# rajan-dubey8/camouflage-multimodal

Measured on AMD Instinct MI355X. Metric: images/sec fwd+bwd (fusion model train step: fwd + loss + bwd + clip + AdamW), higher is better.
Workload: dtype bf16; 1 GPU; BASELINE configs[1] on the path that exists (SURVEY 8d): cross-attention fusion model, packed variable-Nr minibatch (Nr ~ real 303..530 histogram, mean 483), Nk=13 real KG rows, train mode dropout 0.3, random-init weights; batch_per_gpu=16, global_batch=16, rg_dim=128, hidden_dim=256, num_heads=8, parallelism=dp1, precision=bf16 MFMA operands, fp32 accumulate/optimizer

## Files before the change

### camouflage_multimodal_amd/csrc/fused_rows.h

```cpp
#pragma once
#include "common.h"

typedef unsigned short us16;

struct ShadowJob { us16* dst; int N, K, transposed, nsrc; const float* src[4]; int rows[4]; int ld[4]; int chunk_begin; int lo; };
#define SHADOW_MAXJ 24
#define SHADOW_MAXZ 24
struct ShadowBatch { ShadowJob j[SHADOW_MAXJ]; int n; void* zero_ptr[SHADOW_MAXZ]; size_t zero_bytes[SHADOW_MAXZ]; int nzero; };
int launch_weight_shadows(ShadowBatch& sb, hipStream_t stream);

struct FrontStream {
  const float* X; int M;
  const us16* W0; const float* b0;
  const us16* W1; const float* bq; const float* bkv;
  us16* X16;
  us16* R16; us16* Q16; us16* KV16;
  int tile_begin;
};
#define FUSED_FRONT_MAXZ 4
#define FUSED_FRONT_MAXX 20
#define FUSED_BWD1_MAXZ 16
struct FrontArgs {
  FrontStream s[2]; float qscale; int save; unsigned long long* stamps; int exp;
  void* zero_ptr[FUSED_FRONT_MAXZ]; unsigned zero_bytes[FUSED_FRONT_MAXZ]; int nzero;
  int split3;
  ShadowJob xjob[FUSED_FRONT_MAXX]; int nxjob; int xchunks; int xblock0;
};
int launch_fused_front(FrontArgs& a, int variant, hipStream_t stream);

struct BackStream {
  const us16* Wo; const float* bo; const us16* W1; const float* b1; const float* ln_g; const float* ln_b;
  const us16* R16;
  us16* O16; us16* Y16; us16* XH16; float* rstd; uint32_t* mask;
  float* Ymean; float* Hmean;
  uint32_t site_ffn;
};
struct BackArgs {
  BackStream s[2];
  const us16* Q16; const us16* KV16;
  const us16* Q2_16; const us16* KV2_16;
  const int* off; const int* tile_off; const float* inv_nr;
  const int4* tile_desc;
  float* lse2;
  int lead_tiles;
  float* part; int* tickets; int max_splits;
  int B, Nk, rg_tiles_max, rows_rg;
  DropCfg drop; int save; int exp;
  unsigned long long* stamps;
  int save_lse2;
};
int launch_fused_back(BackArgs& a, int variant, int lead_mode, hipStream_t stream);

struct Bwd1Stream {
  const us16* W1T; const us16* WoT;
  const uint32_t* mask; const us16* XH16; const float* rstd; const float* ln_g;
  const float* dHm; int ld_dHm;
  const float* dcomb; int ld_dcomb;
  us16* dH16; us16* dU16;
  float* dgamma; float* dbeta;
};
struct TailWgProd { const float* dy; const float* x; float* dW; float* db; int ld_dy, ld_x, rows, cols; int tile_begin; };
#define TAIL_WG_MAXP 8
struct TailWgArgs { TailWgProd p[TAIL_WG_MAXP]; int n, B, tiles; };
struct Bwd1Args {
  Bwd1Stream s[2];
  const us16* Q16; const us16* KV16;
  us16* dQKV16; float* dKV;
  const us16* O2_16; us16* dO2_16; float* delta2;
  const int* off; const int* tile_off; const float* inv_nr; const int4* tile_desc;
  const int* row_sample;
  int B, Nk, rg_tiles_max, rows_rg; float qscale; DropCfg drop; unsigned long long* stamps;
  int exp;
  int writer_blocks, writer_first_row;
  void* zero_ptr[FUSED_BWD1_MAXZ]; unsigned zero_bytes[FUSED_BWD1_MAXZ]; int nzero;
  TailWgArgs twg;
};
int launch_fused_bwd1(Bwd1Args& a, int variant, hipStream_t stream, int kg_only = 0);
int launch_wide2_bwd1(Bwd1Args& a, int variant, hipStream_t stream);
size_t fused_bwd1_lds();

struct Bwd2Args {
  const us16* Q2_16; const us16* dO2_16; const float* lse2; const float* delta2;
  const us16* KV2_16;
  us16* dQKV16;
  const us16* dU16; const us16* WcRgT; us16* dR16;
  float* dQ2acc;
  const float* dKV;
  const us16* dU2_16; const us16* WcKgT; us16* dQKVkg16; us16* dG16;
  float* dGpart;
  int* tickets;
  const int* off; const int* tile_off; const int4* tile_desc;
  int B, Nk, rg_tiles_max, rows_rg; float qscale; DropCfg drop; unsigned long long* stamps;
  int param_space;
  int split_finish;
};
int launch_fused_bwd2(Bwd2Args& a, int variant, hipStream_t stream);
int launch_wide2_bwd2(Bwd2Args& a, hipStream_t stream);
size_t fused_bwd2_lds();

#define FUSED_PART_FLOATS 544
#define FUSED_MAX_SPLITS 64
size_t fused_front_lds();
size_t fused_back_lds();

#define FUSED_WIDE_MAXSEG 48
int launch_wide_front(FrontArgs& a, int rt, hipStream_t stream, int kg_only = 0);
int launch_wide_rgfwd(const FrontStream& f, float qscale, BackArgs& b, int rt, int max_nr, hipStream_t stream);
int launch_wide_back(BackArgs& a, int rt, int max_nr, hipStream_t stream);
int wide_max_rows(int rt);

int launch_fold_rg(const float* Wq, const float* Wkv, const float* bq, const float* bkv, const float* Wrg, const float* brg, us16* Wf, float* bf, hipStream_t stream);
int launch_wide2_rgfwd(const FrontStream& f, const us16* Wf, const float* bf, float qscale, BackArgs& b, int max_nr, int save_r16, hipStream_t stream);
int wide2_max_rows();
```

### camouflage_multimodal_amd/csrc/fused_rows.hip

```cpp
#include "fused_rows.h"
#include "shadow_inl.h"
#include "gemm.h"
#include "mfma_inl.h"

namespace {

template <int NT, int KS, bool W_IS_A, int DEPTH, bool USE_ROT = true>
struct Stage {
  static constexpr int TOTAL = NT * KS;
  static constexpr int D = DEPTH < TOTAL ? DEPTH : TOTAL;
  static_assert(!USE_ROT || (KS & (KS - 1)) == 0, "rotated k order: power-of-two k steps");
  u32x4 buf[D];
  const u32x4* wp; int rot;
  __device__ __forceinline__ int keff(int ks) const { return USE_ROT ? ((ks + rot) & (KS - 1)) : ks; }
  __device__ __forceinline__ const u32x4* wptr(int i) const { return wp + 64 * (keff(i / NT) * NT + (i % NT)); }
  __device__ __forceinline__ void prefetch(const u32x4* __restrict__ wp_, int rot_) {
    wp = wp_; rot = rot_;
#pragma unroll
    for (int i = 0; i < D; ++i) buf[i] = *wptr(i);
  }
  __device__ __forceinline__ void run(const char* act, f32x16 (&acc)[NT]) {
    run_f([&](int ks) { return *reinterpret_cast<const bf16x8*>(act + 32 * ks); }, acc);
  }
  template <class F>
// ... 424 lines not shown
      if (h == 0) red[slot * 128 + w * 32 + l31] = p;
      __syncthreads();
      return (red[slot * 128 + l31] + red[slot * 128 + 32 + l31]) + (red[slot * 128 + 64 + l31] + red[slot * 128 + 96 + l31]);
    };
    const float mean = row_total(part, 0) * (1.0f / 256.0f);
    float sq = 0.f;
#pragma unroll
    for (int i = 0; i < 32; ++i) { u[i] -= mean; sq = fmaf(u[i], u[i], sq); }
    const float rstd = 1.0f / sqrtf(row_total(sq, 1) * (1.0f / 256.0f) + 1e-5f);
    rstd_keep = rstd;
    const bool rok = l31 < nrows;
#pragma unroll
    for (int t = 0; t < 2; ++t) {
      float ys[16];
#pragma unroll
      for (int g = 0; g < 4; ++g) {
        const int c0 = 64 * w + 32 * t + 8 * g + 4 * h;
        const float4 gm = *reinterpret_cast<const float4*>(S.ln_g + c0), bt = *reinterpret_cast<const float4*>(S.ln_b + c0);
        float* o = u + 16 * t + 4 * g;
        const float x0 = o[0] * rstd, x1 = o[1] * rstd, x2 = o[2] * rstd, x3 = o[3] * rstd;
        const float4 y = make_float4(x0 * gm.x + bt.x, x1 * gm.y + bt.y, x2 * gm.z + bt.z, x3 * gm.w + bt.w);
        *reinterpret_cast<u32x2*>(bufY + l31 * PR + 2 * c0) = u32x2{pack2(y.x, y.y), pack2(y.z, y.w)};
        if constexpr (OCC == 3) {
          ys[4 * g] = rok ? y.x : 0.f; ys[4 * g + 1] = rok ? y.y : 0.f; ys[4 * g + 2] = rok ? y.z : 0.f; ys[4 * g + 3] = rok ? y.w : 0.f;
          if (a.save) *reinterpret_cast<u32x2*>(smem + L::XH + l31 * PR + 2 * c0) = u32x2{pack2(x0, x1), pack2(x2, x3)};
        } else {
          *reinterpret_cast<float4*>(tile32 + l31 * PT + c0) = y;
          o[0] = x0; o[1] = x1; o[2] = x2; o[3] = x3;
        }
      }
      if constexpr (OCC == 2) continue;
#pragma unroll
      for (int st = 0; st < 4; ++st) {
        const int n = 8 >> st, m = 16 >> st;
        const bool up = (l31 & m) != 0;
#pragma unroll
        for (int i = 0; i < n; ++i) {
          const float send = up ? ys[i] : ys[i + n];
          const float keep = up ? ys[i + n] : ys[i];
          ys[i] = keep + __shfl_xor(send, m, 64);
        }
      }
      const float tot = ys[0] + __shfl_xor(ys[0], 1, 64);
      if ((l31 & 1) == 0) {
        const int i16 = (l31 >> 1) & 15;
        atomicAdd(S.Ymean + (size_t)b * 256 + 64 * w + 32 * t + 8 * (i16 >> 2) + 4 * h + (i16 & 3), tot * inv_n);
      }
    }
  }
  __syncthreads();
  stamp(a.stamps, 2);
  if constexpr (OCC == 2) {
    float sum = 0.f;
    for (int r = 0; r < nrows; ++r) sum += tile32[r * PT + tid];
    atomicAdd(S.Ymean + (size_t)b * 256 + tid, sum * inv_n);
  }

  {
    f32x16 acc[4] = {zero16(), zero16(), zero16(), zero16()};
    stf.run(bufY + l31 * PR + 16 * h, acc);
    const bool dodrop = a.drop.p > 0.f;
#pragma unroll
    for (int t = 0; t < 4; ++t) {
      const int f = 128 * w + 32 * t + l31;
      const float bias = S.b1[f];
      float colsum = 0.f;
      uint32_t wlo = 0u, whi = 0u;
#pragma unroll
      for (int i = 0; i < 16; ++i) {
        if (8 * (i >> 2) >= nrows) continue;
        const int row = acc_row(i, h);
        float v = fmaxf(acc[t][i] + bias, 0.f);
        if (dodrop) v *= drop_mult(a.drop, S.site_ffn, (uint32_t)(rowg0 + row) * 512u + (uint32_t)f);
        if (row >= nrows) v = 0.f;
        colsum += v;
        if (a.save) {
          const unsigned long long bal = __ballot(v > 0.f);
          SET_LANE(wlo, (uint32_t)bal, i); SET_LANE(whi, (uint32_t)(bal >> 32), i);
        }
      }
      colsum += __shfl_xor(colsum, 32, 64);
      if (h == 0) atomicAdd(S.Hmean + (size_t)b * 512 + f, colsum * inv_n);
      if (a.save && lane < 16) {
        const int ra = acc_row(lane, 0);
        if (ra < nrows) S.mask[(rowg0 + ra) * 16 + 4 * w + t] = wlo;
        if (ra + 4 < nrows) S.mask[(rowg0 + ra + 4) * 16 + 4 * w + t] = whi;
      }
    }
  }
  if (a.save) {
    char* bufXH = smem + L::XH;
    if (w == 0 && h == 0 && l31 < nrows) S.rstd[rowg0 + l31] = rstd_keep;
    __syncthreads();
    if constexpr (OCC == 2) {
#pragma unroll
      for (int t = 0; t < 2; ++t)
#pragma unroll
        for (int g = 0; g < 4; ++g) {
          const float* o = u + 16 * t + 4 * g;
          *reinterpret_cast<u32x2*>(bufXH + l31 * PR + 2 * (64 * w + 32 * t + 8 * g + 4 * h)) = u32x2{pack2(o[0], o[1]), pack2(o[2], o[3])};
        }
      __syncthreads();
    }
    copy_out<5>(bufXH, PR, 0, S.XH16, 256, rowg0, nrows);
    copy_out<5>(bufO, PR, 0, S.O16, 256, rowg0, nrows);
    copy_out<5>(bufY, PR, 0, S.Y16, 256, rowg0, nrows);
  }
  stamp(a.stamps, 3);
}


constexpr int W_GTAB = 0, W_BUFDU = 1024, W_KS = W_BUFDU + 32 * PR, W_VS = W_KS + 16 * PK, W_BUFDO = W_VS + 16 * PK,
              W_IMGS = W_BUFDO + 32 * PR, W_RED = W_IMGS + 16384, W_LDS = W_RED + 1024;
static_assert(32 * PR + 16384 == 32 * PT * 4, "the fp32 column-sum tile aliases [bufdO | images]");

__device__ __forceinline__ void tail_wg_tile(const TailWgArgs& g, int tile, float* dys, unsigned long long* stamps) {
  stamp(stamps, 0);
  int pi = 0;
  for (int i = 1; i < g.n; ++i) if (tile >= g.p[i].tile_begin) pi = i;
  const TailWgProd& P = g.p[pi];
  const int tid = threadIdx.x, B = g.B, ncb = P.cols >> 8, lt = tile - P.tile_begin, rb = lt / ncb;
  const int r0 = 16 * rb, c = 256 * (lt - rb * ncb) + tid;
  float xv[16], acc[16];
#pragma unroll
  for (int b = 0; b < 16; ++b) xv[b] = b < B ? P.x[(size_t)b * P.ld_x + c] : 0.f;
  const float dv = tid < B * 16 ? P.dy[(size_t)(tid >> 4) * P.ld_dy + r0 + (tid & 15)] : 0.f;
#pragma unroll
  for (int r = 0; r < 16; ++r) acc[r] = P.dW[(size_t)(r0 + r) * P.cols + c];
  const bool bias = c < 16;
  float bacc = bias ? P.db[r0 + tid] : 0.f;
  if (tid < B * 16) dys[tid] = dv;
  __syncthreads();
  stamp(stamps, 1);
#pragma unroll
  for (int b = 0; b < 16; ++b) {
    if (b < B) {
      const float4* d4 = reinterpret_cast<const float4*>(dys + 16 * b);
#pragma unroll
      for (int k = 0; k < 4; ++k) {
        const float4 d = d4[k];
        acc[4 * k] = fmaf(d.x, xv[b], acc[4 * k]); acc[4 * k + 1] = fmaf(d.y, xv[b], acc[4 * k + 1]);
        acc[4 * k + 2] = fmaf(d.z, xv[b], acc[4 * k + 2]); acc[4 * k + 3] = fmaf(d.w, xv[b], acc[4 * k + 3]);
      }
      if (bias) bacc += dys[16 * b + tid];
    }
  }
  stamp(stamps, 2);
#pragma unroll
  for (int r = 0; r < 16; ++r) P.dW[(size_t)(r0 + r) * P.cols + c] = acc[r];
  if (bias) P.db[r0 + tid] = bacc;
  stamp(stamps, 3);
}

template <int DEPTH, bool ROT>
__global__ __launch_bounds__(256, 2) void bwd1_kernel(const Bwd1Args a) {
  extern __shared__ __attribute__((aligned(16))) char smem[];
  const int tid = threadIdx.x, lane = tid & 63, l31 = lane & 31, h = lane >> 5;
  const int w = __builtin_amdgcn_readfirstlane(tid >> 6);
  const bool kg = (int)blockIdx.x >= a.rg_tiles_max && (int)blockIdx.x < a.rg_tiles_max + a.B;
  const int rot = ROT ? (int)(blockIdx.x >> 3) : 0;
  if ((int)blockIdx.x >= a.B + a.rg_tiles_max + a.writer_blocks + a.nzero) {
    tail_wg_tile(a.twg, (int)blockIdx.x - a.B - a.rg_tiles_max - a.writer_blocks - a.nzero, reinterpret_cast<float*>(smem), a.stamps);
    return;
  }
  if ((int)blockIdx.x >= a.B + a.rg_tiles_max + a.writer_blocks) {
    const int zi = (int)blockIdx.x - a.B - a.rg_tiles_max - a.writer_blocks;
    u32x4* z = static_cast<u32x4*>(a.zero_ptr[zi]);
    const unsigned n16 = a.zero_bytes[zi] >> 4;
    for (unsigned i = tid; i < n16; i += 256) z[i] = u32x4{0u, 0u, 0u, 0u};
    return;
  }
  if ((int)blockIdx.x >= a.B + a.rg_tiles_max) {
    constexpr int WR = 4;
    const int wb = (int)blockIdx.x - a.B - a.rg_tiles_max;
    const int total_rows = a.rows_rg + a.B * a.Nk;
    const float gscale = a.drop.scale;
    for (int r0 = a.writer_first_row + (wb * 4 + (tid >> 6)) * WR; r0 < total_rows; r0 += 4 * WR * a.writer_blocks) {
      int sb[WR]; uint32_t word[WR]; bool isk[WR]; int row[WR];
#pragma unroll
      for (int k = 0; k < WR; ++k) {
        const int r = min(r0 + k, total_rows - 1);
        isk[k] = r >= a.rows_rg;
        row[k] = isk[k] ? r - a.rows_rg : r;
        sb[k] = isk[k] ? row[k] / a.Nk : a.row_sample[row[k]];
        word[k] = a.s[isk[k] ? 1 : 0].mask[(size_t)row[k] * 16 + (lane >> 2)];
      }
      float4 g0[WR], g1[WR]; float inv[WR];
#pragma unroll
      for (int k = 0; k < WR; ++k) {
        const Bwd1Stream& W = a.s[isk[k] ? 1 : 0];
        const float* gp = W.dHm + (size_t)sb[k] * W.ld_dHm + 8 * lane;
        g0[k] = *reinterpret_cast<const float4*>(gp); g1[k] = *reinterpret_cast<const float4*>(gp + 4);
        inv[k] = isk[k] ? 1.0f / (float)a.Nk : a.inv_nr[sb[k]];
      }
#pragma unroll
      for (int k = 0; k < WR; ++k) {
        if (r0 + k >= total_rows) break;
        const uint32_t bits = word[k] >> (8 * (lane & 3));
        const float gs = inv[k] * gscale;
        auto sel = [&](int j, float g) { return ((bits >> j) & 1u) ? (uint32_t)f2bf(g * gs) : 0u; };
        const u32x4 fr = u32x4{sel(0, g0[k].x) | (sel(1, g0[k].y) << 16), sel(2, g0[k].z) | (sel(3, g0[k].w) << 16),
                               sel(4, g1[k].x) | (sel(5, g1[k].y) << 16), sel(6, g1[k].z) | (sel(7, g1[k].w) << 16)};
        *reinterpret_cast<u32x4*>(a.s[isk[k] ? 1 : 0].dH16 + (size_t)row[k] * 512 + 8 * lane) = fr;
      }
    }
    return;
  }
  int b; size_t rowg0; int nrows; float inv_n;
  if (kg) {
    b = (int)blockIdx.x - a.rg_tiles_max; rowg0 = (size_t)b * a.Nk; nrows = a.Nk; inv_n = 1.0f / (float)a.Nk;
  } else {
    const int4 td = a.tile_desc[blockIdx.x];
    if (td.x < 0) return;
    b = td.x; rowg0 = td.y; nrows = td.z; inv_n = __int_as_float(td.w);
  }
  const Bwd1Stream& S = a.s[kg ? 1 : 0];
  us16* gtab = reinterpret_cast<us16*>(smem + W_GTAB);
  char* bufdU = smem + W_BUFDU; char* bufQ = bufdU;
  char* Ks = smem + W_KS; char* Vs = smem + W_VS; char* bufdO = smem + W_BUFDO; char* imgs = smem + W_IMGS + w * 4096;
  float* red = reinterpret_cast<float*>(smem + W_RED);
  float* tile32 = reinterpret_cast<float*>(smem + W_BUFDO);
  stamp(a.stamps, 0);
  Stage<2, 32, true, DEPTH, false> st1;
  st1.prefetch(reinterpret_cast<const u32x4*>(S.W1T) + (size_t)w * (32 * 2 * 64) + lane, 0);
  const size_t vrow = rowg0 + min(l31, nrows - 1);
  const bool rok = l31 < nrows;
  {
    const float gs = inv_n * a.drop.scale;
    for (int f = tid; f < 512; f += 256) gtab[f] = f2bf(S.dHm[(size_t)b * S.ld_dHm + f] * gs);
  }
  u32x4 mw[4];
#pragma unroll
  for (int i = 0; i < 4; ++i) mw[i] = reinterpret_cast<const u32x4*>(S.mask + vrow * 16)[i];
  u32x4 qreg[4];
  if (!kg) {
#pragma unroll
    for (int i = 0; i < 4; ++i) {
      const int id = tid + 256 * i;
      qreg[i] = *reinterpret_cast<const u32x4*>(a.Q16 + (rowg0 + min(id >> 5, nrows - 1)) * 256 + 8 * (id & 31));
    }
    for (int c = tid; c < 16 * 64; c += 256) {
      const int j = c >> 6, ch = c & 63;
      u32x4 v = u32x4{0u, 0u, 0u, 0u};
      if (j < a.Nk) v = *reinterpret_cast<const u32x4*>(a.KV16 + ((size_t)b * a.Nk + j) * 512 + 8 * ch);
      if (ch < 32) *reinterpret_cast<u32x4*>(Ks + j * PK + 16 * ch) = v;
      else         *reinterpret_cast<u32x4*>(Vs + j * PK + 16 * (ch - 32)) = v;
    }
  }
  __syncthreads();
  Stage<2, 16, true, DEPTH> st2;
  f32x16 acc1[2] = {zero16(), zero16()};
  st1.run_f([&](int ks) {
    const uint32_t word = mw[ks >> 3][(ks >> 1) & 3];
    const uint32_t bits = (word >> (16 * (ks & 1))) >> (8 * h);
    const u32x4 g = *reinterpret_cast<const u32x4*>(smem + W_GTAB + 2 * (16 * ks + 8 * h));
    u32x4 fr;
#pragma unroll
    for (int d = 0; d < 4; ++d)
      fr[d] = (((bits >> (2 * d)) & 1u) ? (g[d] & 0xFFFFu) : 0u) | (((bits >> (2 * d + 1)) & 1u) ? (g[d] & 0xFFFF0000u) : 0u);
    return as_frag(fr);
  }, acc1);
  st2.prefetch(reinterpret_cast<const u32x4*>(S.WoT) + (size_t)w * (16 * 2 * 64) + lane, rot);
  stamp(a.stamps, 1);
  {
    float gg[32], xh[32];
    float s1 = 0.f, s2 = 0.f;
#pragma unroll
    for (int t = 0; t < 2; ++t)
#pragma unroll
      for (int g = 0; g < 4; ++g) {
        const int c0 = 64 * w + 32 * t + 8 * g + 4 * h;
        const float4 dc = *reinterpret_cast<const float4*>(S.dcomb + (size_t)b * S.ld_dcomb + c0);
        const float4 gm = *reinterpret_cast<const float4*>(S.ln_g + c0);
        const u32x2 xv = *reinterpret_cast<const u32x2*>(S.XH16 + vrow * 256 + c0);
        float* G = gg + 16 * t + 4 * g; float* X = xh + 16 * t + 4 * g;
        X[0] = bf_lo(xv.x); X[1] = bf_hi(xv.x); X[2] = bf_lo(xv.y); X[3] = bf_hi(xv.y);
        const float d0 = fmaf(dc.x, inv_n, acc1[t][4 * g]), d1 = fmaf(dc.y, inv_n, acc1[t][4 * g + 1]);
        const float d2 = fmaf(dc.z, inv_n, acc1[t][4 * g + 2]), d3 = fmaf(dc.w, inv_n, acc1[t][4 * g + 3]);
        *reinterpret_cast<float4*>(tile32 + l31 * PT + c0) = make_float4(d0 * X[0], d1 * X[1], d2 * X[2], d3 * X[3]);
        acc1[t][4 * g] = d0; acc1[t][4 * g + 1] = d1; acc1[t][4 * g + 2] = d2; acc1[t][4 * g + 3] = d3;
        G[0] = d0 * gm.x; G[1] = d1 * gm.y; G[2] = d2 * gm.z; G[3] = d3 * gm.w;
#pragma unroll
        for (int i = 0; i < 4; ++i) { s1 += G[i]; s2 = fmaf(G[i], X[i], s2); }
      }
    auto row_total = [&](float p, int slot) {
      p += __shfl_xor(p, 32, 64);
      if (h == 0) red[slot * 128 + w * 32 + l31] = p;
      __syncthreads();
      return (red[slot * 128 + l31] + red[slot * 128 + 32 + l31]) + (red[slot * 128 + 64 + l31] + red[slot * 128 + 96 + l31]);
    };
    const float m1 = row_total(s1, 0) * (1.0f / 256.0f);
    const float m2 = row_total(s2, 1) * (1.0f / 256.0f);
    {
      float sum = 0.f;
      for (int r = 0; r < nrows; ++r) sum += tile32[r * PT + tid];
      atomicAdd(S.dgamma + tid, sum);
    }
    const float rstd = S.rstd[vrow];
#pragma unroll
    for (int t = 0; t < 2; ++t)
#pragma unroll
      for (int g = 0; g < 4; ++g) {
        const int c0 = 64 * w + 32 * t + 8 * g + 4 * h;
        const float* G = gg + 16 * t + 4 * g; const float* X = xh + 16 * t + 4 * g;
        float du[4];
#pragma unroll
        for (int i = 0; i < 4; ++i) du[i] = rok ? (G[i] - m1 - X[i] * m2) * rstd : 0.f;
        *reinterpret_cast<u32x2*>(bufdU + l31 * PR + 2 * c0) = u32x2{pack2(du[0], du[1]), pack2(du[2], du[3])};
      }
    __syncthreads();
#pragma unroll
    for (int t = 0; t < 2; ++t)
#pragma unroll
// ... 434 lines not shown
      const int c = 32 * head + 8 * g + 4 * h;
      *reinterpret_cast<u32x2*>(bufT + l31 * PQ + 2 * (256 + c)) = u32x2{pack2(dk[4 * g], dk[4 * g + 1]), pack2(dk[4 * g + 2], dk[4 * g + 3])};
      *reinterpret_cast<u32x2*>(bufT + l31 * PQ + 2 * (512 + c)) = u32x2{pack2(dv[4 * g], dv[4 * g + 1]), pack2(dv[4 * g + 2], dv[4 * g + 3])};
    }
    char* im = imgs + head * 1024;
    *reinterpret_cast<u32x2*>(im + l31 * 32 + 8 * h) = u32x2{dsf.x, dsf.y};
    *reinterpret_cast<u32x2*>(im + l31 * 32 + 16 + 8 * h) = u32x2{dsf.z, dsf.w};
    f32x16 dq2 = zero16();
#pragma unroll
    for (int s = 0; s < 2; ++s) {
      const int r0 = 16 * s + 8 * h + q4;
      const bf16x8 sA = join(lds_tr16(im + r0 * 32 + 8 * p4), lds_tr16(im + (r0 + 4) * 32 + 8 * p4));
      const int co = 2 * (32 * head + 16 * g1 + 4 * p4);
      const bf16x8 kB = join(lds_tr16(bufT + r0 * PQ + co), lds_tr16(bufT + (r0 + 4) * PQ + co));
      dq2 = __builtin_amdgcn_mfma_f32_32x32x16_bf16(sA, kB, dq2, 0, 0, 0);
    }
#pragma unroll
    for (int i = 0; i < 8; ++i) {
      const int j = acc_row(i, h);
      if (j < Nk) atomicAdd(a.dQ2acc + ((size_t)b * Nk + j) * 256 + 32 * head + l31, dq2[i] * a.qscale);
    }
  }
  __syncthreads();
  stamp(a.stamps, 1);
  copy_out<6>(bufT, PQ, 512, a.dQKV16 + 256, 768, rowg0, nrows);
  stamp(a.stamps, 2);
  }
  if (a.split_finish) return;
  asm volatile("s_waitcnt vmcnt(0)" ::: "memory");
  __syncthreads();
  if (tid == 0) flag[0] = __hip_atomic_fetch_add(a.tickets + b, 1, __ATOMIC_RELAXED, __HIP_MEMORY_SCOPE_AGENT);
  __syncthreads();
  if (flag[0] != a.tile_off[b + 1] - a.tile_off[b]) return;
  if (tid == 0) {
    __builtin_amdgcn_fence(__ATOMIC_ACQUIRE, "agent");
    asm volatile("s_waitcnt vmcnt(0)" ::: "memory");
  }
  __syncthreads();
  const size_t krow0 = (size_t)b * Nk;
  for (int c = tid; c < 32 * 32; c += 256) {
    const int j = c >> 5, ch = c & 31;
    u32x4 v = u32x4{0u, 0u, 0u, 0u};
    if (j < Nk) {
      const float* src = a.dQ2acc + (krow0 + j) * 256 + 8 * ch;
      const float4 x0 = *reinterpret_cast<const float4*>(src), x1 = *reinterpret_cast<const float4*>(src + 4);
      v = u32x4{pack2(x0.x, x0.y), pack2(x0.z, x0.w), pack2(x1.x, x1.y), pack2(x1.z, x1.w)};
    }
    *reinterpret_cast<u32x4*>(bufT + j * PQ + 16 * ch) = v;
  }
  __syncthreads();
  copy_out<5>(bufT, PQ, 0, a.dQKVkg16, 768, krow0, Nk);
  stamp(a.stamps, 3);
}

__global__ __launch_bounds__(256) void bwd2_finish_kernel(const Bwd2Args a) {
  const size_t krow0 = (size_t)blockIdx.x * a.Nk;
  for (int c = threadIdx.x; c < a.Nk * 32; c += 256) {
    const int j = c >> 5, ch = c & 31;
    const float* src = a.dQ2acc + (krow0 + j) * 256 + 8 * ch;
    const float4 x0 = *reinterpret_cast<const float4*>(src), x1 = *reinterpret_cast<const float4*>(src + 4);
    *reinterpret_cast<u32x4*>(a.dQKVkg16 + (krow0 + j) * 768 + 8 * ch) = u32x4{pack2(x0.x, x0.y), pack2(x0.z, x0.w), pack2(x1.x, x1.y), pack2(x1.z, x1.w)};
  }
}

bool al16(const void* p) { return (reinterpret_cast<uintptr_t>(p) & 15) == 0; }

}

size_t fused_front_lds() { return F_LDS; }
size_t fused_back_lds() { return B_LDS; }

int launch_weight_shadows(ShadowBatch& sb, hipStream_t stream) {
  if (sb.n < 0 || sb.n > SHADOW_MAXJ) return (int)hipErrorInvalidValue;
  int total = 0;
  for (int i = 0; i < sb.n; ++i) {
    ShadowJob& J = sb.j[i];
    if ((J.N & 127) || (J.K & 15) || J.nsrc < 1 || J.nsrc > 4 || !J.dst || !al16(J.dst)) return (int)hipErrorInvalidValue;
    int sum = 0;
    for (int s = 0; s < J.nsrc; ++s) {
      if (!J.src[s] || (J.rows[s] & 7) || (!J.transposed && (!al16(J.src[s]) || (J.ld[s] & 3)))) return (int)hipErrorInvalidValue;
      sum += J.rows[s];
    }
    if (sum != (J.transposed ? J.K : J.N)) return (int)hipErrorInvalidValue;
    J.chunk_begin = total;
    total += J.N * J.K / 8;
  }
  if (sb.nzero < 0 || sb.nzero > SHADOW_MAXZ) return (int)hipErrorInvalidValue;
  for (int i = 0; i < sb.nzero; ++i)
    if (!sb.zero_ptr[i] || !al16(sb.zero_ptr[i]) || (sb.zero_bytes[i] & 15)) return (int)hipErrorInvalidValue;
  int blocks = (total + 255) / 256;
  if (sb.nzero && blocks < 64) blocks = 64;
  if (blocks == 0) return 0;
  const int prof = gemm_prof_open(stream, 0.0, PROF_SHADOW);
  hipLaunchKernelGGL(shadow_kernel, dim3(blocks), dim3(256), 0, stream, sb, total);
  gemm_prof_close(prof, stream);
  return (int)hipGetLastError();
}

int launch_fused_front(FrontArgs& a, int variant, hipStream_t stream) {
  int total = 0;
  for (int i = 0; i < 2; ++i) {
    FrontStream& S = a.s[i];
    if (S.M < 1 || !S.X || !S.W0 || !S.W1 || !S.b0 || !S.bq || !S.bkv || !S.R16 || !S.Q16 || !S.KV16 || (a.save && !S.X16))
      return (int)hipErrorInvalidValue;
    if (!al16(S.X) || !al16(S.b0) || !al16(S.bq) || !al16(S.bkv) || !al16(S.R16) || !al16(S.Q16) || !al16(S.KV16) || !al16(S.W0) || !al16(S.W1))
      return (int)hipErrorInvalidValue;
    S.tile_begin = total;
    total += (S.M + 31) / 32;
  }
  if (a.nzero < 0 || a.nzero > FUSED_FRONT_MAXZ) return (int)hipErrorInvalidValue;
  for (int i = 0; i < a.nzero; ++i)
    if (!a.zero_ptr[i] || !al16(a.zero_ptr[i]) || (a.zero_bytes[i] & 15)) return (int)hipErrorInvalidValue;
  const int prof = gemm_prof_open(stream, 2.0 * ((double)a.s[0].M + a.s[1].M) * (128.0 * 256.0 + 256.0 * 768.0), PROF_FRONT);
  if (variant == 0)      launch_lds<front_kernel<12, false>>(dim3(total), dim3(256), F_LDS, stream, a);
  else if (variant != 2) launch_lds<front_kernel<12, true>>(dim3(total), dim3(256), F_LDS, stream, a);
  else                   launch_lds<front_kernel<16, true>>(dim3(total), dim3(256), F_LDS, stream, a);
  gemm_prof_close(prof, stream);
  return (int)hipGetLastError();
}

int launch_fused_back(BackArgs& a, int variant, int lead_mode, hipStream_t stream) {
  if (a.B < 1 || a.Nk < 1 || a.Nk > 16 || a.rg_tiles_max < 1 || !a.Q16 || !a.KV16 || !a.Q2_16 || !a.KV2_16 || !a.off || !a.tile_off || !a.tile_desc || !a.inv_nr ||
      !a.part || !a.tickets || a.max_splits < 1 || a.max_splits > FUSED_MAX_SPLITS)
    return (int)hipErrorInvalidValue;
  for (int i = 0; i < 2; ++i) {
    const BackStream& S = a.s[i];
    if (!S.Wo || !S.bo || !S.W1 || !S.b1 || !S.ln_g || !S.ln_b || !S.R16 || !S.Ymean || !S.Hmean) return (int)hipErrorInvalidValue;
    if (a.save && (!S.O16 || !S.Y16 || !S.XH16 || !S.rstd || !S.mask)) return (int)hipErrorInvalidValue;
    if (!al16(S.bo) || !al16(S.ln_g) || !al16(S.ln_b) || !al16(S.Wo) || !al16(S.W1) || !al16(S.R16)) return (int)hipErrorInvalidValue;
  }
  const dim3 grid(a.B * a.max_splits + a.rg_tiles_max);
  a.lead_tiles = (lead_mode != 0 && a.rows_rg / 32 >= 256 && (int)grid.x > 512) ? 256 : 0;
  const double rows = (double)a.rows_rg + (double)a.B * a.Nk;
  const int prof = gemm_prof_open(stream, 2.0 * rows * (256.0 * 256.0 + 256.0 * 512.0) + 8.0 * (double)a.rows_rg * a.Nk * 256.0, PROF_BACK);
  if (variant == 0)        launch_lds<back_kernel<12, false, 2>>(grid, dim3(256), BackL<2>::LDS, stream, a);
  else if (variant != 2) {
    if (grid.x <= 512u)    launch_lds<back_kernel<12, true, 2>>(grid, dim3(256), BackL<2>::LDS, stream, a);
    else                   launch_lds<back_kernel<12, true, 3>>(grid, dim3(256), BackL<3>::LDS, stream, a);
  } else                   launch_lds<back_kernel<16, true, 2>>(grid, dim3(256), BackL<2>::LDS, stream, a);
  gemm_prof_close(prof, stream);
  return (int)hipGetLastError();
}

size_t fused_bwd1_lds() { return W_LDS; }

int launch_fused_bwd1(Bwd1Args& a, int variant, hipStream_t stream, int kg_only) {
  if (a.B < 1 || a.Nk < 1 || a.Nk > 16 || a.rg_tiles_max < 1 || !a.Q16 || !a.KV16 || !a.dQKV16 || !a.dKV || !a.O2_16 || !a.dO2_16 || !a.delta2 ||
      !a.off || !a.tile_off || !a.tile_desc || !a.inv_nr || !a.row_sample)
    return (int)hipErrorInvalidValue;
  for (int i = 0; i < 2; ++i) {
    const Bwd1Stream& S = a.s[i];
    if (!S.W1T || !S.WoT || !S.mask || !S.XH16 || !S.rstd || !S.ln_g || !S.dHm || !S.dcomb || !S.dH16 || !S.dU16 || !S.dgamma || !S.dbeta)
      return (int)hipErrorInvalidValue;
    if (!al16(S.W1T) || !al16(S.WoT) || !al16(S.mask) || !al16(S.ln_g) || !al16(S.dcomb) || (S.ld_dcomb & 3) || !al16(S.dH16) || !al16(S.dU16))
      return (int)hipErrorInvalidValue;
  }
  a.writer_first_row = kg_only ? a.rows_rg : 0;
  a.writer_blocks = (a.rows_rg + a.B * a.Nk - a.writer_first_row + 15) / 16;
  if (a.writer_blocks > 8192) a.writer_blocks = 8192;
  if (a.nzero < 0 || a.nzero > FUSED_BWD1_MAXZ) return (int)hipErrorInvalidValue;
  for (int i = 0; i < a.nzero; ++i)
    if (!a.zero_ptr[i] || !al16(a.zero_ptr[i]) || (a.zero_bytes[i] & 15)) return (int)hipErrorInvalidValue;
  TailWgArgs& t = a.twg;
  if (t.n < 0 || t.n > TAIL_WG_MAXP || (t.n && (t.B < 1 || t.B > 16))) return (int)hipErrorInvalidValue;
  t.tiles = 0;
  for (int i = 0; i < t.n; ++i) {
    TailWgProd& p = t.p[i];
    if (!p.dy || !p.x || !p.dW || !p.db || p.rows < 16 || (p.rows & 15) || p.cols < 256 || (p.cols & 255) || p.ld_dy < p.rows || p.ld_x < p.cols)
      return (int)hipErrorInvalidValue;
    p.tile_begin = t.tiles;
    t.tiles += (p.rows / 16) * (p.cols / 256);
  }
  Bwd1Args k = a;
  if (kg_only) { k.rg_tiles_max = 0; k.stamps = nullptr; }
  const dim3 grid(k.B + k.rg_tiles_max + k.writer_blocks + k.nzero + k.twg.tiles);
  const double rows = (kg_only ? 0.0 : (double)a.rows_rg) + (double)a.B * a.Nk;
  const int prof = gemm_prof_open(stream, 2.0 * rows * (512.0 * 256.0 + 256.0 * 256.0) + (kg_only ? 0.0 : 10.0 * (double)a.rows_rg * a.Nk * 256.0), PROF_BWD1);
  if (variant == 0) launch_lds<bwd1_kernel<12, false>>(grid, dim3(256), W_LDS, stream, k);
  else              launch_lds<bwd1_kernel<12, true>>(grid, dim3(256), W_LDS, stream, k);
  gemm_prof_close(prof, stream);
  return (int)hipGetLastError();
}

size_t fused_bwd2_lds() { return X_LDS; }

int launch_fused_bwd2(Bwd2Args& a, int variant, hipStream_t stream) {
  (void)variant;
  if (a.B < 1 || a.Nk < 1 || a.Nk > 16 || a.rg_tiles_max < 1 || !a.Q2_16 || !a.dO2_16 || !a.lse2 || !a.delta2 || !a.KV2_16 || !a.dQKV16 ||
      !a.dU16 || !a.WcRgT || !a.dR16 || !a.dQ2acc || !a.dKV || !a.dU2_16 || !a.WcKgT || !a.dQKVkg16 || !a.dG16 || !a.dGpart || !a.tickets || !a.off || !a.tile_off || !a.tile_desc)
    return (int)hipErrorInvalidValue;
  if (!al16(a.dQKV16) || !al16(a.dQKVkg16) || !al16(a.WcRgT) || !al16(a.WcKgT) || !al16(a.dQ2acc) || !al16(a.dKV)) return (int)hipErrorInvalidValue;
  const double rows = (double)a.rows_rg + (double)a.B * a.Nk;
  const int prof = gemm_prof_open(stream, (a.param_space ? 0.0 : 2.0 * rows * 768.0 * 256.0) + 10.0 * (double)a.rows_rg * a.Nk * 256.0, PROF_BWD2);
  if (!a.param_space) a.split_finish = 0;
  if (!a.param_space) launch_lds<bwd2_kernel<12, false>>(dim3(a.B + a.rg_tiles_max), dim3(256), X_LDS, stream, a);
  else                launch_lds<bwd2p_kernel<12, false>>(dim3(a.B + a.rg_tiles_max), dim3(256), X_LDS, stream, a);
  if (a.split_finish) hipLaunchKernelGGL(bwd2_finish_kernel, dim3(a.B), dim3(256), 0, stream, a);
  gemm_prof_close(prof, stream);
  return (int)hipGetLastError();
}
```

### camouflage_multimodal_amd/csrc/fusion_abi.hip

```cpp
#include <hip/hip_runtime.h>

#include <algorithm>
#include <cmath>
#include <cstdio>
#include <cstring>
#include <string>

#include "../../include/camo_fusion.h"

#include "attn.h"
#include "gemm.h"
#include "fused_rows.h"
#include "tail_wide.h"
#include "attn_maps.h"
#include "gemm16.h"
#include "misc.h"
#include "abi_util.h"

namespace {
thread_local std::string g_err;
}

int camo_abi::fail(int code, const std::string& msg) { g_err = msg; return code; }
int camo_abi::fail_hip(int e, const char* where) {
  g_err = std::string(where) + ": " + hipGetErrorString((hipError_t)e);
  return CAMO_E_HIP;
}
using namespace camo_abi;

namespace {

constexpr camo_options_t k_default_options = { -1,  -1,  -1,  -1,  -1,  1,  0,
                                               -1,  -1,  -1,  -1,  1,  1,
                                               1,  0,  0,  0,  0,  0,  -1};
unsigned long long* g_dbg_stamps = nullptr;
int g_dbg_stamp_blocks = 0;


struct Call {
  void* shadows = nullptr;
  bool shadows_valid = false;
  bool fold_missing = false;
  int shadows_state = 0;
  void* zero_bwd1_ptr[FUSED_BWD1_MAXZ]; unsigned zero_bwd1_bytes[FUSED_BWD1_MAXZ]; int nzero_bwd1 = 0;
  hipEvent_t tail_event = nullptr;
  int tail_skip = 0;
  bool tail_skip_taken = false;
};
const camo_options_t& options_of(const camo_dims_t* d) { return *(d && d->options ? d->options : &k_default_options); }

typedef unsigned short us;

struct Desc { int* row_sample; float* inv_nr; int* tile_off; int4* tile_desc; size_t bytes; };
Desc desc_carve(int B, int T, void* base) {
  Desc d{};
  Carver c(base);
  d.row_sample = c.take<int>((size_t)T); d.inv_nr = c.take<float>((size_t)B); d.tile_off = c.take<int>((size_t)B + 1);
  d.tile_desc = c.take<int4>((size_t)T / 32 + B);
  c.off = (c.off + 255) & ~size_t(255);
  d.bytes = c.off;
  return d;
}

static inline size_t tail_counter_words(int B) { return (size_t)4 * ((B + 15) / 16 > 0 ? (B + 15) / 16 : 1); }

struct Ws {
  float* zero_base; size_t zero_bytes;
  float *R, *G, *Q, *KV2, *KV, *Q2, *P, *P2, *O, *O2, *U, *U2, *st1, *st2, *Y, *Y2, *H1, *H2;
  float *means, *Ymean, *H1mean, *Y2mean, *H2mean; size_t means_n;
  float *comb, *F1, *fused, *hid, *a2;
  float *dlog, *dhid, *dfused, *dF1, *dcomb, *dHm1, *dHm2, *da2;
  float *dH1, *dH2, *dY, *dY2, *dU, *dU2, *dO, *dO2, *dQ, *dKV, *dQ2, *dKV2, *dS2, *dR, *dG;
  struct H16 {
    unsigned short *X, *KG, *R, *G, *O, *O2, *Y, *Y2, *dH1, *dH2, *dU, *dU2, *dQKV, *dQKVkg, *dR, *dG;
    unsigned short *H1, *H2;
    unsigned short *Wrg, *Wkg, *Win1, *Win2, *Wo1, *Wo2, *W1, *W2, *W1T, *W2T, *Wo1T, *Wo2T, *WcRgT, *WcKgT;
  } h;
  size_t Tp, TKp;
  struct F17 {
    us16 *Wrg, *Wkg, *Wqkv_rg, *Wqkv_kg, *Wo1, *Wo2, *W1, *W2;
    us16* Wf_rg; float* bf_rg;
    us16 *X16, *KG16, *R16, *G16, *Q16, *Q2_16, *KV16, *KV2_16, *O16, *O2_16, *Y16, *Y2_16, *XH16, *XH2_16;
    float *rstd1, *rstd2, *lse2, *part; uint32_t *mask1, *mask2;
    us16 *W1T, *W2T, *Wo1T, *Wo2T, *WcRgT, *WcKgT;
    us16 *dH16, *dH2_16, *dU16, *dU2_16, *dQKV16, *dQKVkg16, *dR16, *dG16, *dO2_16;
    float *delta2, *dGpart;
    us16* tailw[20];
  } f;
  int* tickets;
  float* dQ2acc;
  float* parM;
  float* tailsum;
  size_t bytes;
};

bool fused17_dims(const camo_dims_t& d) {
  return d.fusion_type == CAMO_FUSION_CROSS_ATTENTION && d.hidden_dim == 256 && d.num_heads == 8 && d.rg_dim == 128 && d.kg_dim == 128;
}

Ws carve(const camo_dims_t& d, int B, int T, int Nk, void* base) {
  Ws w{};
  Carver c(base);
  const size_t H = d.hidden_dim, TK = (size_t)B * Nk, nh = d.num_heads, Wd = 2 * d.num_classes + 2;
  if (d.fusion_type == CAMO_FUSION_CROSS_ATTENTION) {
    const size_t Fh = H / 2;
    w.R = c.take<float>(T * H); w.G = c.take<float>(TK * H);
    w.Q = c.take<float>(T * H); w.KV2 = c.take<float>(T * 2 * H);
    w.KV = c.take<float>(TK * 2 * H); w.Q2 = c.take<float>(TK * H);
    w.P = c.take<float>(T * nh * Nk); w.P2 = c.take<float>(T * nh * Nk);
    w.O = c.take<float>(T * H); w.O2 = c.take<float>(TK * H);
    w.U = c.take<float>(T * H); w.U2 = c.take<float>(TK * H);
    w.st1 = c.take<float>(T * 2); w.st2 = c.take<float>(TK * 2);
    w.Y = c.take<float>(T * H); w.Y2 = c.take<float>(TK * H);
    w.H1 = c.take<float>(T * 2 * H); w.H2 = c.take<float>(TK * 2 * H);
    w.means_n = (size_t)B * 6 * H;
    {
      const size_t nzt = ((size_t)2 * B + 3) & ~size_t(3);
      const size_t npar = (size_t)2 * (3 * H * d.rg_dim + 3 * H) + 8;
      const size_t nz = w.means_n + (size_t)B * H + nzt + TK * 2 * H + TK * H + (size_t)B * 4 * H + ((tail_counter_words(B) + 3) & ~size_t(3)) + npar;
      float* z = c.take<float>(nz);
      w.zero_base = z; w.zero_bytes = nz * sizeof(float);
      w.means = z; w.dfused = z ? z + w.means_n : nullptr;
      w.tickets = z ? reinterpret_cast<int*>(w.dfused + (size_t)B * H) : nullptr;
      w.dKV = z ? w.dfused + (size_t)B * H + nzt : nullptr;
      w.dQ2acc = z ? w.dKV + TK * 2 * H : nullptr;
      w.tailsum = z ? w.dQ2acc + TK * H : nullptr;
      w.parM = z ? w.tailsum + (size_t)B * 4 * H + ((tail_counter_words(B) + 3) & ~size_t(3)) : nullptr;
    }
    if (w.means) { w.Ymean = w.means; w.H1mean = w.Ymean + B * H; w.Y2mean = w.H1mean + B * 2 * H; w.H2mean = w.Y2mean + B * H; }
    w.comb = c.take<float>(B * 2 * H); w.F1 = c.take<float>(B * H); w.fused = c.take<float>(B * H);
    w.hid = c.take<float>(B * 4 * Fh);
    w.dlog = c.take<float>(B * Wd); w.dhid = c.take<float>(B * 4 * Fh);
    w.dF1 = c.take<float>(B * H); w.dcomb = c.take<float>(B * 2 * H);
    w.dHm1 = c.take<float>(B * 2 * H); w.dHm2 = c.take<float>(B * 2 * H);
    w.dH1 = c.take<float>(T * 2 * H); w.dH2 = c.take<float>(TK * 2 * H);
    w.dY = c.take<float>(T * H); w.dY2 = c.take<float>(TK * H);
    w.dU = c.take<float>(T * H); w.dU2 = c.take<float>(TK * H);
    w.dO = c.take<float>(T * H); w.dO2 = c.take<float>(TK * H);
    w.dQ = c.take<float>(T * H);
    w.dQ2 = c.take<float>(TK * H); w.dKV2 = c.take<float>(T * 2 * H);
    w.dS2 = c.take<float>(T * nh * Nk);
    w.dR = c.take<float>(T * H); w.dG = c.take<float>(TK * H);
    {
      const size_t Tp = ((size_t)T + 127) / 128 * 128, TKp = (TK + 127) / 128 * 128, D = d.rg_dim, Dk = d.kg_dim;
      w.Tp = Tp; w.TKp = TKp;
      Ws::H16& h = w.h;
      h.X = c.take<us>(Tp * D); h.KG = c.take<us>(TKp * Dk); h.R = c.take<us>(Tp * H); h.G = c.take<us>(TKp * H);
      h.O = c.take<us>(Tp * H); h.O2 = c.take<us>(TKp * H); h.Y = c.take<us>(Tp * H); h.Y2 = c.take<us>(TKp * H);
      h.dH1 = c.take<us>(Tp * 2 * H); h.dH2 = c.take<us>(TKp * 2 * H); h.dU = c.take<us>(Tp * H); h.dU2 = c.take<us>(TKp * H);
      h.dQKV = c.take<us>(Tp * 3 * H); h.dQKVkg = c.take<us>(TKp * 3 * H); h.dR = c.take<us>(Tp * H); h.dG = c.take<us>(TKp * H);
      h.Wrg = c.take<us>(H * D); h.Wkg = c.take<us>(H * Dk); h.Win1 = c.take<us>(3 * H * H); h.Win2 = c.take<us>(3 * H * H);
      h.Wo1 = c.take<us>(H * H); h.Wo2 = c.take<us>(H * H); h.W1 = c.take<us>(2 * H * H); h.W2 = c.take<us>(2 * H * H);
      h.W1T = c.take<us>(2 * H * H); h.W2T = c.take<us>(2 * H * H); h.Wo1T = c.take<us>(H * H); h.Wo2T = c.take<us>(H * H);
      h.WcRgT = c.take<us>(3 * H * H); h.WcKgT = c.take<us>(3 * H * H);
      h.H1 = c.take<us>(Tp * 2 * H); h.H2 = c.take<us>(TKp * 2 * H);
      if (fused17_dims(d)) {
        Ws::F17& f = w.f;
        f.Wrg = c.take<us>(H * D); f.Wkg = c.take<us>(H * Dk); f.Wqkv_rg = c.take<us>(3 * H * H); f.Wqkv_kg = c.take<us>(3 * H * H);
        f.Wo1 = c.take<us>(H * H); f.Wo2 = c.take<us>(H * H); f.W1 = c.take<us>(2 * H * H); f.W2 = c.take<us>(2 * H * H);
        f.X16 = c.take<us>(Tp * D); f.KG16 = c.take<us>(TKp * Dk); f.R16 = c.take<us>(Tp * H); f.G16 = c.take<us>(TKp * H);
        f.Q16 = c.take<us>(Tp * H); f.Q2_16 = c.take<us>(TKp * H); f.KV16 = c.take<us>(TKp * 2 * H); f.KV2_16 = c.take<us>(Tp * 2 * H);
        f.O16 = c.take<us>(Tp * H); f.O2_16 = c.take<us>(TKp * H); f.Y16 = c.take<us>(Tp * H); f.Y2_16 = c.take<us>(TKp * H);
        f.XH16 = c.take<us>(Tp * H); f.XH2_16 = c.take<us>(TKp * H);
        f.rstd1 = c.take<float>(Tp); f.rstd2 = c.take<float>(TKp); f.lse2 = c.take<float>((size_t)B * 8 * 16 * 2);
        f.mask1 = c.take<uint32_t>(Tp * 16); f.mask2 = c.take<uint32_t>(TKp * 16);
        f.part = c.take<float>(((size_t)T / 32 + B + 2) * 8 * FUSED_PART_FLOATS);
        f.W1T = c.take<us>(2 * H * H); f.W2T = c.take<us>(2 * H * H); f.Wo1T = c.take<us>(H * H); f.Wo2T = c.take<us>(H * H);
        f.WcRgT = c.take<us>(3 * H * H); f.WcKgT = c.take<us>(3 * H * H);
        f.dH16 = c.take<us>(Tp * 2 * H); f.dH2_16 = c.take<us>(TKp * 2 * H); f.dU16 = c.take<us>(Tp * H); f.dU2_16 = c.take<us>(TKp * H);
        f.dQKV16 = c.take<us>(Tp * 3 * H); f.dQKVkg16 = c.take<us>(TKp * 3 * H); f.dR16 = c.take<us>(Tp * H); f.dG16 = c.take<us>(TKp * H);
        f.dO2_16 = c.take<us>(TKp * H); f.delta2 = c.take<float>((size_t)B * 8 * 16); f.dGpart = c.take<float>(TKp * H);
        for (int i = 0; i < 10; ++i) f.tailw[i] = c.take<us>(i < 6 ? 2 * H * H : (i < 8 ? H * H : 2 * H * H));
        for (int i = 10; i < 20; ++i) f.tailw[i] = c.take<us>((i == 12 || i == 13) ? H * H : 2 * H * H);
        f.Wf_rg = c.take<us>(3 * H * D); f.bf_rg = c.take<float>(3 * H);
      }
    }
  } else {
    const size_t F = H / 2, Fh = F / 2, Dc = (size_t)d.rg_dim + d.kg_dim;
    w.means_n = (size_t)B * Dc;
    {
      const size_t nz = w.means_n + (size_t)B * F;
      float* z = c.take<float>(nz);
      w.zero_base = z; w.zero_bytes = nz * sizeof(float);
      w.comb = z;
      w.dfused = z ? z + w.means_n : nullptr;
    }
    w.means = w.comb;
    w.F1 = c.take<float>(B * H);
    w.a2 = c.take<float>(B * F);
    w.fused = c.take<float>(B * F);
    w.hid = c.take<float>(B * 4 * Fh);
    w.dlog = c.take<float>(B * Wd); w.dhid = c.take<float>(B * 4 * Fh);
    w.da2 = c.take<float>(B * F); w.dF1 = c.take<float>(B * H);
  }
  c.off = (c.off + 255) & ~size_t(255);
  w.bytes = c.off;
  return w;
}

int check_dims(const camo_dims_t* d, int B, int T, int Nk) {
  if (!d) return fail(CAMO_E_ARG, "dims is null");
  if (B < 1 || T < B || Nk < 1) return fail(CAMO_E_ARG, "need B >= 1, T >= B (every sample has >= 1 RG row), Nk >= 1");
  if (d->rg_dim < 1 || d->kg_dim < 1 || d->hidden_dim < 4 || d->num_classes < 1 || d->num_classes > 64)
    return fail(CAMO_E_ARG, "bad model dimensions");
  if (!(d->dropout >= 0.f && d->dropout < 1.f)) return fail(CAMO_E_ARG, "dropout must be in [0,1)");
  if (d->fusion_type == CAMO_FUSION_CROSS_ATTENTION) {
    if (d->num_heads < 1 || d->hidden_dim % d->num_heads) return fail(CAMO_E_ARG, "hidden_dim must be divisible by num_heads");
    if (d->hidden_dim % 2) return fail(CAMO_E_UNSUPPORTED, "hidden_dim must be even");
    if (!attn_supported(d->hidden_dim, d->num_heads, Nk))
      return fail(CAMO_E_UNSUPPORTED, "attention kernels support num_heads <= 256, head_dim <= 256, Nk <= 64 within 160 KB of LDS");
    if (!ln_supported(d->hidden_dim)) return fail(CAMO_E_UNSUPPORTED, "LayerNorm kernels support hidden_dim <= 1024");
  } else if (d->fusion_type == CAMO_FUSION_LATE) {
    if (d->hidden_dim % 4) return fail(CAMO_E_UNSUPPORTED, "late fusion needs hidden_dim divisible by 4");
  } else {
    return fail(CAMO_E_ARG, "unknown fusion_type");
  }
  if ((double)T * d->hidden_dim * 2 > 2.0e9 || (double)T * d->num_heads * Nk > 4.0e9)
    return fail(CAMO_E_UNSUPPORTED, "batch too large for 32-bit element indices");
  return 0;
}

void set_res(GemmProb& p, const float* res, int ldr) { p.res = res; p.ldr = ldr; }
void set_drop(GemmProb& p, uint32_t site) { p.flags |= GF_DROPOUT; p.drop_site = site; }
void set_bcast(GemmProb& p, const float* v, int ldv, const int* row_sample, const float* inv_nr, int uniform_n) {
  p.flags |= GF_RES_BCAST; p.res = v; p.ldr = ldv; p.row_sample = row_sample; p.inv_nr = inv_nr; p.uniform_n = uniform_n;
}

struct GB16 {
  Gemm16Batch b; Gemm16Knobs kn; hipStream_t st;
  GB16(const DropCfg& d, const camo_options_t& o, hipStream_t st_) : st(st_) {
    std::memset(&b, 0, sizeof(b)); b.drop = d;
    kn.tn_big = o.tn_big; kn.balance = o.tn_balance; kn.tn_kcap = o.tn_kcap; kn.exp = o.tn_exp;
  }
  Gemm16Prob& add() { Gemm16Prob& p = b.p[b.n++]; std::memset(&p, 0, sizeof(p)); p.aux_scale = 1.f; return p; }
  Gemm16Prob& nt(const us* x, int ldx, const us* W, int ldw, const float* bias, float* y, int ldy, us* y16, int ldy16,
                 int M, int N, int K, int flags = 0) {
    Gemm16Prob& p = add();
    p.A = x; p.lda = ldx; p.B = W; p.ldb = ldw; p.bias = bias; p.C = y; p.ldc = ldy; p.C16 = y16; p.ldc16 = ldy16;
    p.M = M; p.N = N; p.K = K; p.flags = flags;
    return p;
  }
  Gemm16Prob& tn(const us* dy, int lddy, const us* x, int ldx, float* dW, int lddw, float* db, int Nout, int Nin, int rows) {
    Gemm16Prob& p = add();
    p.A = dy; p.lda = lddy; p.B = x; p.ldb = ldx; p.C = dW; p.ldc = lddw; p.bias_grad = db;
    p.M = Nout; p.N = Nin; p.K = rows; p.flags = GF_A_KMAJOR | GF_B_KMAJOR | GF_ATOMIC;
    return p;
  }
  int run() {
    if (b.n == 0) return 0;
    int e = launch_gemm16_batch(b, kn, st);
    b.n = 0;
    return e;
  }
};
void set_res(Gemm16Prob& p, const float* res, int ldr) { p.res = res; p.ldr = ldr; }
void set_drop(Gemm16Prob& p, uint32_t site) { p.flags |= GF_DROPOUT; p.drop_site = site; }
void set_bcast(Gemm16Prob& p, const float* v, int ldv, const int* row_sample, const float* inv_nr, int uniform_n) {
  p.flags |= GF_RES_BCAST; p.res = v; p.ldr = ldv; p.row_sample = row_sample; p.inv_nr = inv_nr; p.uniform_n = uniform_n;
}

struct ShadowSet { us16 *Wrg, *Wkg, *Wqkv_rg, *Wqkv_kg, *Wo1, *Wo2, *W1, *W2, *W1T, *W2T, *Wo1T, *Wo2T, *WcRgT, *WcKgT, *Wf_rg; float* bf_rg; size_t bytes; };
static ShadowSet shadow_carve(void* base) {
  ShadowSet x{};
  Carver c(base);
  const size_t H = 256, D = 128, HH = H * H;
  x.Wrg = c.take<us16>(H * D); x.Wkg = c.take<us16>(H * D); x.Wqkv_rg = c.take<us16>(3 * HH); x.Wqkv_kg = c.take<us16>(3 * HH);
  x.Wo1 = c.take<us16>(HH); x.Wo2 = c.take<us16>(HH); x.W1 = c.take<us16>(2 * HH); x.W2 = c.take<us16>(2 * HH);
  x.W1T = c.take<us16>(2 * HH); x.W2T = c.take<us16>(2 * HH); x.Wo1T = c.take<us16>(HH); x.Wo2T = c.take<us16>(HH);
  x.WcRgT = c.take<us16>(3 * HH); x.WcKgT = c.take<us16>(3 * HH);
  x.Wf_rg = c.take<us16>(3 * H * D); x.bf_rg = c.take<float>(3 * H);
  x.bytes = (c.off + 255) & ~size_t(255);
  return x;
}
void bind_shadows(void* shadows, Ws& w) {
  const ShadowSet x = shadow_carve(shadows);
  Ws::F17& f = w.f;
  f.Wrg = x.Wrg; f.Wkg = x.Wkg; f.Wqkv_rg = x.Wqkv_rg; f.Wqkv_kg = x.Wqkv_kg; f.Wo1 = x.Wo1; f.Wo2 = x.Wo2; f.W1 = x.W1; f.W2 = x.W2;
  f.W1T = x.W1T; f.W2T = x.W2T; f.Wo1T = x.Wo1T; f.Wo2T = x.Wo2T; f.WcRgT = x.WcRgT; f.WcKgT = x.WcKgT;
  f.Wf_rg = x.Wf_rg; f.bf_rg = x.bf_rg;
}

enum CallKind { CALL_INFERENCE, CALL_FORWARD_SAVE , CALL_BACKWARD, CALL_TRAIN  };
struct PlanIn {
  const camo_options_t& o; const camo_dims_t& d;
  bool rg_proj, kg_proj;
  int precision, B, T, Nk, max_nr;
  CallKind kind;
  bool attn_maps;
  bool fused_maps;
  int cus;
};

static void plan_fused_forward(const PlanIn& in, bool save, bool param_space, camo_plan_t& p) {
  const camo_options_t& o = in.o;
  const int B = in.B, T = in.T, max_nr = in.max_nr, C = in.d.num_classes;
  const bool infer = in.kind == CALL_INFERENCE, train = in.kind == CALL_TRAIN;
  int rt = o.fused_rt;
  if (rt < 0) rt = save ? 0 : (T >= 22528 ? 4 : (T >= 13312 ? 2 : 0));
  if (rt != 0 && rt != 1 && rt != 2 && rt != 4) rt = 0;
  if (rt && max_nr > wide_max_rows(rt) - 64 * rt) rt = 0;
  const bool maps = p.maps != 0;
  if (maps) rt = 0;
  bool rg64 = !maps && o.wide2 != 0 && o.fused_one != 0 && max_nr <= wide2_max_rows();
  if (rg64 && o.wide2 < 0) rg64 = o.fused_rt < 0 && o.wide_front_rt == 0 && T >= (save ? 57344 : 10240);
  const bool rg_one = rg64 || (rt >= 2 && o.fused_one != 0);
  const bool rows128 = T >= 4 * 32 * 224;
  int wf_rt = 0;
  if ((save || maps) && rt == 0 && o.fused_rt < 0 && o.wide_front_rt >= 0 && (T >= 10240 || o.wide_front_rt > 0)) {
    wf_rt = o.wide_front_rt > 0 ? o.wide_front_rt : (rows128 ? 4 : 2);
    if ((wf_rt != 1 && wf_rt != 2 && wf_rt != 4) || max_nr > wide_max_rows(wf_rt) - 64 * wf_rt) wf_rt = 0;
  }
  p.save = save;
  if (rg_one) p.front = CAMO_FRONT_KG;
  else if (rt || wf_rt) { p.front = CAMO_FRONT_WIDE; p.front_rt = rt ? rt : wf_rt; }
  else p.front = CAMO_FRONT_ROWS32;
  if (rg64) {
    p.back = CAMO_BACK_RG_64;
    p.save_r16 = !param_space || o.fused_save != 0;
  } else if (rt) { p.back = rg_one ? CAMO_BACK_RG_WIDE : CAMO_BACK_WIDE; p.back_rt = rt; }
  else p.back = CAMO_BACK_ROWS32;

  const bool one_launch = o.tail17 != 0 && tail_fused_ok(B, C, in.cus);
  const bool planes_infer = infer && o.tailw != 0 && rg_one && tail_wide_ok(B, C) && (o.tailw > 0 || B > 32 || !tail_fused_ok(B, C, in.cus));
  const bool planes_train = train && heads_loss_ok(B, C) && B > 64 && o.tailw != 0 && rows128 && wf_rt != 0 && tail_wide_ok(B, C);
  if (planes_infer) p.tail = CAMO_TAIL_PLANES;
  else if ((infer || train) && one_launch) p.tail = CAMO_TAIL_ONE_LAUNCH;
  else if (planes_train) p.tail = o.tailw_bwd != 0 ? CAMO_TAIL_PLANES_TRAIN : CAMO_TAIL_PLANES_TRAIN_FWD;
  else p.tail = CAMO_TAIL_GEMMS;
  if (train && p.tail == CAMO_TAIL_ONE_LAUNCH) {
    p.loss = CAMO_LOSS_TAIL;
    p.tail_wg = B > 16 ? CAMO_TAIL_WG_LAUNCH : CAMO_TAIL_WG_BWD1;
    p.tail_event = p.tail_wg == CAMO_TAIL_WG_BWD1 ? CAMO_EVENT_AFTER_BWD1 : CAMO_EVENT_BEFORE_NODES;
  }
}

static void plan_fused_backward(const PlanIn& in, bool param_space, camo_plan_t& p) {
  const camo_options_t& o = in.o;
  p.param_space = param_space;
  const bool bwd1w = o.wide2_bwd != 0 && (o.wide2_bwd > 0 || (o.fused_rt < 0 && in.T >= 16384));
  p.bwd1 = bwd1w ? CAMO_BWD1_64 : CAMO_BWD1_ROWS32;
  p.bwd2 = !(param_space && bwd1w) ? CAMO_BWD2_ROWS32 : (o.wide2_bwd != 2 ? CAMO_BWD2_64 : CAMO_BWD2_ROWS32_SPLIT);
}

camo_plan_t make_plan(const PlanIn& in) {
  const camo_options_t& o = in.o; const camo_dims_t& d = in.d;
  const int B = in.B, T = in.T, Nk = in.Nk, max_nr = in.max_nr;
  const bool train = in.kind == CALL_TRAIN;
  camo_plan_t p; std::memset(&p, 0, sizeof(p));
  if (train) p.loss = heads_loss_ok(B, d.num_classes) ? CAMO_LOSS_HEADS : CAMO_LOSS_LAUNCH;
  if (d.fusion_type == CAMO_FUSION_LATE) {
    p.nodes = CAMO_NODES_LATE;
    if (train) p.tail_event = CAMO_EVENT_END;
    return p;
  }
  if (train) p.tail_event = CAMO_EVENT_BEFORE_NODES;
  const bool proj = in.rg_proj && in.kg_proj, bf16 = in.precision == CAMO_PREC_BF16;
  const bool maps = in.attn_maps && in.fused_maps && in.kind == CALL_INFERENCE;
  if ((!in.attn_maps || maps) && o.fused != 0 && bf16 && fused17_dims(d) && Nk <= 16 && max_nr <= 64 * FUSED_MAX_SPLITS && proj) {
    p.nodes = CAMO_NODES_FUSED;
    p.maps = maps;
    p.shadows = in.kind != CALL_BACKWARD;
    const bool param_space = o.param_space < 0 ? T >= 10240 : o.param_space > 0;
    if (in.kind != CALL_BACKWARD) plan_fused_forward(in, in.kind != CALL_INFERENCE || o.fused_save != 0, param_space, p);
    if (in.kind == CALL_BACKWARD || train) plan_fused_backward(in, param_space, p);
    return p;
  }
  const bool use16 = o.sched16 != 0 && bf16 && proj && !(d.hidden_dim % 64) && !(d.rg_dim % 64) && !(d.kg_dim % 64) &&
                     attn_mfma_ok(d.hidden_dim, d.num_heads, Nk, max_nr, false) && attn_mfma_ok(d.hidden_dim, d.num_heads, Nk, max_nr, true) &&
                     ((double)T + 128.0) * 3.0 * d.hidden_dim * 2.0 < 4.0e9;
  p.nodes = use16 ? CAMO_NODES_BF16 : CAMO_NODES_GENERAL;
  return p;
}

struct Batch {
  const camo_dims_t* dims; const float* const* P; float* const* Gr; const float* rg; const int32_t* rg_offsets; const void* desc; const float* kg;
  int B, T, Nk, max_nr; void* workspace; size_t workspace_bytes; int training; uint64_t seed; int precision; hipStream_t st;
  const camo_options_t* opt; camo_plan_t plan; Desc bd; Ws w; DropCfg drop;
};

void plan_batch(Batch& x, CallKind kind, bool attn_maps, bool fused_maps = false) {
  x.opt = &options_of(x.dims);
  if (x.P) x.plan = make_plan(PlanIn{*x.opt, *x.dims, x.P[CAMO_P_RG_PROJ_W] != nullptr, x.P[CAMO_P_KG_PROJ_W] != nullptr, x.precision, x.B, x.T, x.Nk, x.max_nr,
                                     kind, attn_maps, fused_maps, device_cus()});
}

int open_batch(Batch& x, const Call& c, bool ptrs_ok) {
  if (!x.P || !x.rg || !x.rg_offsets || !x.desc || !x.kg || !x.workspace || !ptrs_ok) return fail(CAMO_E_ARG, "null pointer argument");
  x.bd = desc_carve(x.B, x.T, const_cast<void*>(x.desc));
  if (x.max_nr < 1 || x.max_nr > x.T) return fail(CAMO_E_ARG, "max_nr out of range");
  if (x.precision != CAMO_PREC_F32 && x.precision != CAMO_PREC_BF16) return fail(CAMO_E_ARG, "unknown precision");
  x.w = carve(*x.dims, x.B, x.T, x.Nk, x.workspace);
  if (c.shadows) bind_shadows(c.shadows, x.w);
  if (x.workspace_bytes < x.w.bytes) return fail(CAMO_E_WORKSPACE, "workspace smaller than camo_workspace_bytes()");
  x.drop = make_drop(x.training, x.dims->dropout, x.seed);
  return 0;
}

struct FusedLoss { const int64_t* y; const float* e; const float* s; float* terms; int32_t* pred; };
GB tail_gemms(const Batch& x) { return GB(x.drop, CAMO_PREC_F32, x.st); }

int heads_forward(const Batch& x, int head0, int F, float* outs, const FusedLoss* fl, bool hidden_done = false, bool defer_out_grads = false) {
  const camo_dims_t& d = *x.dims; const Ws& w = x.w;
  const float* const* hp = x.P + head0;
  const int B = x.B, Fh = F / 2, C = d.num_classes, Wd = 2 * C + 2;
  const int nout[4] = {C, C, 1, 1}, coff[4] = {0, C, 2 * C, 2 * C + 1};
  GB g = tail_gemms(x);
  if (!hidden_done) {
    for (int h = 0; h < 4; ++h) {
      GemmProb& p = g.nt(w.fused, F, hp[4 * h], F, hp[4 * h + 1], w.hid + h * Fh, 4 * Fh, B, Fh, F, GF_RELU);
      set_drop(p, SITE_HEAD0 + h);
    }
    CK(g.run(), "heads hidden");
  }
  if (fl) {
    float* const* hg = x.Gr + head0;
    HeadsOut ho;
    for (int h = 0; h < 4; ++h) { ho.W[h] = hp[4 * h + 2]; ho.b[h] = hp[4 * h + 3]; ho.gW[h] = hg[4 * h + 2]; ho.gb[h] = hg[4 * h + 3]; }
    CK(launch_heads_loss(w.hid, ho, reinterpret_cast<const long long*>(fl->y), fl->e, fl->s, B, C, Fh, x.drop.scale, outs, fl->terms,
                         fl->pred, w.dhid, x.st, defer_out_grads ? w.dlog : nullptr), "heads out + loss + heads out bwd");
    return 0;
  }
  for (int h = 0; h < 4; ++h)
    g.nt(w.hid + h * Fh, 4 * Fh, hp[4 * h + 2], Fh, hp[4 * h + 3], outs + coff[h], Wd, B, nout[h], Fh, h == 3 ? GF_SIGMOID : 0);
  CK(g.run(), "heads out");
  return 0;
}

int heads_backward(const Batch& x, int head0, int F, const float* outs, const float* d_outs, int pre_activation, bool heads_out_done) {
  const camo_dims_t& d = *x.dims; const Ws& w = x.w;
  const float* const* hp = x.P + head0; float* const* hg = x.Gr + head0;
  const int B = x.B, Fh = F / 2, C = d.num_classes, Wd = 2 * C + 2;
  const int nout[4] = {C, C, 1, 1}, coff[4] = {0, C, 2 * C, 2 * C + 1};
  GB g = tail_gemms(x);
  if (!heads_out_done) {
    const float* dlog = d_outs;
    if (!pre_activation) { CK(launch_head_out_grad(outs, d_outs, w.dlog, B, Wd, x.st), "head_out_grad"); dlog = w.dlog; }
    for (int h = 0; h < 4; ++h) {
      GemmProb& p = g.nn(dlog + coff[h], Wd, hp[4 * h + 2], Fh, w.dhid + h * Fh, 4 * Fh, B, Fh, nout[h]);
      set_relu_bwd(p, w.hid + h * Fh, 4 * Fh, x.drop.scale);
      g.tn(dlog + coff[h], Wd, w.hid + h * Fh, 4 * Fh, hg[4 * h + 2], Fh, hg[4 * h + 3], nout[h], Fh, B);
    }
    CK(g.run(), "heads out bwd");
  }
  for (int h = 0; h < 4; ++h) {
    g.nn(w.dhid + h * Fh, 4 * Fh, hp[4 * h], F, w.dfused, F, B, F, Fh, GF_ATOMIC);
    g.tn(w.dhid + h * Fh, 4 * Fh, w.fused, F, hg[4 * h], F, hg[4 * h + 1], Fh, F, B);
  }
  CK(g.run(), "heads hidden bwd");
  return 0;
}

template <typename F> void for_tail_wg(const Batch& b, F&& f) {
  const Ws& w = b.w; float* const* Gr = b.Gr;
  const int H = b.dims->hidden_dim, Fh = H / 2;
  for (int h = 0; h < 4; ++h) f(w.dhid + h * Fh, 4 * Fh, w.fused, H, Gr[CAMO_P_HEADS + 4 * h], Gr[CAMO_P_HEADS + 4 * h + 1], Fh, H);
  f(w.dfused, H, w.F1, H, Gr[CAMO_P_FU_W3], Gr[CAMO_P_FU_B3], H, H);
  f(w.dF1, H, w.comb, 2 * H, Gr[CAMO_P_FU_W0], Gr[CAMO_P_FU_B0], H, 2 * H);
  f(w.dcomb, 2 * H, w.H1mean, 2 * H, Gr[CAMO_P_F1_W3], Gr[CAMO_P_F1_B3], H, 2 * H);
  f(w.dcomb + H, 2 * H, w.H2mean, 2 * H, Gr[CAMO_P_F2_W3], Gr[CAMO_P_F2_B3], H, 2 * H);
}
void add_tail_wg(const Batch& b, GB& g) {
  for_tail_wg(b, [&](const float* dy, int ld_dy, const float* x, int ld_x, float* dW, float* db, int rows, int cols) { g.tn(dy, ld_dy, x, ld_x, dW, cols, db, rows, cols, b.B); });
}

int forward_nodes16(const Batch& x, float* attn_rg2kg, float* attn_kg2rg) {
  const camo_dims_t& d = *x.dims; const float* const* P = x.P; const Ws& w = x.w; const DropCfg& drop = x.drop; hipStream_t st = x.st;
  const float* rg = x.rg; const float* kg = x.kg; const int32_t* rg_offsets = x.rg_offsets;
  const int32_t* row_sample = x.bd.row_sample; const float* inv_nr = x.bd.inv_nr;
  const int B = x.B, T = x.T, Nk = x.Nk, max_nr = x.max_nr;
  const int H = d.hidden_dim, D = d.rg_dim, Dk = d.kg_dim, TK = B * Nk, nh = d.num_heads;
  const size_t HH = (size_t)H * H;
  const Ws::H16& h = w.h;
  {
    PrepBatch pb; pb.n = 0;
    auto job = [&](int type, const float* src, void* dst, size_t n, int rows, int cols, int ld, int off) {
      PrepJob& J = pb.j[pb.n++];
      J.type = type; J.src = src; J.dst = dst; J.n = n; J.rows = rows; J.cols = cols; J.ld_dst = ld; J.col_off = off; J.blk_begin = 0;
    };
    auto cast = [&](const float* src, us* dst, size_t n) { job(PREP_CAST, src, dst, n, 0, 0, 0, 0); };
    auto castT = [&](const float* src, us* dst, int rows, int cols, int ld, int off) { job(PREP_CAST_T, src, dst, 0, rows, cols, ld, off); };
    auto pad = [&](us* buf, size_t rows, size_t rows_p, size_t width) {
      job(PREP_ZERO, nullptr, buf + rows * width, (rows_p - rows) * width * sizeof(us), 0, 0, 0, 0);
    };
    job(PREP_ZERO, nullptr, w.zero_base, (size_t)(reinterpret_cast<char*>(w.dKV) - reinterpret_cast<char*>(w.zero_base)), 0, 0, 0, 0);
    cast(rg, h.X, (size_t)T * D); cast(kg, h.KG, (size_t)TK * Dk);
    cast(P[CAMO_P_RG_PROJ_W], h.Wrg, (size_t)H * D); cast(P[CAMO_P_KG_PROJ_W], h.Wkg, (size_t)H * Dk);
    cast(P[CAMO_P_A1_IN_W], h.Win1, 3 * HH); cast(P[CAMO_P_A2_IN_W], h.Win2, 3 * HH);
    cast(P[CAMO_P_A1_OUT_W], h.Wo1, HH); cast(P[CAMO_P_A2_OUT_W], h.Wo2, HH);
    cast(P[CAMO_P_F1_W0], h.W1, 2 * HH); cast(P[CAMO_P_F2_W0], h.W2, 2 * HH);
    castT(P[CAMO_P_F1_W0], h.W1T, 2 * H, H, 2 * H, 0); castT(P[CAMO_P_F2_W0], h.W2T, 2 * H, H, 2 * H, 0);
    castT(P[CAMO_P_A1_OUT_W], h.Wo1T, H, H, H, 0); castT(P[CAMO_P_A2_OUT_W], h.Wo2T, H, H, H, 0);
    castT(P[CAMO_P_A1_IN_W], h.WcRgT, H, H, 3 * H, 0); castT(P[CAMO_P_A2_IN_W] + HH, h.WcRgT, 2 * H, H, 3 * H, H);
    castT(P[CAMO_P_A2_IN_W], h.WcKgT, H, H, 3 * H, 0); castT(P[CAMO_P_A1_IN_W] + HH, h.WcKgT, 2 * H, H, 3 * H, H);
    const size_t t = T, tk = TK;
    pad(h.X, t, w.Tp, D); pad(h.R, t, w.Tp, H); pad(h.O, t, w.Tp, H); pad(h.Y, t, w.Tp, H); pad(h.dH1, t, w.Tp, 2 * H);
    pad(h.dU, t, w.Tp, H); pad(h.dQKV, t, w.Tp, 3 * H); pad(h.dR, t, w.Tp, H); pad(h.H1, t, w.Tp, 2 * H);
    pad(h.KG, tk, w.TKp, Dk); pad(h.G, tk, w.TKp, H); pad(h.O2, tk, w.TKp, H); pad(h.Y2, tk, w.TKp, H); pad(h.dH2, tk, w.TKp, 2 * H);
    pad(h.dU2, tk, w.TKp, H); pad(h.dQKVkg, tk, w.TKp, 3 * H); pad(h.dG, tk, w.TKp, H); pad(h.H2, tk, w.TKp, 2 * H);
    CK(launch_prep(pb, st), "prep (clear + bf16 casts)");
  }
  GB16 g(drop, *x.opt, st);
  g.nt(h.KG, Dk, h.Wkg, Dk, P[CAMO_P_KG_PROJ_B], w.G, H, h.G, H, TK, H, Dk);
  g.nt(h.X, D, h.Wrg, D, P[CAMO_P_RG_PROJ_B], w.R, H, h.R, H, T, H, D);
  CK(g.run(), "input projections");
  g.nt(h.R, H, h.Win1, H, P[CAMO_P_A1_IN_B], w.Q, H, nullptr, 0, T, H, H);
  g.nt(h.R, H, h.Win2 + HH, H, P[CAMO_P_A2_IN_B] + H, w.KV2, 2 * H, nullptr, 0, T, 2 * H, H);
  g.nt(h.G, H, h.Win1 + HH, H, P[CAMO_P_A1_IN_B] + H, w.KV, 2 * H, nullptr, 0, TK, 2 * H, H);
  g.nt(h.G, H, h.Win2, H, P[CAMO_P_A2_IN_B], w.Q2, H, nullptr, 0, TK, H, H);
  CK(g.run(), "attention in-projections");
  CK(launch_attn_fwd_pair(w.Q, w.KV, w.Q2, w.KV2, rg_offsets, w.P, w.P2, Bf16Dst{h.O, H}, Bf16Dst{h.O2, H}, w.O2, B, max_nr, H, nh, Nk,
                          drop, st), "attention fwd (both directions)");
  if (attn_rg2kg) CK(launch_attn_avg_site(w.P, attn_rg2kg, T, nh, Nk, SITE_ATTN_RG2KG, drop, st), "attn avg rg2kg");
  if (attn_kg2rg) CK(launch_attn_avg(w.P2, attn_kg2rg, T, nh, Nk, drop, st), "attn avg");
  if (H == 256) {
    Gemm16Prob& p1 = g.nt(h.O, H, h.Wo1, H, P[CAMO_P_A1_OUT_B], w.U, H, h.Y, H, T, H, H);
    set_res(p1, w.R, H);
    p1.ln_mode = 1; p1.ln_gamma = P[CAMO_P_LN1_W]; p1.ln_beta = P[CAMO_P_LN1_B]; p1.ln_stats = w.st1;
    p1.colmean = w.Ymean; p1.ldm = H; p1.row_sample = row_sample; p1.inv_nr = inv_nr;
    Gemm16Prob& p2 = g.nt(h.O2, H, h.Wo2, H, P[CAMO_P_A2_OUT_B], w.U2, H, h.Y2, H, TK, H, H);
    set_res(p2, w.G, H);
    p2.ln_mode = 1; p2.ln_gamma = P[CAMO_P_LN2_W]; p2.ln_beta = P[CAMO_P_LN2_B]; p2.ln_stats = w.st2;
    p2.colmean = w.Y2mean; p2.ldm = H; p2.uniform_n = Nk;
    CK(g.run(), "attention out-projections + layernorm");
  } else {
    set_res(g.nt(h.O, H, h.Wo1, H, P[CAMO_P_A1_OUT_B], w.U, H, nullptr, 0, T, H, H), w.R, H);
    set_res(g.nt(h.O2, H, h.Wo2, H, P[CAMO_P_A2_OUT_B], w.U2, H, nullptr, 0, TK, H, H), w.G, H);
    CK(g.run(), "attention out-projections");
    LnSeg s0{w.U, w.Y, w.st1, P[CAMO_P_LN1_W], P[CAMO_P_LN1_B], T, h.Y, w.Ymean, row_sample, inv_nr, 0};
    LnSeg s1{w.U2, w.Y2, w.st2, P[CAMO_P_LN2_W], P[CAMO_P_LN2_B], TK, h.Y2, w.Y2mean, nullptr, nullptr, Nk};
    CK(launch_ln_fwd(s0, s1, H, st), "layernorm fwd");
  }
  {
    Gemm16Prob& p1 = g.nt(h.Y, H, h.W1, H, P[CAMO_P_F1_B0], nullptr, 0, h.H1, 2 * H, T, 2 * H, H, GF_RELU);
    set_drop(p1, SITE_FFN_RG);
    p1.colmean = w.H1mean; p1.ldm = 2 * H; p1.row_sample = row_sample; p1.inv_nr = inv_nr;
    Gemm16Prob& p2 = g.nt(h.Y2, H, h.W2, H, P[CAMO_P_F2_B0], nullptr, 0, h.H2, 2 * H, TK, 2 * H, H, GF_RELU);
    set_drop(p2, SITE_FFN_KG);
    p2.colmean = w.H2mean; p2.ldm = 2 * H; p2.uniform_n = Nk;
  }
  CK(g.run(), "ffn layer 0");
  return 0;
}

int forward_nodes17(Call& c, const Batch& x, float* attn_rg2kg, float* attn_kg2rg) {
  const camo_plan_t& pl = x.plan; const float* const* P = x.P; const Ws& w = x.w; hipStream_t st = x.st;
  const int H = 256, D = 128, B = x.B, T = x.T, Nk = x.Nk, TK = B * Nk, max_nr = x.max_nr;
  const size_t HH = (size_t)H * H;
  const bool save = pl.save != 0;
  const Ws::F17& f = w.f;
  FrontArgs fa; std::memset(&fa, 0, sizeof(fa));
  {
    ShadowBatch sb; std::memset(&sb, 0, sizeof(sb));
    auto job = [&](us* dst, int N, int K, int transposed, const float* s0, int r0, const float* s1 = nullptr, int r1 = 0) {
      ShadowJob& J = sb.j[sb.n++];
      const int ld = transposed ? N : K;
      J.dst = dst; J.N = N; J.K = K; J.transposed = transposed; J.nsrc = s1 ? 2 : 1;
      J.src[0] = s0; J.rows[0] = r0; J.ld[0] = ld; J.src[1] = s1; J.rows[1] = r1; J.ld[1] = ld;
    };
    const bool build = !c.shadows_valid;
    if (c.shadows) c.shadows_state = save ? 2 : 1;
    if (build) {
      job(f.Wrg, H, D, 0, P[CAMO_P_RG_PROJ_W], H); job(f.Wkg, H, D, 0, P[CAMO_P_KG_PROJ_W], H);
      job(f.Wqkv_rg, 3 * H, H, 0, P[CAMO_P_A1_IN_W], H, P[CAMO_P_A2_IN_W] + HH, 2 * H);
      job(f.Wqkv_kg, 3 * H, H, 0, P[CAMO_P_A2_IN_W], H, P[CAMO_P_A1_IN_W] + HH, 2 * H);
      job(f.Wo1, H, H, 0, P[CAMO_P_A1_OUT_W], H); job(f.Wo2, H, H, 0, P[CAMO_P_A2_OUT_W], H);
      job(f.W1, 2 * H, H, 0, P[CAMO_P_F1_W0], 2 * H); job(f.W2, 2 * H, H, 0, P[CAMO_P_F2_W0], 2 * H);
    }
    auto zero = [&](void* ptr, size_t bytes) { if (bytes) { sb.zero_ptr[sb.nzero] = ptr; sb.zero_bytes[sb.nzero++] = (bytes + 15) & ~size_t(15); } };
    if (save) {
      if (build) {
        job(f.W1T, H, 2 * H, 1, P[CAMO_P_F1_W0], 2 * H); job(f.W2T, H, 2 * H, 1, P[CAMO_P_F2_W0], 2 * H);
        job(f.Wo1T, H, H, 1, P[CAMO_P_A1_OUT_W], H); job(f.Wo2T, H, H, 1, P[CAMO_P_A2_OUT_W], H);
        job(f.WcRgT, H, 3 * H, 1, P[CAMO_P_A1_IN_W], H, P[CAMO_P_A2_IN_W] + HH, 2 * H);
        job(f.WcKgT, H, 3 * H, 1, P[CAMO_P_A2_IN_W], H, P[CAMO_P_A1_IN_W] + HH, 2 * H);
      }
      zero(w.zero_base, w.zero_bytes);
      const size_t t = T, tk = TK;
      auto pad = [&](us* buf, size_t rows, size_t rows_p, size_t width) { zero(buf + rows * width, (rows_p - rows) * width * sizeof(us)); };
      pad(f.X16, t, w.Tp, D); pad(f.R16, t, w.Tp, H); pad(f.O16, t, w.Tp, H); pad(f.Y16, t, w.Tp, H); pad(f.dH16, t, w.Tp, 2 * H);
      pad(f.dU16, t, w.Tp, H); pad(f.dQKV16, t, w.Tp, 3 * H); pad(f.dR16, t, w.Tp, H);
      pad(f.KG16, tk, w.TKp, D); pad(f.G16, tk, w.TKp, H); pad(f.O2_16, tk, w.TKp, H); pad(f.Y2_16, tk, w.TKp, H); pad(f.dH2_16, tk, w.TKp, 2 * H);
      pad(f.dU2_16, tk, w.TKp, H); pad(f.dQKVkg16, tk, w.TKp, 3 * H); pad(f.dG16, tk, w.TKp, H);
      zero(w.dHm1, (size_t)B * 2 * H * sizeof(float)); zero(w.dHm2, (size_t)B * 2 * H * sizeof(float));
    } else {
      zero(w.zero_base, (size_t)(reinterpret_cast<char*>(w.dKV) - reinterpret_cast<char*>(w.zero_base)));
      zero(w.tailsum, ((size_t)B * 4 * H + ((tail_counter_words(B) + 3) & ~size_t(3))) * sizeof(float));
    }
    const bool fold = !save && (build || c.fold_missing);
    if (build) CK(launch_weight_shadows(sb, st), "weight shadows");
    if (fold) CK(launch_fold_rg(P[CAMO_P_A1_IN_W], P[CAMO_P_A2_IN_W] + HH, P[CAMO_P_A1_IN_B], P[CAMO_P_A2_IN_B] + H, P[CAMO_P_RG_PROJ_W], P[CAMO_P_RG_PROJ_B],
                                f.Wf_rg, f.bf_rg, st), "folded in-projection");
    if (!build) {
      for (int i = 0; i < sb.nzero; ++i) {
        const bool early = sb.zero_ptr[i] == (void*)w.zero_base || sb.zero_ptr[i] == (void*)w.dHm1 || sb.zero_ptr[i] == (void*)w.dHm2 || sb.zero_ptr[i] == (void*)w.tailsum;
        if (sb.zero_bytes[i] > 0xFFFFFFF0ull) return fail(CAMO_E_ARG, "clear range too large");
        if (early) {
          if (fa.nzero >= FUSED_FRONT_MAXZ) return fail(CAMO_E_ARG, "too many early clear ranges");
          fa.zero_ptr[fa.nzero] = sb.zero_ptr[i]; fa.zero_bytes[fa.nzero++] = (unsigned)sb.zero_bytes[i];
        } else {
          if (c.nzero_bwd1 >= FUSED_BWD1_MAXZ) return fail(CAMO_E_ARG, "too many late clear ranges");
          c.zero_bwd1_ptr[c.nzero_bwd1] = sb.zero_ptr[i]; c.zero_bwd1_bytes[c.nzero_bwd1++] = (unsigned)sb.zero_bytes[i];
        }
      }
    }
  }
  fa.qscale = 1.0f / sqrtf(32.0f); fa.save = save ? 1 : 0;
  fa.s[0] = FrontStream{x.rg, T, f.Wrg, P[CAMO_P_RG_PROJ_B], f.Wqkv_rg, P[CAMO_P_A1_IN_B], P[CAMO_P_A2_IN_B] + H, f.X16, f.R16, f.Q16, f.KV2_16, 0};
  fa.s[1] = FrontStream{x.kg, TK, f.Wkg, P[CAMO_P_KG_PROJ_B], f.Wqkv_kg, P[CAMO_P_A2_IN_B], P[CAMO_P_A1_IN_B] + H, f.KG16, f.G16, f.Q2_16, f.KV16, 0};
  fa.stamps = g_dbg_stamps; fa.exp = x.opt->exp;
  if (pl.tail >= CAMO_TAIL_PLANES) {
    const float* hsrc[4] = {P[CAMO_P_HEADS], P[CAMO_P_HEADS + 4], P[CAMO_P_HEADS + 8], P[CAMO_P_HEADS + 12]};
    auto xj = [&](us* dst, int N, int K, int transposed, const float* src, int lo) {
      ShadowJob& J = fa.xjob[fa.nxjob++];
      std::memset(&J, 0, sizeof(J));
      J.dst = dst; J.N = N; J.K = K; J.transposed = transposed; J.nsrc = 1; J.src[0] = src; J.rows[0] = transposed ? K : N; J.ld[0] = transposed ? N : K; J.lo = lo;
    };
    auto xheads = [&](us* dst, int N, int K, int transposed, int lo) {
      ShadowJob& J = fa.xjob[fa.nxjob++];
      std::memset(&J, 0, sizeof(J));
      J.dst = dst; J.N = N; J.K = K; J.transposed = transposed; J.nsrc = 4; J.lo = lo;
      for (int h = 0; h < 4; ++h) { J.src[h] = hsrc[h]; J.rows[h] = H / 2; J.ld[h] = H; }
    };
    for (int lo = 0; lo < 2; ++lo) {
      xj(f.tailw[0 + lo], H, 2 * H, 0, P[CAMO_P_F1_W3], lo); xj(f.tailw[2 + lo], H, 2 * H, 0, P[CAMO_P_F2_W3], lo);
      xj(f.tailw[4 + lo], H, 2 * H, 0, P[CAMO_P_FU_W0], lo); xj(f.tailw[6 + lo], H, H, 0, P[CAMO_P_FU_W3], lo);
    }
    for (int lo = 0; lo < 2; ++lo) xheads(f.tailw[8 + lo], 2 * H, H, 0, lo);
    if (pl.tail != CAMO_TAIL_PLANES)
      for (int lo = 0; lo < 2; ++lo) {
        xheads(f.tailw[10 + lo], H, 2 * H, 1, lo);
        xj(f.tailw[12 + lo], H, H, 1, P[CAMO_P_FU_W3], lo);
        xj(f.tailw[14 + lo], 2 * H, H, 1, P[CAMO_P_FU_W0], lo);
        xj(f.tailw[16 + lo], 2 * H, H, 1, P[CAMO_P_F1_W3], lo);
        xj(f.tailw[18 + lo], 2 * H, H, 1, P[CAMO_P_F2_W3], lo);
      }
  }
  if (pl.front == CAMO_FRONT_KG) { fa.split3 = 1; CK(launch_wide_front(fa, 1, st, 1), "fused forward, KG rows' front half (32-row tiles, one in-projection pass per block)"); }
  else if (pl.front == CAMO_FRONT_WIDE) CK(launch_wide_front(fa, pl.front_rt, st, 0), "fused forward, front half (wide tiles)");
  else CK(launch_fused_front(fa, x.opt->fused_variant, st), "fused forward, front half");
  BackArgs ba; std::memset(&ba, 0, sizeof(ba));
  ba.s[0] = BackStream{f.Wo1, P[CAMO_P_A1_OUT_B], f.W1, P[CAMO_P_F1_B0], P[CAMO_P_LN1_W], P[CAMO_P_LN1_B], f.R16,
                       f.O16, f.Y16, f.XH16, f.rstd1, f.mask1, w.Ymean, w.H1mean, SITE_FFN_RG};
  ba.s[1] = BackStream{f.Wo2, P[CAMO_P_A2_OUT_B], f.W2, P[CAMO_P_F2_B0], P[CAMO_P_LN2_W], P[CAMO_P_LN2_B], f.G16,
                       f.O2_16, f.Y2_16, f.XH2_16, f.rstd2, f.mask2, w.Y2mean, w.H2mean, SITE_FFN_KG};
  ba.Q16 = f.Q16; ba.KV16 = f.KV16; ba.Q2_16 = f.Q2_16; ba.KV2_16 = f.KV2_16;
  ba.off = x.rg_offsets; ba.tile_off = x.bd.tile_off; ba.tile_desc = x.bd.tile_desc; ba.inv_nr = x.bd.inv_nr; ba.lse2 = f.lse2;
  ba.B = B; ba.Nk = Nk; ba.rows_rg = T; ba.rg_tiles_max = T / 32 + B;
  ba.part = f.part; ba.tickets = w.tickets; ba.max_splits = (max_nr + 63) / 64;
  ba.drop = x.drop; ba.save = save ? 1 : 0; ba.save_lse2 = pl.maps; ba.exp = x.opt->exp;
  ba.stamps = g_dbg_stamps ? g_dbg_stamps + (size_t)g_dbg_stamp_blocks * 8 : nullptr;
  switch (pl.back) {
    case CAMO_BACK_RG_64: CK(launch_wide2_rgfwd(fa.s[0], f.Wf_rg, f.bf_rg, fa.qscale, ba, max_nr, pl.save_r16, st), "fused forward, RG rows in one launch (64-row half-blocks)"); break;
    case CAMO_BACK_RG_WIDE: CK(launch_wide_rgfwd(fa.s[0], fa.qscale, ba, pl.back_rt, max_nr, st), "fused forward, RG rows in one launch (wide tiles)"); break;
    case CAMO_BACK_WIDE: CK(launch_wide_back(ba, pl.back_rt, max_nr, st), "fused forward, back half (wide tiles)"); break;
    default: CK(launch_fused_back(ba, x.opt->fused_variant, x.opt->back_lead, st), "fused forward, back half");
  }
  if (pl.maps) {
    AttnMapsArgs ma; std::memset(&ma, 0, sizeof(ma));
    ma.Q16 = f.Q16; ma.KV16 = f.KV16; ma.Q2_16 = f.Q2_16; ma.KV2_16 = f.KV2_16; ma.lse2 = f.lse2; ma.tile_desc = x.bd.tile_desc;
    ma.rg2kg = attn_rg2kg; ma.kg2rg = attn_kg2rg; ma.Nk = Nk; ma.tiles = T / 32 + B; ma.rows_rg = T;
    CK(launch_attn_maps(ma, st), "attention maps of the fused forward");
  }
  return 0;
}

int record_tail_event(const Call& c, hipStream_t st) { return c.tail_event ? (int)hipEventRecord(c.tail_event, st) : 0; }

int backward_nodes16(const Batch& x) {
  const camo_dims_t& d = *x.dims; const float* const* P = x.P; float* const* Gr = x.Gr; const Ws& w = x.w; const DropCfg& drop = x.drop; hipStream_t st = x.st;
  const int32_t* rg_offsets = x.rg_offsets; const int32_t* row_sample = x.bd.row_sample; const float* inv_nr = x.bd.inv_nr;
  const int B = x.B, T = x.T, Nk = x.Nk;
  const int H = d.hidden_dim, D = d.rg_dim, Dk = d.kg_dim, TK = B * Nk, nh = d.num_heads;
  const size_t HH = (size_t)H * H;
  const Ws::H16& h = w.h;
  const bool virt = H == 256 && B <= 32;
  if (!virt) {
    BcastSeg s0{nullptr, w.dHm1, 2 * H, row_sample, inv_nr, 0, nullptr, T, h.dH1, h.H1};
    BcastSeg s1{nullptr, w.dHm2, 2 * H, nullptr, nullptr, Nk, nullptr, TK, h.dH2, h.H2};
    CK(launch_relu_bcast_bwd(s0, s1, 2 * H, drop.scale, st), "relu bcast bwd");
  }
  auto make_virt = [&](Gemm16Prob& p, const float* g_rows, bool rg_side) {
    p.flags |= GF_A_VIRT; p.virt_g = g_rows; p.ldg = 2 * H; p.aux_scale = drop.scale;
    if (rg_side) { p.row_sample = row_sample; p.inv_nr = inv_nr; p.uniform_n = 0; } else { p.row_sample = nullptr; p.inv_nr = nullptr; p.uniform_n = Nk; }
    if (p.flags & GF_A_KMAJOR) p.ldc16 = B;
  };
  GB16 g(drop, *x.opt, st);
  if (H == 256) {
    Gemm16Prob& p1 = g.nt(virt ? h.H1 : h.dH1, 2 * H, h.W1T, 2 * H, nullptr, w.dU, H, h.dU, H, T, H, 2 * H);
    set_bcast(p1, w.dcomb, 2 * H, row_sample, inv_nr, 0);
    p1.ln_mode = 2; p1.ln_gamma = P[CAMO_P_LN1_W]; p1.ln_stats = w.st1; p1.ln_x = w.U;
    p1.ln_dgamma = Gr[CAMO_P_LN1_W]; p1.ln_dbeta = Gr[CAMO_P_LN1_B];
    if (virt) make_virt(p1, w.dHm1, true);
    Gemm16Prob& p2 = g.nt(virt ? h.H2 : h.dH2, 2 * H, h.W2T, 2 * H, nullptr, w.dU2, H, h.dU2, H, TK, H, 2 * H);
    set_bcast(p2, w.dcomb + H, 2 * H, nullptr, nullptr, Nk);
    p2.ln_mode = 2; p2.ln_gamma = P[CAMO_P_LN2_W]; p2.ln_stats = w.st2; p2.ln_x = w.U2;
    p2.ln_dgamma = Gr[CAMO_P_LN2_W]; p2.ln_dbeta = Gr[CAMO_P_LN2_B];
    if (virt) make_virt(p2, w.dHm2, false);
  } else {
    set_bcast(g.nt(h.dH1, 2 * H, h.W1T, 2 * H, nullptr, w.dY, H, nullptr, 0, T, H, 2 * H), w.dcomb, 2 * H, row_sample, inv_nr, 0);
    set_bcast(g.nt(h.dH2, 2 * H, h.W2T, 2 * H, nullptr, w.dY2, H, nullptr, 0, TK, H, 2 * H), w.dcomb + H, 2 * H, nullptr, nullptr, Nk);
  }
  {
    Gemm16Prob& t1 = g.tn(virt ? h.H1 : h.dH1, 2 * H, h.Y, H, Gr[CAMO_P_F1_W0], H, Gr[CAMO_P_F1_B0], 2 * H, H, T);
    if (virt) make_virt(t1, w.dHm1, true);
    Gemm16Prob& t2 = g.tn(virt ? h.H2 : h.dH2, 2 * H, h.Y2, H, Gr[CAMO_P_F2_W0], H, Gr[CAMO_P_F2_B0], 2 * H, H, TK);
    if (virt) make_virt(t2, w.dHm2, false);
  }
  CK(g.run(), "ffn layer 0 bwd");
  if (H != 256) {
    LnBwdSeg s0{w.U, w.dY, w.st1, P[CAMO_P_LN1_W], w.dU, Gr[CAMO_P_LN1_W], Gr[CAMO_P_LN1_B], T, h.dU};
    LnBwdSeg s1{w.U2, w.dY2, w.st2, P[CAMO_P_LN2_W], w.dU2, Gr[CAMO_P_LN2_W], Gr[CAMO_P_LN2_B], TK, h.dU2};
    CK(launch_ln_bwd(s0, s1, H, st), "layernorm bwd");
  }
  g.nt(h.dU, H, h.Wo1T, H, nullptr, w.dO, H, nullptr, 0, T, H, H);
  g.nt(h.dU2, H, h.Wo2T, H, nullptr, w.dO2, H, nullptr, 0, TK, H, H);
  g.tn(h.dU, H, h.O, H, Gr[CAMO_P_A1_OUT_W], H, Gr[CAMO_P_A1_OUT_B], H, H, T);
  g.tn(h.dU2, H, h.O2, H, Gr[CAMO_P_A2_OUT_W], H, Gr[CAMO_P_A2_OUT_B], H, H, TK);
  CK(g.run(), "out-projection bwd");
  CK(launch_attn_bwd_pair(w.Q, w.KV, w.P, w.dO, w.Q2, w.KV2, w.P2, w.dO2, rg_offsets, Bf16Dst{h.dQKV, 3 * H},
                          Bf16Dst{h.dQKVkg + H, 3 * H}, Bf16Dst{h.dQKVkg, 3 * H}, Bf16Dst{h.dQKV + H, 3 * H}, w.O2, B, H, nh, Nk, drop, st),
     "attention bwd (both directions)");
  set_res(g.nt(h.dQKV, 3 * H, h.WcRgT, 3 * H, nullptr, nullptr, 0, h.dR, H, T, H, 3 * H), w.dU, H);
  set_res(g.nt(h.dQKVkg, 3 * H, h.WcKgT, 3 * H, nullptr, nullptr, 0, h.dG, H, TK, H, 3 * H), w.dU2, H);
  CK(g.run(), "in-projection bwd (input gradients)");
  g.tn(h.dQKV, 3 * H, h.R, H, Gr[CAMO_P_A1_IN_W], H, Gr[CAMO_P_A1_IN_B], H, H, T);
  g.tn(h.dQKV + H, 3 * H, h.R, H, Gr[CAMO_P_A2_IN_W] + HH, H, Gr[CAMO_P_A2_IN_B] + H, 2 * H, H, T);
  g.tn(h.dQKVkg, 3 * H, h.G, H, Gr[CAMO_P_A2_IN_W], H, Gr[CAMO_P_A2_IN_B], H, H, TK);
  g.tn(h.dQKVkg + H, 3 * H, h.G, H, Gr[CAMO_P_A1_IN_W] + HH, H, Gr[CAMO_P_A1_IN_B] + H, 2 * H, H, TK);
  g.tn(h.dR, H, h.X, D, Gr[CAMO_P_RG_PROJ_W], D, Gr[CAMO_P_RG_PROJ_B], H, D, T);
  g.tn(h.dG, H, h.KG, Dk, Gr[CAMO_P_KG_PROJ_W], Dk, Gr[CAMO_P_KG_PROJ_B], H, Dk, TK);
  CK(g.run(), "in-projection and input-projection weight gradients");
  return 0;
}

int tail17(Call& c, const Batch& x, float* outs, const FusedLoss* fl) {
  const camo_dims_t& d = *x.dims; const float* const* P = x.P; float* const* Gr = x.Gr; const Ws& w = x.w; hipStream_t st = x.st;
  const int H = 256, B = x.B;
  TailFusedArgs a; std::memset(&a, 0, sizeof(a));
  a.Ymean = w.Ymean; a.H1mean = w.H1mean; a.Y2mean = w.Y2mean; a.H2mean = w.H2mean;
  a.W13 = P[CAMO_P_F1_W3]; a.b13 = P[CAMO_P_F1_B3]; a.W23 = P[CAMO_P_F2_W3]; a.b23 = P[CAMO_P_F2_B3];
  a.Wfu0 = P[CAMO_P_FU_W0]; a.bfu0 = P[CAMO_P_FU_B0]; a.Wfu3 = P[CAMO_P_FU_W3]; a.bfu3 = P[CAMO_P_FU_B3];
  for (int x = 0; x < 4; ++x) {
    a.Wh0[x] = P[CAMO_P_HEADS + 4 * x]; a.bh0[x] = P[CAMO_P_HEADS + 4 * x + 1]; a.Wh3[x] = P[CAMO_P_HEADS + 4 * x + 2]; a.bh3[x] = P[CAMO_P_HEADS + 4 * x + 3];
  }
  if (fl) {
    a.gW13 = Gr[CAMO_P_F1_W3]; a.gb13 = Gr[CAMO_P_F1_B3]; a.gW23 = Gr[CAMO_P_F2_W3]; a.gb23 = Gr[CAMO_P_F2_B3];
    a.gWfu0 = Gr[CAMO_P_FU_W0]; a.gbfu0 = Gr[CAMO_P_FU_B0]; a.gWfu3 = Gr[CAMO_P_FU_W3]; a.gbfu3 = Gr[CAMO_P_FU_B3];
    for (int x = 0; x < 4; ++x) {
      a.gWh0[x] = Gr[CAMO_P_HEADS + 4 * x]; a.gbh0[x] = Gr[CAMO_P_HEADS + 4 * x + 1]; a.gWh3[x] = Gr[CAMO_P_HEADS + 4 * x + 2]; a.gbh3[x] = Gr[CAMO_P_HEADS + 4 * x + 3];
    }
    a.y = reinterpret_cast<const long long*>(fl->y); a.e = fl->e; a.s = fl->s; a.terms = fl->terms; a.pred = fl->pred;
    a.dcomb = w.dcomb; a.dHm1 = w.dHm1; a.dHm2 = w.dHm2;
  }
  a.outs = outs;
  a.F1sum = w.tailsum; a.hidsum = w.tailsum + (size_t)B * H; a.dF1sum = w.tailsum + (size_t)B * 3 * H;
  a.counters = reinterpret_cast<unsigned int*>(w.tailsum + (size_t)B * 4 * H);
  a.B = B; a.C = d.num_classes; a.mode = fl ? 1 : 0; a.drop = x.drop;
  a.stamps = g_dbg_stamps ? g_dbg_stamps + (size_t)4 * g_dbg_stamp_blocks * 8 : nullptr;
  a.debug_skip = c.tail_skip;
  if (fl) { a.comb_out = w.comb; a.F1_out = w.F1; a.fused_out = w.fused; a.dhid_out = w.dhid; a.dfused_out = w.dfused; a.dF1_out = w.dF1; }
  CK(launch_tail_fused(a, st), "per-sample tail (one launch)");
  c.tail_skip_taken = a.debug_skip != 0;
  if (x.plan.tail_wg == CAMO_TAIL_WG_LAUNCH) {
    GB g(x.drop, 0, st);
    add_tail_wg(x, g);
    CK(g.run(), "per-sample tail, weight gradients");
  }
  return 0;
}

int tail_planes_forward(const Batch& x, float* outs, const FusedLoss* fl) {
  const camo_dims_t& d = *x.dims; const float* const* P = x.P; const Ws& w = x.w;
  const bool train = x.plan.tail != CAMO_TAIL_PLANES;
  TailWideArgs ta; std::memset(&ta, 0, sizeof(ta));
  ta.Ymean = w.Ymean; ta.H1mean = w.H1mean; ta.Y2mean = w.Y2mean; ta.H2mean = w.H2mean;
  const us* const* tw = w.f.tailw;
  ta.T13h = tw[0]; ta.T13l = tw[1]; ta.T23h = tw[2]; ta.T23l = tw[3]; ta.Tfu0h = tw[4]; ta.Tfu0l = tw[5]; ta.Tfu3h = tw[6]; ta.Tfu3l = tw[7]; ta.Th0h = tw[8]; ta.Th0l = tw[9];
  ta.b13 = P[CAMO_P_F1_B3]; ta.b23 = P[CAMO_P_F2_B3]; ta.bfu0 = P[CAMO_P_FU_B0]; ta.bfu3 = P[CAMO_P_FU_B3];
  for (int x = 0; x < 4; ++x) { ta.bh0[x] = P[CAMO_P_HEADS + 4 * x + 1]; ta.Wh3[x] = P[CAMO_P_HEADS + 4 * x + 2]; ta.bh3[x] = P[CAMO_P_HEADS + 4 * x + 3]; }
  ta.outs = outs; ta.B = x.B; ta.C = d.num_classes; ta.drop = x.drop;
  if (train) { ta.comb_out = w.comb; ta.F1_out = w.F1; ta.fused_out = w.fused; ta.hid_out = w.hid; }
  CK(launch_tail_wide(ta, x.st), "per-sample tail (wide, one launch)");
  if (!train) return 0;
  return heads_forward(x, CAMO_P_HEADS, d.hidden_dim, outs, fl, true, x.plan.tail == CAMO_TAIL_PLANES_TRAIN);
}

int tail_planes_backward(const Batch& x) {
  const camo_dims_t& d = *x.dims; float* const* Gr = x.Gr; const Ws& w = x.w;
  const int H = d.hidden_dim, B = x.B;
  TailWideBwdArgs ta; std::memset(&ta, 0, sizeof(ta));
  const us* const* tw = w.f.tailw;
  ta.dhid = w.dhid; ta.F1 = w.F1;
  ta.Th0h = tw[10]; ta.Th0l = tw[11]; ta.Tfu3h = tw[12]; ta.Tfu3l = tw[13]; ta.Tfu0h = tw[14]; ta.Tfu0l = tw[15];
  ta.T13h = tw[16]; ta.T13l = tw[17]; ta.T23h = tw[18]; ta.T23l = tw[19];
  ta.dfused = w.dfused; ta.dF1 = w.dF1; ta.dcomb = w.dcomb; ta.dHm1 = w.dHm1; ta.dHm2 = w.dHm2;
  ta.B = B; ta.scale = x.drop.scale;
  CK(launch_tail_wide_bwd(ta, x.st), "per-sample tail, input gradients (wide, one launch)");
  const int Fh = H / 2, C = d.num_classes, Wd = 2 * C + 2, nout[4] = {C, C, 1, 1}, coff[4] = {0, C, 2 * C, 2 * C + 1};
  float* const* hg = Gr + CAMO_P_HEADS;
  GB gt = tail_gemms(x);
  for (int h = 0; h < 4; ++h) gt.tn(w.dlog + coff[h], Wd, w.hid + h * Fh, 4 * Fh, hg[4 * h + 2], Fh, hg[4 * h + 3], nout[h], Fh, B);
  add_tail_wg(x, gt);
  CK(gt.run(), "per-sample tail, weight gradients");
  return 0;
}

int backward_nodes17(Call& c, const Batch& x) {
  const camo_plan_t& pl = x.plan; const float* const* P = x.P; float* const* Gr = x.Gr; const Ws& w = x.w; const DropCfg& drop = x.drop; hipStream_t st = x.st;
  const int32_t* rg_offsets = x.rg_offsets; const Desc& bd = x.bd;
  const int H = 256, D = 128, B = x.B, T = x.T, Nk = x.Nk, TK = B * Nk;
  const size_t HH = (size_t)H * H;
  const Ws::F17& f = w.f;
  Bwd1Args a1; std::memset(&a1, 0, sizeof(a1));
  a1.s[0] = Bwd1Stream{f.W1T, f.Wo1T, f.mask1, f.XH16, f.rstd1, P[CAMO_P_LN1_W], w.dHm1, 2 * H, w.dcomb, 2 * H, f.dH16, f.dU16,
                       Gr[CAMO_P_LN1_W], Gr[CAMO_P_LN1_B]};
  a1.s[1] = Bwd1Stream{f.W2T, f.Wo2T, f.mask2, f.XH2_16, f.rstd2, P[CAMO_P_LN2_W], w.dHm2, 2 * H, w.dcomb + H, 2 * H, f.dH2_16, f.dU2_16,
                       Gr[CAMO_P_LN2_W], Gr[CAMO_P_LN2_B]};
  a1.Q16 = f.Q16; a1.KV16 = f.KV16; a1.dQKV16 = f.dQKV16; a1.dKV = w.dKV;
  a1.O2_16 = f.O2_16; a1.dO2_16 = f.dO2_16; a1.delta2 = f.delta2;
  a1.off = rg_offsets; a1.tile_off = bd.tile_off; a1.tile_desc = bd.tile_desc; a1.inv_nr = bd.inv_nr; a1.row_sample = bd.row_sample;
  a1.B = B; a1.Nk = Nk; a1.rows_rg = T; a1.rg_tiles_max = T / 32 + B; a1.qscale = 1.0f / sqrtf(32.0f); a1.drop = drop;
  a1.stamps = g_dbg_stamps ? g_dbg_stamps + (size_t)2 * g_dbg_stamp_blocks * 8 : nullptr;
  a1.nzero = c.nzero_bwd1; a1.exp = x.opt->exp;
  for (int i = 0; i < c.nzero_bwd1; ++i) { a1.zero_ptr[i] = c.zero_bwd1_ptr[i]; a1.zero_bytes[i] = c.zero_bwd1_bytes[i]; }
  if (pl.tail_wg == CAMO_TAIL_WG_BWD1) {
    TailWgArgs& t = a1.twg;
    for_tail_wg(x, [&](const float* dy, int ld_dy, const float* xin, int ld_x, float* dW, float* db, int rows, int cols) {
      t.p[t.n++] = TailWgProd{dy, xin, dW, db, ld_dy, ld_x, rows, cols, 0};
    });
    t.B = B;
  }
  if (pl.bwd1 == CAMO_BWD1_64) CK(launch_wide2_bwd1(a1, x.opt->fused_variant, st), "fused backward, first half (64-row half-blocks)");
  else                         CK(launch_fused_bwd1(a1, x.opt->fused_variant, st), "fused backward, first half");
  if (pl.tail_event == CAMO_EVENT_AFTER_BWD1) CK(record_tail_event(c, st), "tail event");
  Bwd2Args a2; std::memset(&a2, 0, sizeof(a2));
  a2.Q2_16 = f.Q2_16; a2.dO2_16 = f.dO2_16; a2.lse2 = f.lse2; a2.delta2 = f.delta2; a2.KV2_16 = f.KV2_16; a2.dQKV16 = f.dQKV16;
  a2.dU16 = f.dU16; a2.WcRgT = f.WcRgT; a2.dR16 = f.dR16; a2.dQ2acc = w.dQ2acc; a2.dKV = w.dKV;
  a2.dU2_16 = f.dU2_16; a2.WcKgT = f.WcKgT; a2.dQKVkg16 = f.dQKVkg16; a2.dG16 = f.dG16; a2.dGpart = f.dGpart;
  a2.tickets = w.tickets + B; a2.off = rg_offsets; a2.tile_off = bd.tile_off; a2.tile_desc = bd.tile_desc;
  a2.B = B; a2.Nk = Nk; a2.rows_rg = T; a2.rg_tiles_max = T / 32 + B; a2.qscale = a1.qscale; a2.drop = drop;
  a2.stamps = g_dbg_stamps ? g_dbg_stamps + (size_t)3 * g_dbg_stamp_blocks * 8 : nullptr;
  const bool param_space = pl.param_space != 0;
  a2.param_space = param_space ? 1 : 0;
  a2.split_finish = pl.bwd2 != CAMO_BWD2_ROWS32 ? 1 : 0;
  if (pl.bwd2 == CAMO_BWD2_64) CK(launch_wide2_bwd2(a2, st), "fused backward, second half (64-row blocks)");
  else CK(launch_fused_bwd2(a2, x.opt->fused_variant, st), "fused backward, second half");
  if (!param_space) {
    GB16 g(drop, *x.opt, st);
    g.tn(f.dH16, 2 * H, f.Y16, H, Gr[CAMO_P_F1_W0], H, Gr[CAMO_P_F1_B0], 2 * H, H, T);
    g.tn(f.dU16, H, f.O16, H, Gr[CAMO_P_A1_OUT_W], H, Gr[CAMO_P_A1_OUT_B], H, H, T);
    g.tn(f.dQKV16, 3 * H, f.R16, H, Gr[CAMO_P_A1_IN_W], H, Gr[CAMO_P_A1_IN_B], H, H, T);
    g.tn(f.dQKV16 + H, 3 * H, f.R16, H, Gr[CAMO_P_A2_IN_W] + HH, H, Gr[CAMO_P_A2_IN_B] + H, 2 * H, H, T);
    g.tn(f.dR16, H, f.X16, D, Gr[CAMO_P_RG_PROJ_W], D, Gr[CAMO_P_RG_PROJ_B], H, D, T);
    g.tn(f.dH2_16, 2 * H, f.Y2_16, H, Gr[CAMO_P_F2_W0], H, Gr[CAMO_P_F2_B0], 2 * H, H, TK);
    g.tn(f.dU2_16, H, f.O2_16, H, Gr[CAMO_P_A2_OUT_W], H, Gr[CAMO_P_A2_OUT_B], H, H, TK);
    g.tn(f.dQKVkg16, 3 * H, f.G16, H, Gr[CAMO_P_A2_IN_W], H, Gr[CAMO_P_A2_IN_B], H, H, TK);
    g.tn(f.dQKVkg16 + H, 3 * H, f.G16, H, Gr[CAMO_P_A1_IN_W] + HH, H, Gr[CAMO_P_A1_IN_B] + H, 2 * H, H, TK);
    g.tn(f.dG16, H, f.KG16, D, Gr[CAMO_P_KG_PROJ_W], D, Gr[CAMO_P_KG_PROJ_B], H, D, TK);
    CK(g.run(), "node-level weight gradients");
    return 0;
  }
  float* const Mrg = w.parM; float* const Mkg = Mrg + (size_t)3 * H * D;
  float* const dbrg = Mkg + (size_t)3 * H * D; float* const dbkg = dbrg + 3 * H;
  GB16 g(drop, *x.opt, st);
  g.tn(f.dH16, 2 * H, f.Y16, H, Gr[CAMO_P_F1_W0], H, Gr[CAMO_P_F1_B0], 2 * H, H, T);
  g.tn(f.dU16, H, f.O16, H, Gr[CAMO_P_A1_OUT_W], H, Gr[CAMO_P_A1_OUT_B], H, H, T);
  g.tn(f.dQKV16, 3 * H, f.X16, D, Mrg, D, dbrg, H, D, T).bias_grad2 = Gr[CAMO_P_A1_IN_B];
  g.tn(f.dQKV16 + H, 3 * H, f.X16, D, Mrg + (size_t)H * D, D, dbrg + H, 2 * H, D, T).bias_grad2 = Gr[CAMO_P_A2_IN_B] + H;
  g.tn(f.dU16, H, f.X16, D, Gr[CAMO_P_RG_PROJ_W], D, Gr[CAMO_P_RG_PROJ_B], H, D, T);
  g.tn(f.dH2_16, 2 * H, f.Y2_16, H, Gr[CAMO_P_F2_W0], H, Gr[CAMO_P_F2_B0], 2 * H, H, TK);
  g.tn(f.dU2_16, H, f.O2_16, H, Gr[CAMO_P_A2_OUT_W], H, Gr[CAMO_P_A2_OUT_B], H, H, TK);
  g.tn(f.dQKVkg16, 3 * H, f.KG16, D, Mkg, D, dbkg, H, D, TK).bias_grad2 = Gr[CAMO_P_A2_IN_B];
  g.tn(f.dQKVkg16 + H, 3 * H, f.KG16, D, Mkg + (size_t)H * D, D, dbkg + H, 2 * H, D, TK).bias_grad2 = Gr[CAMO_P_A1_IN_B] + H;
  g.tn(f.dU2_16, H, f.KG16, D, Gr[CAMO_P_KG_PROJ_W], D, Gr[CAMO_P_KG_PROJ_B], H, D, TK);
  CK(g.run(), "node-level weight gradients");
  {
    const UnfoldStream urg{Mrg, dbrg, P[CAMO_P_A1_IN_W], P[CAMO_P_A2_IN_W] + HH, P[CAMO_P_RG_PROJ_W], P[CAMO_P_RG_PROJ_B], Gr[CAMO_P_A1_IN_W],
                           Gr[CAMO_P_A2_IN_W] + HH, Gr[CAMO_P_RG_PROJ_W], Gr[CAMO_P_RG_PROJ_B]};
    const UnfoldStream ukg{Mkg, dbkg, P[CAMO_P_A2_IN_W], P[CAMO_P_A1_IN_W] + HH, P[CAMO_P_KG_PROJ_W], P[CAMO_P_KG_PROJ_B], Gr[CAMO_P_A2_IN_W],
                           Gr[CAMO_P_A1_IN_W] + HH, Gr[CAMO_P_KG_PROJ_W], Gr[CAMO_P_KG_PROJ_B]};
    CK(launch_unfold(urg, ukg, st), "projection / in-projection weight gradients (parameter space)");
  }
  return 0;
}

int forward_late(const Batch& x, float* outs, const FusedLoss* fl) {
  const camo_dims_t& d = *x.dims; const float* const* P = x.P; const Ws& w = x.w; hipStream_t st = x.st;
  const int H = d.hidden_dim, D = d.rg_dim, Dk = d.kg_dim, B = x.B, Nk = x.Nk, F = H / 2, Dc = D + Dk;
  CK((int)hipMemsetAsync(w.zero_base, 0, w.zero_bytes, st), "memset zero block");
  GB gt = tail_gemms(x);
  SegMean sm[2] = {{x.rg, D, D, x.rg_offsets, 0, w.comb, Dc}, {x.kg, Dk, Dk, nullptr, Nk, w.comb + D, Dc}};
  CK(launch_seg_mean(sm, 2, B, x.max_nr > Nk ? x.max_nr : Nk, st), "late means");
  set_drop(gt.nt(w.comb, Dc, P[CAMO_PL_W0], Dc, P[CAMO_PL_B0], w.F1, H, B, H, Dc, GF_RELU), SITE_LATE0);
  CK(gt.run(), "late fc0");
  set_drop(gt.nt(w.F1, H, P[CAMO_PL_W3], H, P[CAMO_PL_B3], w.a2, F, B, F, H, GF_RELU), SITE_LATE0 + 1);
  CK(gt.run(), "late fc3");
  gt.nt(w.a2, F, P[CAMO_PL_W6], F, P[CAMO_PL_B6], w.fused, F, B, F, F);
  CK(gt.run(), "late fc6");
  return heads_forward(x, CAMO_PL_HEADS, F, outs, fl);
}

int backward_late(const Batch& x, const float* outs, const float* d_outs, int pre_activation, bool heads_out_done) {
  const camo_dims_t& d = *x.dims; const float* const* P = x.P; float* const* Gr = x.Gr; const Ws& w = x.w; const DropCfg& drop = x.drop;
  const int H = d.hidden_dim, B = x.B, F = H / 2, Dc = d.rg_dim + d.kg_dim;
  if (int e = heads_backward(x, CAMO_PL_HEADS, F, outs, d_outs, pre_activation, heads_out_done)) return e;
  GB gt = tail_gemms(x);
  set_relu_bwd(gt.nn(w.dfused, F, P[CAMO_PL_W6], F, w.da2, F, B, F, F), w.a2, F, drop.scale);
  gt.tn(w.dfused, F, w.a2, F, Gr[CAMO_PL_W6], F, Gr[CAMO_PL_B6], F, F, B);
  CK(gt.run(), "late fc6 bwd");
  set_relu_bwd(gt.nn(w.da2, F, P[CAMO_PL_W3], H, w.dF1, H, B, H, F), w.F1, H, drop.scale);
  gt.tn(w.da2, F, w.F1, H, Gr[CAMO_PL_W3], H, Gr[CAMO_PL_B3], F, H, B);
  CK(gt.run(), "late fc3 bwd");
  gt.tn(w.dF1, H, w.comb, Dc, Gr[CAMO_PL_W0], Dc, Gr[CAMO_PL_B0], H, Dc, B);
  CK(gt.run(), "late fc0 bwd");
  return 0;
}

int forward_nodes_general(const Batch& x, float* attn_rg2kg, float* attn_kg2rg) {
  const camo_dims_t& d = *x.dims; const float* const* P = x.P; const Ws& w = x.w; const DropCfg& drop = x.drop; hipStream_t st = x.st;
  const float* rg = x.rg; const float* kg = x.kg; const int32_t* rg_offsets = x.rg_offsets;
  const int H = d.hidden_dim, D = d.rg_dim, Dk = d.kg_dim, B = x.B, T = x.T, Nk = x.Nk, TK = B * Nk, nh = d.num_heads, max_nr = x.max_nr;
  const size_t HH2 = (size_t)H * H;
  CK((int)hipMemsetAsync(w.zero_base, 0, w.zero_bytes, st), "memset zero block");
  GB g(drop, x.precision, st);
  const float* R = rg; const float* G = kg;
  if (P[CAMO_P_KG_PROJ_W]) { g.nt(kg, Dk, P[CAMO_P_KG_PROJ_W], Dk, P[CAMO_P_KG_PROJ_B], w.G, H, TK, H, Dk); G = w.G; }
  if (P[CAMO_P_RG_PROJ_W]) { g.nt(rg, D, P[CAMO_P_RG_PROJ_W], D, P[CAMO_P_RG_PROJ_B], w.R, H, T, H, D); R = w.R; }
  CK(g.run(), "input projections");
  g.nt(R, H, P[CAMO_P_A1_IN_W], H, P[CAMO_P_A1_IN_B], w.Q, H, T, H, H);
  g.nt(R, H, P[CAMO_P_A2_IN_W] + HH2, H, P[CAMO_P_A2_IN_B] + H, w.KV2, 2 * H, T, 2 * H, H);
  g.nt(G, H, P[CAMO_P_A1_IN_W] + HH2, H, P[CAMO_P_A1_IN_B] + H, w.KV, 2 * H, TK, 2 * H, H);
  g.nt(G, H, P[CAMO_P_A2_IN_W], H, P[CAMO_P_A2_IN_B], w.Q2, H, TK, H, H);
  CK(g.run(), "attention in-projections");
  CK(launch_attn_rg2kg_fwd(w.Q, w.KV, rg_offsets, w.P, w.O, attn_rg2kg, B, T, max_nr, H, nh, Nk, drop, st), "attn rg2kg fwd");
  CK(launch_attn_kg2rg_fwd(w.Q2, w.KV2, rg_offsets, w.P2, w.O2, B, max_nr, H, nh, Nk, drop, st), "attn kg2rg fwd");
  if (attn_kg2rg) CK(launch_attn_avg(w.P2, attn_kg2rg, T, nh, Nk, drop, st), "attn avg");
  set_res(g.nt(w.O, H, P[CAMO_P_A1_OUT_W], H, P[CAMO_P_A1_OUT_B], w.U, H, T, H, H), R, H);
  set_res(g.nt(w.O2, H, P[CAMO_P_A2_OUT_W], H, P[CAMO_P_A2_OUT_B], w.U2, H, TK, H, H), G, H);
  CK(g.run(), "attention out-projections");
  {
    LnSeg s0{w.U, w.Y, w.st1, P[CAMO_P_LN1_W], P[CAMO_P_LN1_B], T};
    LnSeg s1{w.U2, w.Y2, w.st2, P[CAMO_P_LN2_W], P[CAMO_P_LN2_B], TK};
    CK(launch_ln_fwd(s0, s1, H, st), "layernorm fwd");
  }
  set_drop(g.nt(w.Y, H, P[CAMO_P_F1_W0], H, P[CAMO_P_F1_B0], w.H1, 2 * H, T, 2 * H, H, GF_RELU), SITE_FFN_RG);
  set_drop(g.nt(w.Y2, H, P[CAMO_P_F2_W0], H, P[CAMO_P_F2_B0], w.H2, 2 * H, TK, 2 * H, H, GF_RELU), SITE_FFN_KG);
  CK(g.run(), "ffn layer 0");
  SegMean sm[4] = {{w.Y, H, H, rg_offsets, 0, w.Ymean, H}, {w.H1, 2 * H, 2 * H, rg_offsets, 0, w.H1mean, 2 * H},
                   {w.Y2, H, H, nullptr, Nk, w.Y2mean, H}, {w.H2, 2 * H, 2 * H, nullptr, Nk, w.H2mean, 2 * H}};
  CK(launch_seg_mean(sm, 4, B, max_nr > Nk ? max_nr : Nk, st), "pool");
  return 0;
}

int forward_tail_gemms(const Batch& x, float* outs, const FusedLoss* fl) {
  const float* const* P = x.P; const Ws& w = x.w;
  const int H = x.dims->hidden_dim, B = x.B;
  GB gt = tail_gemms(x);
  set_res(gt.nt(w.H1mean, 2 * H, P[CAMO_P_F1_W3], 2 * H, P[CAMO_P_F1_B3], w.comb, 2 * H, B, H, 2 * H), w.Ymean, H);
  set_res(gt.nt(w.H2mean, 2 * H, P[CAMO_P_F2_W3], 2 * H, P[CAMO_P_F2_B3], w.comb + H, 2 * H, B, H, 2 * H), w.Y2mean, H);
  CK(gt.run(), "ffn layer 3 on pooled rows");
  set_drop(gt.nt(w.comb, 2 * H, P[CAMO_P_FU_W0], 2 * H, P[CAMO_P_FU_B0], w.F1, H, B, H, 2 * H, GF_RELU), SITE_FUSE);
  CK(gt.run(), "fusion layer 0");
  gt.nt(w.F1, H, P[CAMO_P_FU_W3], H, P[CAMO_P_FU_B3], w.fused, H, B, H, H);
  CK(gt.run(), "fusion layer 3");
  return heads_forward(x, CAMO_P_HEADS, H, outs, fl);
}

int forward_impl(Call& c, const Batch& x, float* outs, float* attn_rg2kg, float* attn_kg2rg, const FusedLoss* fl) {
  const camo_dims_t& d = *x.dims;
  if (x.plan.nodes == CAMO_NODES_LATE) return forward_late(x, outs, fl);
  if (!x.P[CAMO_P_RG_PROJ_W] && d.rg_dim != d.hidden_dim) return fail(CAMO_E_ARG, "rg_proj weight missing but rg_dim != hidden_dim");
  if (!x.P[CAMO_P_KG_PROJ_W] && d.kg_dim != d.hidden_dim) return fail(CAMO_E_ARG, "kg_proj weight missing but kg_dim != hidden_dim");
  if (x.plan.nodes == CAMO_NODES_FUSED) {
    if (int e = forward_nodes17(c, x, attn_rg2kg, attn_kg2rg)) return e;
    if (x.plan.tail >= CAMO_TAIL_PLANES) return tail_planes_forward(x, outs, fl);
    if (x.plan.tail == CAMO_TAIL_ONE_LAUNCH) return tail17(c, x, outs, fl);
  } else if (x.plan.nodes == CAMO_NODES_BF16) {
    if (int e = forward_nodes16(x, attn_rg2kg, attn_kg2rg)) return e;
  } else {
    if (int e = forward_nodes_general(x, attn_rg2kg, attn_kg2rg)) return e;
  }
  return forward_tail_gemms(x, outs, fl);
}

int backward_tail_gemms(const Batch& x, const float* outs, const float* d_outs, int pre_activation, bool heads_out_done) {
  const float* const* P = x.P; float* const* Gr = x.Gr; const Ws& w = x.w; const DropCfg& drop = x.drop;
  const int H = x.dims->hidden_dim, B = x.B;
  if (int e = heads_backward(x, CAMO_P_HEADS, H, outs, d_outs, pre_activation, heads_out_done)) return e;
  GB gt = tail_gemms(x);
  set_relu_bwd(gt.nn(w.dfused, H, P[CAMO_P_FU_W3], H, w.dF1, H, B, H, H), w.F1, H, drop.scale);
  gt.tn(w.dfused, H, w.F1, H, Gr[CAMO_P_FU_W3], H, Gr[CAMO_P_FU_B3], H, H, B);
  CK(gt.run(), "fusion layer 3 bwd");
  gt.nn(w.dF1, H, P[CAMO_P_FU_W0], 2 * H, w.dcomb, 2 * H, B, 2 * H, H);
  gt.tn(w.dF1, H, w.comb, 2 * H, Gr[CAMO_P_FU_W0], 2 * H, Gr[CAMO_P_FU_B0], H, 2 * H, B);
  CK(gt.run(), "fusion layer 0 bwd");
  gt.nn(w.dcomb, 2 * H, P[CAMO_P_F1_W3], 2 * H, w.dHm1, 2 * H, B, 2 * H, H);
  gt.nn(w.dcomb + H, 2 * H, P[CAMO_P_F2_W3], 2 * H, w.dHm2, 2 * H, B, 2 * H, H);
  gt.tn(w.dcomb, 2 * H, w.H1mean, 2 * H, Gr[CAMO_P_F1_W3], 2 * H, Gr[CAMO_P_F1_B3], H, 2 * H, B);
  gt.tn(w.dcomb + H, 2 * H, w.H2mean, 2 * H, Gr[CAMO_P_F2_W3], 2 * H, Gr[CAMO_P_F2_B3], H, 2 * H, B);
  CK(gt.run(), "ffn layer 3 bwd (pooled)");
  return 0;
}

int backward_nodes_general(const Batch& x) {
  const camo_dims_t& d = *x.dims; const float* const* P = x.P; float* const* Gr = x.Gr; const Ws& w = x.w; const DropCfg& drop = x.drop; hipStream_t st = x.st;
  const float* rg = x.rg; const float* kg = x.kg; const int32_t* rg_offsets = x.rg_offsets; const int32_t* row_sample = x.bd.row_sample; const float* inv_nr = x.bd.inv_nr;
  const int H = d.hidden_dim, D = d.rg_dim, Dk = d.kg_dim, B = x.B, T = x.T, Nk = x.Nk, TK = B * Nk, nh = d.num_heads, max_nr = x.max_nr;
  const bool has_rgp = P[CAMO_P_RG_PROJ_W] != nullptr, has_kgp = P[CAMO_P_KG_PROJ_W] != nullptr;
  const float* R = has_rgp ? w.R : rg;
  const float* G = has_kgp ? w.G : kg;
  GB g(drop, x.precision, st);
  {
    BcastSeg s0{w.H1, w.dHm1, 2 * H, row_sample, inv_nr, 0, w.dH1, T};
    BcastSeg s1{w.H2, w.dHm2, 2 * H, nullptr, nullptr, Nk, w.dH2, TK};
    CK(launch_relu_bcast_bwd(s0, s1, 2 * H, drop.scale, st), "relu bcast bwd");
  }
  set_bcast(g.nn(w.dH1, 2 * H, P[CAMO_P_F1_W0], H, w.dY, H, T, H, 2 * H), w.dcomb, 2 * H, row_sample, inv_nr, 0);
  set_bcast(g.nn(w.dH2, 2 * H, P[CAMO_P_F2_W0], H, w.dY2, H, TK, H, 2 * H), w.dcomb + H, 2 * H, nullptr, nullptr, Nk);
  g.tn(w.dH1, 2 * H, w.Y, H, Gr[CAMO_P_F1_W0], H, Gr[CAMO_P_F1_B0], 2 * H, H, T);
  g.tn(w.dH2, 2 * H, w.Y2, H, Gr[CAMO_P_F2_W0], H, Gr[CAMO_P_F2_B0], 2 * H, H, TK);
  CK(g.run(), "ffn layer 0 bwd");
  {
    LnBwdSeg s0{w.U, w.dY, w.st1, P[CAMO_P_LN1_W], w.dU, Gr[CAMO_P_LN1_W], Gr[CAMO_P_LN1_B], T};
// ... 360 lines not shown
```

### camouflage_multimodal_amd/csrc/misc.h

```cpp
#pragma once
#include "common.h"

struct LnSeg { const float* U; float* Y; float* stats; const float* gamma; const float* beta; int rows;
               unsigned short* Y16;
               float* mean; const int* row_sample; const float* inv_n; int uniform_n; };
struct LnBwdSeg { const float* U; const float* dY; const float* stats; const float* gamma; float* dU;
                  float* dgamma; float* dbeta; int rows;
                  unsigned short* dU16;  };
struct SegMean { const float* X; int ld, C; const int* offs; int uniform_n; float* out; int ldo; };
struct BcastSeg { const float* act; const float* v; int ldv; const int* row_sample; const float* inv_n;
                  int uniform_n; float* dst; int rows;
                  unsigned short* dst16;
                  const unsigned short* act16;  };

enum : int { PREP_ZERO = 0, PREP_CAST = 1, PREP_CAST_T = 2 };
struct PrepJob { const float* src; void* dst; size_t n; int type, rows, cols, ld_dst, col_off, blk_begin; };
#define PREP_MAXJ 48
struct PrepBatch { PrepJob j[PREP_MAXJ]; int n; };
int launch_prep(PrepBatch& pb, hipStream_t stream);

int ln_supported(int H);
int launch_rowmap(const int* offs, int* row_sample, float* inv_nr, int* tile_off, int4* tile_desc, int B, int ntile_max, int max_nr, hipStream_t stream);

struct UnfoldStream { const float *M, *db, *Wq, *Wkv, *Wp, *bp; float *Gq, *Gkv, *Gp, *Gbp; };
int launch_unfold(const UnfoldStream& rg, const UnfoldStream& kg, hipStream_t stream);
int launch_gather_batch(const float* rg_all, const long long* sample_off, const float* kg_all, const long long* y_all, const float* e_all, const float* s_all,
                        const long long* idx, int B, int T, int D, int KG, float* rg_out, float* kg_out, int* off_out, long long* y_out, float* e_out,
                        float* s_out, float noise_std, unsigned long long seed, hipStream_t stream);
int launch_ln_fwd(const LnSeg& s0, const LnSeg& s1, int H, hipStream_t stream);
int launch_ln_bwd(const LnBwdSeg& s0, const LnBwdSeg& s1, int H, hipStream_t stream);
int launch_seg_mean(const SegMean* segs, int nseg, int B, int max_rows, hipStream_t stream);
int launch_relu_bcast_bwd(const BcastSeg& s0, const BcastSeg& s1, int C, float scale, hipStream_t stream);
int launch_head_out_grad(const float* outs, const float* d_outs, float* d_logits, int B, int W, hipStream_t stream);
int launch_loss(const float* outs, const long long* y, const float* e, const float* s, int B, int C,
                float* terms, float* d_outs, float* d_pre, int* pred, hipStream_t stream);
#define HEADS_MAXW 130
struct HeadsOut { const float* W[4]; const float* b[4]; float* gW[4]; float* gb[4]; };
int heads_loss_ok(int B, int C);
int launch_heads_loss(const float* hid, const HeadsOut& hp, const long long* y, const float* e, const float* s, int B, int C,
                      int Fh, float scale, float* outs, float* terms, int* pred, float* dhid, hipStream_t stream, float* dlog = nullptr);
int launch_sumsq(const float* g, size_t n, float* out, hipStream_t stream);
int launch_clip_adamw(float* p, float* g, float* m, float* v, size_t n, float* sumsq, float max_norm,
                      float lr, float b1, float b2, float eps, float wd, int step, int zero_grads, hipStream_t stream);

struct TailFusedArgs {
  const float *Ymean, *H1mean, *Y2mean, *H2mean;
  const float *W13, *b13, *W23, *b23, *Wfu0, *bfu0, *Wfu3, *bfu3; const float* Wh0[4]; const float* bh0[4]; const float* Wh3[4]; const float* bh3[4];
  float *gW13, *gb13, *gW23, *gb23, *gWfu0, *gbfu0, *gWfu3, *gbfu3; float* gWh0[4]; float* gbh0[4]; float* gWh3[4]; float* gbh3[4];
  const long long* y; const float* e; const float* s;
  float* outs; float* terms; int* pred;
  float *F1sum, *hidsum, *dF1sum; unsigned int* counters;
  float *dcomb, *dHm1, *dHm2;
  float *comb_out, *F1_out, *fused_out, *dhid_out, *dfused_out, *dF1_out;
  int B, C, mode; DropCfg drop;
  unsigned long long* stamps;
  int debug_skip;
};
int tail_fused_ok(int B, int C);
int tail_fused_ok(int B, int C, int cus);
int device_cus();
int launch_tail_fused(const TailFusedArgs& a, hipStream_t stream);
int tail_timeouts(unsigned int* out);
int launch_tail_poison_to_grads(float* g, hipStream_t stream);

struct AdamShadowBlock {
  size_t off;
  int rows, cols;
  unsigned short* plain; int pN, pn0;
  unsigned short* trans; int tK, tk0;
  int tile_begin;
};
#define ADAM_SHADOW_MAXB 12
#define ADAM_SHADOW_MAXR 16
struct AdamShadowArgs {
  AdamShadowBlock blk[ADAM_SHADOW_MAXB]; int nblk;
  size_t range_begin[ADAM_SHADOW_MAXR], range_len[ADAM_SHADOW_MAXR]; int nrange;
  int tiles, nbig;
};
int launch_clip_adamw_shadows(float* p, float* g, float* m, float* v, float* sumsq, float max_norm, float lr, float b1, float b2,
                              float eps, float wd, int step, int zero_grads, AdamShadowArgs& a, hipStream_t stream);
```

### camouflage_multimodal_amd/csrc/misc.hip

```cpp
#include "misc.h"
#include "gemm.h"


namespace {

__global__ __launch_bounds__(256) void batchdesc_kernel(const int* __restrict__ offs, int* __restrict__ row_sample, float* __restrict__ inv_nr,
                                                        int* __restrict__ tile_off, int4* __restrict__ tile_desc, int B, int ntile_max) {
  __shared__ int part[256];
  __shared__ int total_s;
  const int t = threadIdx.x, per = (B + 255) / 256, b0 = min(B, t * per), b1 = min(B, b0 + per);
  const int T = offs[B];
  int s = 0;
  for (int b = b0; b < b1; ++b) s += (offs[b + 1] - offs[b] + 31) >> 5;
  {
    const int lane = t & 63, w = t >> 6;
    int incl = s;
#pragma unroll
    for (int o = 1; o < 64; o <<= 1) { const int v = __shfl_up(incl, o, 64); if (lane >= o) incl += v; }
    if (lane == 63) part[w] = incl;
    __syncthreads();
    const int w0 = part[0], w1 = part[1], w2 = part[2], w3 = part[3];
    __syncthreads();
    const int base = w == 0 ? 0 : (w == 1 ? w0 : (w == 2 ? w0 + w1 : w0 + w1 + w2));
    part[t] = base + incl - s;
    if (t == 0) total_s = w0 + w1 + w2 + w3;
  }
  __syncthreads();
  const int ntiles = total_s;
  if (blockIdx.x == 0) {
    int acc = part[t];
    for (int b = b0; b < b1; ++b) { tile_off[b] = acc; acc += (offs[b + 1] - offs[b] + 31) >> 5; }
    if (t == 0) tile_off[B] = ntiles;
    for (int b = t; b < B; b += 256) inv_nr[b] = 1.0f / (float)(offs[b + 1] - offs[b]);
  }
  const int r = blockIdx.x * 256 + t;
  if (r < T) {
    int lo = 0, hi = B - 1;
    while (lo < hi) { const int mid = (lo + hi + 1) >> 1; if (offs[mid] <= r) lo = mid; else hi = mid - 1; }
    row_sample[r] = lo;
  }
  if (t < 8) {
    const int tl = blockIdx.x * 8 + t;
    if (tl < ntile_max) {
      int4 d = make_int4(-1, 0, 0, 0);
      if (tl < ntiles) {
        int c = 0, hi = (B + per - 1) / per - 1;
        while (c < hi) { const int mid = (c + hi + 1) >> 1; if (part[mid] <= tl) c = mid; else hi = mid - 1; }
        int b = min(B - 1, c * per), acc = part[c];
        while (b + 1 < B) { const int n = (offs[b + 1] - offs[b] + 31) >> 5; if (acc + n > tl) break; acc += n; ++b; }
        const int r0 = offs[b] + 32 * (tl - acc), nr = offs[b + 1] - offs[b];
        d = make_int4(b, r0, min(32, offs[b + 1] - r0), __float_as_int(1.0f / (float)nr));
      }
      tile_desc[tl] = d;
    }
  }
}

constexpr int GATHER_ROWS = 64;
constexpr int GATHER_MAXB = 4096;
__device__ __forceinline__ float2 gather_noise(uint32_t a, uint32_t b, float std) {
  const float u1 = ((float)(a >> 8) + 1.0f) * (1.0f / 16777216.0f), u2 = (float)(b >> 8) * (1.0f / 16777216.0f);
  const float r = std * sqrtf(-2.0f * __logf(u1));
  float sn, cs;
  __sincosf(6.28318530718f * u2, &sn, &cs);
  return make_float2(r * cs, r * sn);
}
__global__ __launch_bounds__(256) void gather_batch_kernel(const float* __restrict__ rg_all, const long long* __restrict__ sample_off, const float* __restrict__ kg_all,
                                                          const long long* __restrict__ y_all, const float* __restrict__ e_all, const float* __restrict__ s_all,
                                                          const long long* __restrict__ idx, int B, int T, int D, int KG, int row_blocks,
                                                          float* __restrict__ rg_out, float* __restrict__ kg_out, int* __restrict__ off_out,
                                                          long long* __restrict__ y_out, float* __restrict__ e_out, float* __restrict__ s_out,
                                                          float noise_std, uint32_t seed_lo, uint32_t seed_hi) {
  __shared__ int off[GATHER_MAXB + 1];
  __shared__ int part[256];
  const int t = threadIdx.x;
  if ((int)blockIdx.x >= row_blocks) {
    const int b = (int)blockIdx.x - row_blocks;
    const long long src = idx[b];
    const bool aug = noise_std > 0.f && (fmix32((uint32_t)b * 0x9E3779B9u + seed_lo) ^ seed_hi) >> 31;
    for (int c = t; c < KG / 2; c += 256) {
      float2 v = *reinterpret_cast<const float2*>(kg_all + src * KG + 2 * c);
      if (aug) { const float2 n = gather_noise(fmix32(0x51ED270Bu + (uint32_t)(b * KG + 2 * c) + seed_lo) ^ seed_hi, fmix32(0x2545F491u + (uint32_t)(b * KG + 2 * c) + seed_hi) ^ seed_lo, noise_std); v.x += n.x; v.y += n.y; }
      *reinterpret_cast<float2*>(kg_out + (size_t)b * KG + 2 * c) = v;
    }
    if (t == 0) { y_out[b] = y_all[src]; e_out[b] = e_all[src]; s_out[b] = s_all[src]; }
    return;
  }
  const int per = (B + 255) / 256, b0 = min(B, t * per), b1 = min(B, b0 + per);
  int sum = 0;
  for (int b = b0; b < b1; ++b) { const long long i = idx[b]; sum += (int)(sample_off[i + 1] - sample_off[i]); }
  part[t] = sum;
  __syncthreads();
  if (t == 0) { int acc = 0; for (int i = 0; i < 256; ++i) { const int v = part[i]; part[i] = acc; acc += v; } off[B] = acc; }
  __syncthreads();
  {
    int acc = part[t];
    for (int b = b0; b < b1; ++b) { off[b] = acc; const long long i = idx[b]; acc += (int)(sample_off[i + 1] - sample_off[i]); }
  }
  __syncthreads();
  if (blockIdx.x == 0) for (int b = t; b <= B; b += 256) off_out[b] = off[b];
  const int lanes = D / 4, rpp = 256 / lanes;
  const int lr = t / lanes, lc = t % lanes;
  if (lr >= rpp) return;
  for (int r0 = 0; r0 < GATHER_ROWS; r0 += rpp) {
    const int r = (int)blockIdx.x * GATHER_ROWS + r0 + lr;
    if (r >= T || r >= off[B]) break;
    int lo = 0, hi = B - 1;
    while (lo < hi) { const int mid = (lo + hi + 1) >> 1; if (off[mid] <= r) lo = mid; else hi = mid - 1; }
    const long long srow = sample_off[idx[lo]] + (r - off[lo]);
    float4 v = *reinterpret_cast<const float4*>(rg_all + srow * D + 4 * lc);
    if (noise_std > 0.f && ((fmix32((uint32_t)lo * 0x9E3779B9u + seed_lo) ^ seed_hi) >> 31)) {
      const uint32_t e0 = (uint32_t)r * (uint32_t)D + 4u * (uint32_t)lc;
      const float2 n0 = gather_noise(fmix32(e0 + seed_lo) ^ seed_hi, fmix32(e0 + 0x68E31DA4u + seed_hi) ^ seed_lo, noise_std);
      const float2 n1 = gather_noise(fmix32(e0 + 2u + seed_lo) ^ seed_hi, fmix32(e0 + 2u + 0x68E31DA4u + seed_hi) ^ seed_lo, noise_std);
      v.x += n0.x; v.y += n0.y; v.z += n1.x; v.w += n1.y;
    }
    *reinterpret_cast<float4*>(rg_out + (size_t)r * D + 4 * lc) = v;
  }
}

constexpr int LNF_R = 4;
constexpr int LNF_W = 4;
template <int HPL>
__global__ __launch_bounds__(64 * LNF_W) void ln_fwd_kernel(LnSeg s0, LnSeg s1, int H, int nb0) {
  __shared__ float part[LNF_W][64 * HPL];
  __shared__ int scur[LNF_W];
  const bool first = (int)blockIdx.x < nb0;
  const LnSeg& S = first ? s0 : s1;
  const int wave = threadIdx.x >> 6, lane = threadIdx.x & 63;
  const int rbase = ((first ? blockIdx.x : blockIdx.x - nb0) * LNF_W + wave) * LNF_R;
  const bool pool = S.mean != nullptr;
  float gam[HPL], bet[HPL], cs[HPL];
#pragma unroll
  for (int i = 0; i < HPL; ++i) {
    const int c = lane + 64 * i;
    gam[i] = c < H ? S.gamma[c] : 0.f; bet[i] = c < H ? S.beta[c] : 0.f; cs[i] = 0.f;
  }
  auto flush = [&](int sm) {
    const float inv = S.row_sample ? S.inv_n[sm] : 1.0f / (float)S.uniform_n;
#pragma unroll
    for (int i = 0; i < HPL; ++i) {
      const int c = lane + 64 * i;
      if (c < H) atomicAdd(S.mean + (size_t)sm * H + c, cs[i] * inv);
      cs[i] = 0.f;
    }
  };
  int cur = -1;
  float x[LNF_R][HPL];
#pragma unroll
  for (int r = 0; r < LNF_R; ++r) {
    const int row = min(rbase + r, S.rows - 1);
    const float* u = S.U + (size_t)row * H;
#pragma unroll
    for (int i = 0; i < HPL; ++i) { const int c = lane + 64 * i; x[r][i] = c < H ? u[c] : 0.f; }
// ... 300 lines not shown
    for (int k = 0; k < C; ++k) z += ex(oi[k] - mx);
    const float iz = rc(z);
    terms4[1] = -(oi[yb] - mx - lg(z));
    for (int k = 0; k < C; ++k) put(C + k, (FAST ? ex(oi[k] - mx) * iz : expf(oi[k] - mx) / z) - (k == yb ? 1.0f : 0.0f));
  }
  {
    const float x = o[2 * C], t = eb;
    terms4[2] = 0.5f * (fmaxf(x, 0.f) - x * t + (FAST ? __logf(1.0f + __expf(-fabsf(x))) : log1pf(expf(-fabsf(x)))));
    put(2 * C, 0.5f * ((FAST ? rc(1.0f + ex(-x)) : 1.0f / (1.0f + expf(-x))) - t));
  }
  {
    const float x = o[2 * C + 1], t = sb;
    terms4[3] = 0.3f * (x - t) * (x - t);
    put(2 * C + 1, 0.6f * (x - t));
  }
}

__global__ void loss_kernel(const float* __restrict__ outs, const long long* __restrict__ y,
                            const float* __restrict__ e, const float* __restrict__ s, int B, int C,
                            float* __restrict__ terms, float* __restrict__ d_outs, float* __restrict__ d_pre,
                            int* __restrict__ pred) {
  const int b = blockIdx.x * blockDim.x + threadIdx.x;
  if (b >= B) return;
  const int W = 2 * C + 2;
  loss_sample(outs + (size_t)b * W, (int)y[b], e[b], s[b], C, terms + 4 * b, d_outs ? d_outs + (size_t)b * W : nullptr,
              d_pre ? d_pre + (size_t)b * W : nullptr, pred ? pred + b : nullptr);
}

template <bool ACC>
__global__ __launch_bounds__(256) void heads_loss_kernel(const float* __restrict__ hid, HeadsOut hp,
                                                         const long long* __restrict__ y, const float* __restrict__ e,
                                                         const float* __restrict__ s, int B, int S, int C, int Fh, float scale,
                                                         float* __restrict__ outs, float* __restrict__ terms,
                                                         int* __restrict__ pred, float* __restrict__ dhid, float* __restrict__ dlog) {
  __shared__ float so[HEADS_MAXW], sd[HEADS_MAXW];
  const int x = threadIdx.x >> 6, lane = threadIdx.x & 63;
  const int W = 2 * C + 2, nout = x < 2 ? C : 1, coff = x == 0 ? 0 : (x == 1 ? C : (x == 2 ? 2 * C : 2 * C + 1));
  const float* Wx = x == 0 ? hp.W[0] : (x == 1 ? hp.W[1] : (x == 2 ? hp.W[2] : hp.W[3]));
  const float* bx = x == 0 ? hp.b[0] : (x == 1 ? hp.b[1] : (x == 2 ? hp.b[2] : hp.b[3]));
  float* gWx = x == 0 ? hp.gW[0] : (x == 1 ? hp.gW[1] : (x == 2 ? hp.gW[2] : hp.gW[3]));
  float* gbx = x == 0 ? hp.gb[0] : (x == 1 ? hp.gb[1] : (x == 2 ? hp.gb[2] : hp.gb[3]));
  const float bias0 = bx[0];
  constexpr int HC = 4;
  constexpr int AO = ACC ? 8 : 1;
  float gacc[AO][HC], gbacc = 0.f;
#pragma unroll
  for (int o = 0; o < AO; ++o)
#pragma unroll
    for (int i = 0; i < HC; ++i) gacc[o][i] = 0.f;
  for (int si = 0; si < S; ++si) {
    const int b = blockIdx.x * S + si;
    if (b >= B) break;
    const float* h = hid + (size_t)b * 4 * Fh + x * Fh;
    const int yb = (int)y[b]; const float eb = e[b], sb = s[b];
    float hv[HC];
#pragma unroll
    for (int i = 0; i < HC; ++i) { const int c = lane + 64 * i; hv[i] = c < Fh ? h[c] : 0.f; }
    for (int o = 0; o < nout; ++o) {
      float acc = 0.f;
#pragma unroll
      for (int i = 0; i < HC; ++i) { const int c = lane + 64 * i; if (c < Fh) acc = fmaf(hv[i], Wx[(size_t)o * Fh + c], acc); }
      for (int c = lane + 64 * HC; c < Fh; c += 64) acc = fmaf(h[c], Wx[(size_t)o * Fh + c], acc);
      acc = wave_sum(acc);
      if (lane == 0) {
        float v = acc + (o == 0 ? bias0 : bx[o]);
        if (x == 3) v = 1.0f / (1.0f + __expf(-v));
        so[coff + o] = v;
        outs[(size_t)b * W + coff + o] = v;
      }
    }
    __syncthreads();
    if (threadIdx.x == 0) loss_sample(so, yb, eb, sb, C, terms + 4 * b, nullptr, sd, pred ? pred + b : nullptr);
    __syncthreads();
    if (dlog && threadIdx.x < W) dlog[(size_t)b * W + threadIdx.x] = sd[threadIdx.x];
    auto back = [&](int c, float hval, int i) {
      float dh = 0.f;
      if (dlog) {
        for (int o = 0; o < nout; ++o) dh = fmaf(sd[coff + o], Wx[(size_t)o * Fh + c], dh);
      } else if constexpr (ACC) {
#pragma unroll
        for (int o = 0; o < 8; ++o) {
          if (o < nout) {
            const float d = sd[coff + o];
            dh = fmaf(d, Wx[(size_t)o * Fh + c], dh);
            if (i >= 0) gacc[o][i >= 0 ? i : 0] = fmaf(d, hval, gacc[o][i >= 0 ? i : 0]); else atomicAdd(gWx + (size_t)o * Fh + c, d * hval);
          }
        }
      } else {
        for (int o = 0; o < nout; ++o) {
          const float d = sd[coff + o];
          dh = fmaf(d, Wx[(size_t)o * Fh + c], dh);
          atomicAdd(gWx + (size_t)o * Fh + c, d * hval);
        }
      }
      dhid[(size_t)b * 4 * Fh + x * Fh + c] = hval > 0.f ? dh * scale : 0.f;
    };
#pragma unroll
    for (int i = 0; i < HC; ++i) { const int c = lane + 64 * i; if (c < Fh) back(c, hv[i], i); }
    for (int c = lane + 64 * HC; c < Fh; c += 64) back(c, h[c], -1);
    if (!dlog && lane < nout) gbacc += sd[coff + lane];
    __syncthreads();
  }
  if (dlog) return;
  if constexpr (ACC) {
#pragma unroll
    for (int o = 0; o < 8; ++o)
#pragma unroll
      for (int i = 0; i < HC; ++i) { const int c = lane + 64 * i; if (o < nout && c < Fh) atomicAdd(gWx + (size_t)o * Fh + c, gacc[o][i]); }
  }
  if (lane < nout) atomicAdd(gbx + lane, gbacc);
}


constexpr int TG = 64;
__device__ unsigned int g_tail_timeouts = 0;
__device__ __forceinline__ void tstamp(unsigned long long* stamps, int k) {
  if (stamps && threadIdx.x == 0) stamps[(size_t)blockIdx.x * 32 + k] = __builtin_amdgcn_s_memrealtime();
}
__device__ unsigned int g_tail_poison = 0;
__device__ __forceinline__ void tail_arrive_wait(unsigned int* counter, unsigned int* timeout, int* lds_flag, bool skip_arrival = false) {
  asm volatile("s_waitcnt vmcnt(0)" ::: "memory");
  __syncthreads();
  if (threadIdx.x == 0) {
    if (!skip_arrival) __hip_atomic_fetch_add(counter, 1u, __ATOMIC_RELAXED, __HIP_MEMORY_SCOPE_AGENT);
    unsigned int spins = 0;
    while (__hip_atomic_load(counter, __ATOMIC_RELAXED, __HIP_MEMORY_SCOPE_AGENT) < (unsigned int)TG) {
      __builtin_amdgcn_s_sleep(1);
      if (++spins > (1u << 21)) {
        __hip_atomic_store(timeout, 1u, __ATOMIC_RELAXED, __HIP_MEMORY_SCOPE_AGENT);
        atomicAdd(&g_tail_timeouts, 1u);
        __hip_atomic_store(&g_tail_poison, 1u, __ATOMIC_RELAXED, __HIP_MEMORY_SCOPE_AGENT);
        *lds_flag = 1;
        break;
      }
    }
    __builtin_amdgcn_fence(__ATOMIC_ACQUIRE, "agent");
    asm volatile("s_waitcnt vmcnt(0)" ::: "memory");
  }
  __syncthreads();
}

constexpr int TF_MAXB = 16;
constexpr int TF_MAXGROUPS = 3;
constexpr int TF_MAXW = 18;
constexpr int TF_LDS_FLOATS = 2 * TF_MAXB * 512 + 2 * TF_MAXB * 256 + 2048 + 2048 + 3 * 128 + 64 + 64 + 2 * TF_MAXB * TF_MAXW + TF_MAXW * 129 + 2 +
                             8 * 512 + 4 * 256;

__device__ __forceinline__ void wave_sum4(float (&acc)[4]) {
#pragma unroll
  for (int j = 0; j < 4; ++j) acc[j] = wave_sum_lane63(acc[j]);
}

constexpr int TF_THREADS = 1024;

__global__ __launch_bounds__(TF_THREADS) void tail_fused_kernel(const TailFusedArgs a) {
  extern __shared__ __attribute__((aligned(16))) float sm[];
  __shared__ int s_timed_out;
  if (threadIdx.x == 0) s_timed_out = 0;
  const bool wg = a.mode != 0;
  const int tid = threadIdx.x, lane = tid & 63, g = blockIdx.x & (TG - 1), sg = blockIdx.x >> 6, C = a.C, Wd = 2 * C + 2;
  const bool multi = gridDim.x > TG;
  const int sb = TF_MAXB * sg, B = min(TF_MAXB, a.B - sb);
  const float* const gYmean = a.Ymean + (size_t)sb * 256; const float* const gY2mean = a.Y2mean + (size_t)sb * 256;
  const float* const gH1mean = a.H1mean + (size_t)sb * 512; const float* const gH2mean = a.H2mean + (size_t)sb * 512;
  float* const gF1sum = a.F1sum + (size_t)sb * 256; float* const ghidsum = a.hidsum + (size_t)sb * 512; float* const gdF1sum = a.dF1sum + (size_t)sb * 256;
  float* const gouts = a.outs + (size_t)sb * Wd;
  const bool md = a.mode != 0;
  const long long* const gy = md ? a.y + sb : nullptr; const float* const ge = md ? a.e + sb : nullptr; const float* const gs = md ? a.s + sb : nullptr;
  float* const gterms = md ? a.terms + 4 * sb : nullptr; int* const gpred = md && a.pred ? a.pred + sb : nullptr;
  float* const gdcomb = md ? a.dcomb + (size_t)sb * 512 : nullptr;
  float* const gdHm1 = md ? a.dHm1 + (size_t)sb * 512 : nullptr; float* const gdHm2 = md ? a.dHm2 + (size_t)sb * 512 : nullptr;
  float* const gcomb_out = wg ? a.comb_out + (size_t)sb * 512 : nullptr; float* const gF1_out = wg ? a.F1_out + (size_t)sb * 256 : nullptr;
  float* const gfused_out = wg ? a.fused_out + (size_t)sb * 256 : nullptr; float* const gdhid_out = wg ? a.dhid_out + (size_t)sb * 512 : nullptr;
  float* const gdfused_out = wg ? a.dfused_out + (size_t)sb * 256 : nullptr; float* const gdF1_out = wg ? a.dF1_out + (size_t)sb * 256 : nullptr;
  unsigned int* const cnt = a.counters + 4 * sg;
  unsigned int* const gaveup = a.counters + 3;
  auto put = [&](float* p, float v) { if (multi) atomicAdd(p, v); else *p = v; };
  const int q = __builtin_amdgcn_readfirstlane(tid >> 8), t = tid & 255, wv = __builtin_amdgcn_readfirstlane((tid >> 6) & 3);
  const int b0 = 4 * q, B4 = (B + 3) & ~3;
  const bool active = b0 < B;
  float* R1 = sm;
  float* R2 = R1 + TF_MAXB * 512;
  float* F1 = R2 + TF_MAXB * 512;
  float* DF = F1 + TF_MAXB * 256;
  float* wA = DF + TF_MAXB * 256;
  float* wB = wA + 2048;
  float* combS = wB + 2048; float* dcombS = combS + 128; float* ymS = dcombS + 128; float* fusedS = ymS + 128; float* dfusedS = fusedS + 64;
  float* outsS = dfusedS + 64; float* dpre = outsS + TF_MAXB * TF_MAXW;
  float* w3s = dpre + TF_MAXB * TF_MAXW;
  float* W3L = w3s + ((TF_MAXW * 129 + 3) & ~3);
  float* WfL = W3L + 8 * 512;
  const bool kgs = g >= 32;
  const int c0 = 8 * (g & 31), ccol = (kgs ? 256 : 0) + c0;
  const float* Hmean = kgs ? gH2mean : gH1mean; const float* Ymean = kgs ? gY2mean : gYmean;
  const float* W3s = kgs ? a.W23 : a.W13; const float* b3s = kgs ? a.b23 : a.b13;
  float* dHm = kgs ? gdHm2 : gdHm1;
  const bool dodrop = a.drop.p > 0.f;
  const float dscale = a.drop.scale;
  auto headW0 = [&](int x) { return x == 0 ? a.Wh0[0] : (x == 1 ? a.Wh0[1] : (x == 2 ? a.Wh0[2] : a.Wh0[3])); };
  auto headB0 = [&](int x) { return x == 0 ? a.bh0[0] : (x == 1 ? a.bh0[1] : (x == 2 ? a.bh0[2] : a.bh0[3])); };
  auto headW3 = [&](int x) { return x == 0 ? a.Wh3[0] : (x == 1 ? a.Wh3[1] : (x == 2 ? a.Wh3[2] : a.Wh3[3])); };
  auto headB3 = [&](int x) { return x == 0 ? a.bh3[0] : (x == 1 ? a.bh3[1] : (x == 2 ? a.bh3[2] : a.bh3[3])); };
  auto gheadW3 = [&](int x) { return x == 0 ? a.gWh3[0] : (x == 1 ? a.gWh3[1] : (x == 2 ? a.gWh3[2] : a.gWh3[3])); };
  auto gheadB3 = [&](int x) { return x == 0 ? a.gbh3[0] : (x == 1 ? a.gbh3[1] : (x == 2 ? a.gbh3[2] : a.gbh3[3])); };
  auto head_of = [&](int o, int& x, int& oo) {
    if (o < C) { x = 0; oo = o; } else if (o < 2 * C) { x = 1; oo = o - C; } else if (o == 2 * C) { x = 2; oo = 0; } else { x = 3; oo = 0; }
  };
  const float4 z4 = make_float4(0.f, 0.f, 0.f, 0.f);
  tstamp(a.stamps, 0);
  const float4 w3l = *reinterpret_cast<const float4*>(W3s + (size_t)(c0 + (tid >> 7)) * 512 + 4 * (tid & 127));
  float4 hv[2];
#pragma unroll
  for (int it = 0; it < 2; ++it) { const int i = tid + TF_THREADS * it; hv[it] = i < B * 128 ? reinterpret_cast<const float4*>(Hmean)[i] : z4; }
  const float ymv = tid < B * 8 ? Ymean[(tid >> 3) * 256 + c0 + (tid & 7)] + b3s[c0 + (tid & 7)] : 0.f;
  const float4 wfl = tid < 256 ? *reinterpret_cast<const float4*>(a.Wfu3 + (size_t)(4 * g + (tid >> 6)) * 256 + 4 * (tid & 63)) : z4;
  float4 wb0 = z4, wb1 = z4, wav = z4;
  if (q == 0) {
    const float4* p = reinterpret_cast<const float4*>(a.Wfu0 + (size_t)t * 512 + ccol);
    wb0 = p[0]; wb1 = p[1];
  } else if (q < 3) {
    const int m = tid - 256;
    wav = *reinterpret_cast<const float4*>(headW0(m >> 7) + (size_t)(m & 127) * 256 + 4 * g);
  }
  float w3v[3];
#pragma unroll
  for (int it = 0; it < 3; ++it) {
    const int p = tid + TF_THREADS * it;
    w3v[it] = 0.f;
    if (p < Wd * 129) {
      const int o = p / 129, k = p - 129 * o;
      int x, oo; head_of(o, x, oo);
      w3v[it] = k < 128 ? headW3(x)[(size_t)oo * 128 + k] : headB3(x)[oo];
    }
  }
  const float bias2 = g == 0 ? a.bfu0[t] : 0.f;
  const float bias3 = a.bfu3[4 * g + wv];
  const float bias4a = g == 0 ? headB0(t >> 7)[t & 127] : 0.f, bias4b = g == 0 ? headB0(2 + (t >> 7))[t & 127] : 0.f;
  const int hx = (8 * g) >> 7, hmm0 = (8 * g) & 127, hnout = hx < 2 ? C : 1, hcoff = hx == 0 ? 0 : (hx == 1 ? C : (hx == 2 ? 2 * C : 2 * C + 1));
  float* dW3h = gheadW3(hx) + (size_t)(tid >> 3) * 128 + hmm0 + (tid & 7);
  float oW3h = 0.f, ob3h = 0.f;
  if (a.mode && !multi) {
    if (tid < hnout * 8) oW3h = *dW3h;
    if (g == 0 && tid >= 128 && tid < 128 + Wd) { int xx, oo; head_of(tid - 128, xx, oo); ob3h = gheadB3(xx)[oo]; }
  }
#pragma unroll
  for (int it = 0; it < 2; ++it) { const int i = tid + TF_THREADS * it; if (i < B4 * 128) reinterpret_cast<float4*>(R1)[i] = hv[it]; }
  reinterpret_cast<float4*>(W3L)[tid] = w3l;
  if (tid < 128) ymS[tid] = ymv;
  __syncthreads();
  tstamp(a.stamps, 1);
  if (active) {
#pragma unroll
    for (int cc = 0; cc < 2; ++cc) {
      float acc[4] = {0.f, 0.f, 0.f, 0.f};
#pragma unroll
      for (int i = 0; i < 8; ++i)
#pragma unroll
        for (int j = 0; j < 4; ++j) acc[j] = fmaf(W3L[(2 * wv + cc) * 512 + lane + 64 * i], R1[(b0 + j) * 512 + lane + 64 * i], acc[j]);
      wave_sum4(acc);
      if (lane == 63) {
#pragma unroll
        for (int j = 0; j < 4; ++j) {
          const float cv = acc[j] + ymS[(b0 + j) * 8 + 2 * wv + cc];
          combS[(b0 + j) * 8 + 2 * wv + cc] = cv;
          if (wg && b0 + j < B) gcomb_out[(size_t)(b0 + j) * 512 + ccol + 2 * wv + cc] = cv;
        }
      }
    }
  }
  if (q == 0) { reinterpret_cast<float4*>(wB)[2 * t] = wb0; reinterpret_cast<float4*>(wB)[2 * t + 1] = wb1; }
  else if (q < 3) reinterpret_cast<float4*>(wA)[tid - 256] = wav;
#pragma unroll
  for (int it = 0; it < 3; ++it) { const int p = tid + TF_THREADS * it; if (p < Wd * 129) w3s[p] = w3v[it]; }
  if (tid < 256) reinterpret_cast<float4*>(WfL)[tid] = wfl;
  __syncthreads();
  tstamp(a.stamps, 2);
  if (active) {
    float w8[8];
#pragma unroll
    for (int c = 0; c < 8; ++c) w8[c] = wB[t * 8 + c];
#pragma unroll
    for (int j = 0; j < 4; ++j) {
      const float4 ca = reinterpret_cast<const float4*>(combS)[(b0 + j) * 2], cb = reinterpret_cast<const float4*>(combS)[(b0 + j) * 2 + 1];
      const float acc = bias2 + w8[0] * ca.x + w8[1] * ca.y + w8[2] * ca.z + w8[3] * ca.w + w8[4] * cb.x + w8[5] * cb.y + w8[6] * cb.z + w8[7] * cb.w;
      if (b0 + j < B) atomicAdd(gF1sum + (b0 + j) * 256 + t, acc);
    }
  }
  tstamp(a.stamps, 3);
  tail_arrive_wait(cnt + 0, gaveup, &s_timed_out, a.debug_skip == (int)blockIdx.x + 1);
  tstamp(a.stamps, 4);
  {
    const float4 v4 = tid < B * 64 ? reinterpret_cast<const float4*>(gF1sum)[tid] : z4;
    if (tid < B4 * 64) {
      float v[4] = {fmaxf(v4.x, 0.f), fmaxf(v4.y, 0.f), fmaxf(v4.z, 0.f), fmaxf(v4.w, 0.f)};
      if (dodrop) {
#pragma unroll
        for (int e = 0; e < 4; ++e) v[e] *= drop_mult(a.drop, SITE_FUSE, (uint32_t)(sb * 256 + 4 * tid + e));
      }
      reinterpret_cast<float4*>(F1)[tid] = make_float4(v[0], v[1], v[2], v[3]);
      if (wg && g == 0 && tid < B * 64) reinterpret_cast<float4*>(gF1_out)[tid] = make_float4(v[0], v[1], v[2], v[3]);
    }
  }
  __syncthreads();
  tstamp(a.stamps, 5);
  if (active) {
    float acc[4] = {0.f, 0.f, 0.f, 0.f};
#pragma unroll
    for (int i = 0; i < 4; ++i)
#pragma unroll
      for (int j = 0; j < 4; ++j) acc[j] = fmaf(WfL[wv * 256 + lane + 64 * i], F1[(b0 + j) * 256 + lane + 64 * i], acc[j]);
    wave_sum4(acc);
    if (lane == 63) {
#pragma unroll
      for (int j = 0; j < 4; ++j) {
// ... 387 lines not shown
    const int sl = blk / 8, tc = (blk & 7) >> 1, tk = blk & 1, c0 = 64 * tc, kk0 = 64 * tk, r0 = 128 * sl;
    const float* W = r0 < UF_H ? S.Wq + (size_t)r0 * UF_H : S.Wkv + (size_t)(r0 - UF_H) * UF_H;
    const float* Mr = S.M + (size_t)r0 * UF_D;
    const int r = t >> 4, c4 = 4 * (t & 15);
    float4 av8[8], bv8[8];
#pragma unroll
    for (int q = 0; q < 8; ++q) {
      av8[q] = *reinterpret_cast<const float4*>(W + (size_t)(16 * q + r) * UF_H + c0 + c4);
      bv8[q] = *reinterpret_cast<const float4*>(Mr + (size_t)(16 * q + r) * UF_D + kk0 + c4);
    }
#pragma unroll
    for (int q = 0; q < 8; ++q) {
      const float4 a = av8[q], b = bv8[q];
      __syncthreads();
      *reinterpret_cast<float4*>(&As[r][c4]) = a;
      *reinterpret_cast<float4*>(&Bs[r][c4]) = b;
      __syncthreads();
      mac();
    }
#pragma unroll
    for (int i = 0; i < 4; ++i)
#pragma unroll
      for (int j = 0; j < 4; ++j) atomicAdd(S.Gp + (size_t)(c0 + 4 * ty + i) * UF_D + kk0 + 4 * tx + j, acc[i][j]);
  }
}

}

int launch_unfold(const UnfoldStream& rg, const UnfoldStream& kg, hipStream_t stream) {
  const int prof = gemm_prof_open(stream, 2.0 * 2.0 * 2.0 * 768.0 * 256.0 * 128.0, PROF_GEMM);
  hipLaunchKernelGGL(unfold_kernel, dim3(204), dim3(256), 0, stream, rg, kg);
  gemm_prof_close(prof, stream);
  return (int)hipGetLastError();
}

int launch_gather_batch(const float* rg_all, const long long* sample_off, const float* kg_all, const long long* y_all, const float* e_all, const float* s_all,
                        const long long* idx, int B, int T, int D, int KG, float* rg_out, float* kg_out, int* off_out, long long* y_out, float* e_out,
                        float* s_out, float noise_std, unsigned long long seed, hipStream_t stream) {
  if (B < 1 || B > GATHER_MAXB || T < B || D < 4 || (D & 3) || D > 1024 || KG < 2 || (KG & 1)) return (int)hipErrorInvalidValue;
  const int row_blocks = (T + GATHER_ROWS - 1) / GATHER_ROWS;
  hipLaunchKernelGGL(gather_batch_kernel, dim3(row_blocks + B), dim3(256), 0, stream, rg_all, sample_off, kg_all, y_all, e_all, s_all, idx, B, T, D, KG, row_blocks,
                     rg_out, kg_out, off_out, y_out, e_out, s_out, noise_std, (uint32_t)(seed & 0xFFFFFFFFull), (uint32_t)(seed >> 32));
  return (int)hipGetLastError();
}
int launch_prep(PrepBatch& pb, hipStream_t stream) {
  int total = 0;
  for (int i = 0; i < pb.n; ++i) {
    PrepJob& J = pb.j[i];
    J.blk_begin = total;
    if (J.type == PREP_ZERO) total += (int)(((J.n >> 4) + 1023) / 1024);
    else if (J.type == PREP_CAST) total += (int)(((J.n >> 2) + 1023) / 1024);
    else total += ((J.rows + 63) / 64) * ((J.cols + 63) / 64);
  }
  if (total == 0) return 0;
  hipLaunchKernelGGL(prep_kernel, dim3(total), dim3(256), 0, stream, pb);
  return (int)hipGetLastError();
}

int launch_rowmap(const int* offs, int* row_sample, float* inv_nr, int* tile_off, int4* tile_desc, int B, int ntile_max, int max_nr, hipStream_t stream) {
  (void)max_nr;
  const int T_upper = 32 * ntile_max;
  const int blocks = (T_upper + 255) / 256;
  hipLaunchKernelGGL(batchdesc_kernel, dim3(blocks), dim3(256), 0, stream, offs, row_sample, inv_nr, tile_off, tile_desc, B, ntile_max);
  return (int)hipGetLastError();
}

int ln_supported(int H) { return H >= 1 && H <= 1024; }

int launch_ln_fwd(const LnSeg& s0, const LnSeg& s1, int H, hipStream_t stream) {
  const int rpb = LNF_W * LNF_R;
  const int nb0 = (s0.rows + rpb - 1) / rpb, nb1 = (s1.rows + rpb - 1) / rpb;
  if (nb0 + nb1 == 0) return 0;
  if (H <= 256) hipLaunchKernelGGL(ln_fwd_kernel<4>, dim3(nb0 + nb1), dim3(64 * LNF_W), 0, stream, s0, s1, H, nb0);
  else          hipLaunchKernelGGL(ln_fwd_kernel<16>, dim3(nb0 + nb1), dim3(64 * LNF_W), 0, stream, s0, s1, H, nb0);
  return (int)hipGetLastError();
}

int launch_ln_bwd(const LnBwdSeg& s0_, const LnBwdSeg& s1_, int H, hipStream_t stream) {
  constexpr int rpb = 32;
  const LnBwdSeg& s0 = s0_; const LnBwdSeg& s1 = s1_;
  auto nblk = [](int rows) { int b = (rows + rpb - 1) / rpb; return rows == 0 ? 0 : (b > 2048 ? 2048 : (b < 1 ? 1 : b)); };
  const int nb0 = nblk(s0.rows), nb1 = nblk(s1.rows);
  if (nb0 + nb1 == 0) return 0;
  const bool vec = (H & 3) == 0;
  if (H <= 256) {
    if (vec) hipLaunchKernelGGL((ln_bwd_kernel<4, true>), dim3(nb0 + nb1), dim3(64 * LNB_W), 0, stream, s0, s1, H, nb0);
    else     hipLaunchKernelGGL((ln_bwd_kernel<4, false>), dim3(nb0 + nb1), dim3(64 * LNB_W), 0, stream, s0, s1, H, nb0);
  } else {
    if (vec) hipLaunchKernelGGL((ln_bwd_kernel<16, true>), dim3(nb0 + nb1), dim3(64 * LNB_W), 0, stream, s0, s1, H, nb0);
    else     hipLaunchKernelGGL((ln_bwd_kernel<16, false>), dim3(nb0 + nb1), dim3(64 * LNB_W), 0, stream, s0, s1, H, nb0);
  }
  return (int)hipGetLastError();
}

int launch_seg_mean(const SegMean* segs, int nseg, int B, int max_rows, hipStream_t stream) {
  SegMean z{}; SegMean s[4] = {z, z, z, z};
  for (int i = 0; i < nseg && i < 4; ++i) s[i] = segs[i];
  const int rpb = 32;
  bool vec = true;
  for (int i = 0; i < nseg && i < 4; ++i)
    vec = vec && (s[i].C & 3) == 0 && (s[i].ld & 3) == 0 && (reinterpret_cast<uintptr_t>(s[i].X) & 15) == 0;
  const dim3 grid((max_rows + rpb - 1) / rpb, B, nseg);
  if (vec) hipLaunchKernelGGL(seg_mean_kernel<true>, grid, dim3(256), 0, stream, s[0], s[1], s[2], s[3], rpb);
  else     hipLaunchKernelGGL(seg_mean_kernel<false>, grid, dim3(256), 0, stream, s[0], s[1], s[2], s[3], rpb);
  return (int)hipGetLastError();
}

int launch_relu_bcast_bwd(const BcastSeg& s0, const BcastSeg& s1, int C, float scale, hipStream_t stream) {
  const long n0 = (long)s0.rows * C, n1 = (long)s1.rows * C;
  if (n0 + n1 == 0) return 0;
  auto al16 = [](const void* p) { return (reinterpret_cast<uintptr_t>(p) & 15) == 0; };
  const bool vec = (C & 3) == 0 && (s0.ldv & 3) == 0 && (s1.ldv & 3) == 0 && al16(s0.act) && al16(s0.v) && al16(s0.dst) &&
                   al16(s1.act) && al16(s1.v) && al16(s1.dst) && al16(s0.dst16) && al16(s1.dst16) && al16(s0.act16) && al16(s1.act16);
  if (vec) hipLaunchKernelGGL(relu_bcast_bwd_kernel<4>, dim3((unsigned)(((n0 + n1) / 4 + 255) / 256)), dim3(256), 0, stream, s0, s1, C, n0, scale);
  else     hipLaunchKernelGGL(relu_bcast_bwd_kernel<1>, dim3((unsigned)((n0 + n1 + 255) / 256)), dim3(256), 0, stream, s0, s1, C, n0, scale);
  return (int)hipGetLastError();
}

int launch_head_out_grad(const float* outs, const float* d_outs, float* d_logits, int B, int W, hipStream_t stream) {
  hipLaunchKernelGGL(head_out_grad_kernel, dim3((B * W + 255) / 256), dim3(256), 0, stream, outs, d_outs, d_logits, B, W);
  return (int)hipGetLastError();
}

int launch_loss(const float* outs, const long long* y, const float* e, const float* s, int B, int C,
                float* terms, float* d_outs, float* d_pre, int* pred, hipStream_t stream) {
  hipLaunchKernelGGL(loss_kernel, dim3((B + 63) / 64), dim3(64), 0, stream, outs, y, e, s, B, C, terms, d_outs, d_pre, pred);
  return (int)hipGetLastError();
}

int heads_loss_ok(int B, int C) { return B >= 1 && C >= 1 && 2 * C + 2 <= HEADS_MAXW; }
int launch_heads_loss(const float* hid, const HeadsOut& hp, const long long* y, const float* e, const float* s, int B, int C,
                      int Fh, float scale, float* outs, float* terms, int* pred, float* dhid, hipStream_t stream, float* dlog) {
  if (!heads_loss_ok(B, C)) return (int)hipErrorInvalidValue;
  const int prof = gemm_prof_open(stream, 0.0, PROF_TAIL);
  const int S = B <= 64 ? 1 : (B <= 256 ? 2 : (B <= 512 ? 4 : 8));
  const dim3 grid((B + S - 1) / S);
  if (C <= 8) hipLaunchKernelGGL(heads_loss_kernel<true>, grid, dim3(256), 0, stream, hid, hp, y, e, s, B, S, C, Fh, scale, outs, terms, pred, dhid, dlog);
  else        hipLaunchKernelGGL(heads_loss_kernel<false>, grid, dim3(256), 0, stream, hid, hp, y, e, s, B, S, C, Fh, scale, outs, terms, pred, dhid, dlog);
  gemm_prof_close(prof, stream);
  return (int)hipGetLastError();
}

int device_cus() {
  static const int cus = [] { int dev = 0, n = 0; (void)hipGetDevice(&dev); (void)hipDeviceGetAttribute(&n, hipDeviceAttributeMultiprocessorCount, dev); return n; }();
  return cus;
}
int tail_fused_ok(int B, int C, int cus) {
  return B >= 1 && B <= TF_MAXGROUPS * TF_MAXB && C >= 1 && 2 * C + 2 <= TF_MAXW && cus >= TG * ((B + TF_MAXB - 1) / TF_MAXB);
}
int tail_fused_ok(int B, int C) { return tail_fused_ok(B, C, device_cus()); }
int launch_tail_fused(const TailFusedArgs& a, hipStream_t stream) {
  if (!tail_fused_ok(a.B, a.C)) return (int)hipErrorInvalidValue;
  if (a.mode && (!a.comb_out || !a.F1_out || !a.fused_out || !a.dhid_out || !a.dfused_out || !a.dF1_out)) return (int)hipErrorInvalidValue;
  const int prof = gemm_prof_open(stream, 0.0, PROF_TAIL);
  launch_lds<tail_fused_kernel>(dim3(TG * ((a.B + TF_MAXB - 1) / TF_MAXB)), dim3(TF_THREADS), TF_LDS_FLOATS * 4, stream, a);
  gemm_prof_close(prof, stream);
  return (int)hipGetLastError();
}

int tail_timeouts(unsigned int* out) {
  return (int)hipMemcpyFromSymbol(out, HIP_SYMBOL(g_tail_timeouts), sizeof(unsigned int));
}

__global__ void tail_poison_to_grads_kernel(float* __restrict__ g) {
  if (__hip_atomic_load(&g_tail_poison, __ATOMIC_RELAXED, __HIP_MEMORY_SCOPE_AGENT) != 0u) g[0] = __uint_as_float(0x7FC00000u);
}
int launch_tail_poison_to_grads(float* g, hipStream_t stream) {
  hipLaunchKernelGGL(tail_poison_to_grads_kernel, dim3(1), dim3(1), 0, stream, g);
  return (int)hipGetLastError();
}

int launch_sumsq(const float* g, size_t n, float* out, hipStream_t stream) {
  const int prof = gemm_prof_open(stream, 0.0, PROF_OPT);
  hipLaunchKernelGGL(sumsq_kernel, dim3(SUMSQ_BLOCKS), dim3(256), 0, stream, g, n, out);
  gemm_prof_close(prof, stream);
  return (int)hipGetLastError();
}

__device__ __forceinline__ size_t shadow_chunk(int N, int K, int n, int k0) {
  const int KS = K >> 4, NTw = N >> 7, tile32 = n >> 5;
  const int w = tile32 / NTw, t = tile32 - w * NTw;
  return (((size_t)w * KS + (k0 >> 4)) * NTw + t) * 64 + (n & 31) + 32 * ((k0 >> 3) & 1);
}

__global__ __launch_bounds__(256) void adamw_shadow_kernel(float* __restrict__ p, float* __restrict__ g, float* __restrict__ m,
                                                           float* __restrict__ v, float* __restrict__ sumsq, float max_norm, float lr,
                                                           float b1, float b2, float eps, float wd, float inv_bc1, float inv_sqrt_bc2,
                                                           int zero_grads, const AdamShadowArgs a) {
  __shared__ float red[4];
  __shared__ __attribute__((aligned(16))) unsigned short tile[32 * 72];
  const int tid = threadIdx.x;
  const bool is_tile = (int)blockIdx.x < a.tiles;
  int bi = 0, tr = 0, tc = 0;
  const int r = tid >> 3, c = tid & 7;
  float4 *p4 = nullptr, *g4 = nullptr, *m4 = nullptr, *v4 = nullptr;
  float4 pa, pb, ga, gb, ma, mb, va, vb;
  if (is_tile) {
#pragma unroll
    for (int i = 1; i < ADAM_SHADOW_MAXB; ++i)
      if (i < a.nblk && (int)blockIdx.x >= a.blk[i].tile_begin) bi = i;
    const AdamShadowBlock& B = a.blk[bi];
    const int tl = (int)blockIdx.x - B.tile_begin, ct = B.cols >> 6;
    tr = tl / ct; tc = tl - tr * ct;
    const size_t e = B.off + (size_t)(32 * tr + r) * B.cols + 64 * tc + 8 * c;
    p4 = reinterpret_cast<float4*>(p + e); g4 = reinterpret_cast<float4*>(g + e);
    m4 = reinterpret_cast<float4*>(m + e); v4 = reinterpret_cast<float4*>(v + e);
    pa = p4[0]; pb = p4[1]; ga = g4[0]; gb = g4[1]; ma = m4[0]; mb = m4[1]; va = v4[0]; vb = v4[1];
  }
  {
    const float part = wave_sum(sumsq[1 + tid]);
    if ((tid & 63) == 0) red[tid >> 6] = part;
    __syncthreads();
  }
  const float total = (red[0] + red[1]) + (red[2] + red[3]);
  if (blockIdx.x == 0 && tid == 0) sumsq[0] = total;
  const float coef = fminf(1.0f, max_norm / (sqrtf(total) + 1e-6f));
  const bool skip_step = !(total < __builtin_huge_valf());
  const float decay = 1.0f - lr * wd, step = lr * inv_bc1, omb1 = 1.0f - b1, omb2 = 1.0f - b2;
  auto upd = [&](float& pi, float& gi, float& mi, float& vi) {
    adamw_update(pi, gi, mi, vi, skip_step, coef, decay, b1, omb1, b2, omb2, step, inv_sqrt_bc2, eps, zero_grads);
  };
  if (is_tile) {
    const AdamShadowBlock& B = a.blk[bi];
    const int row = 32 * tr + r, col = 64 * tc + 8 * c;
    upd(pa.x, ga.x, ma.x, va.x); upd(pa.y, ga.y, ma.y, va.y); upd(pa.z, ga.z, ma.z, va.z); upd(pa.w, ga.w, ma.w, va.w);
    upd(pb.x, gb.x, mb.x, vb.x); upd(pb.y, gb.y, mb.y, vb.y); upd(pb.z, gb.z, mb.z, vb.z); upd(pb.w, gb.w, mb.w, vb.w);
    p4[0] = pa; p4[1] = pb; g4[0] = ga; g4[1] = gb; m4[0] = ma; m4[1] = mb; v4[0] = va; v4[1] = vb;
    const uint4 ch = make_uint4(pack2(pa.x, pa.y), pack2(pa.z, pa.w), pack2(pb.x, pb.y), pack2(pb.z, pb.w));
    reinterpret_cast<uint4*>(B.plain)[shadow_chunk(B.pN, B.cols, B.pn0 + row, col)] = ch;
    if (B.trans) {
      *reinterpret_cast<uint4*>(tile + r * 72 + 8 * c) = ch;
      __syncthreads();
      const int cl = tid & 63, rc = tid >> 6;
      unsigned short t8[8];
#pragma unroll
      for (int i = 0; i < 8; ++i) t8[i] = tile[(8 * rc + i) * 72 + cl];
      const uint4 tch = make_uint4((unsigned)t8[0] | ((unsigned)t8[1] << 16), (unsigned)t8[2] | ((unsigned)t8[3] << 16),
                                   (unsigned)t8[4] | ((unsigned)t8[5] << 16), (unsigned)t8[6] | ((unsigned)t8[7] << 16));
      reinterpret_cast<uint4*>(B.trans)[shadow_chunk(B.cols, B.tK, 64 * tc + cl, B.tk0 + 32 * tr + 8 * rc)] = tch;
    }
    return;
  }
  const int eb = (int)blockIdx.x - a.tiles, neb = (int)gridDim.x - a.tiles;
  auto run = [&](int ri, size_t first, size_t stride) {
    const size_t n4 = a.range_len[ri] >> 2;
    float4* p4 = reinterpret_cast<float4*>(p + a.range_begin[ri]); float4* g4 = reinterpret_cast<float4*>(g + a.range_begin[ri]);
    float4* m4 = reinterpret_cast<float4*>(m + a.range_begin[ri]); float4* v4 = reinterpret_cast<float4*>(v + a.range_begin[ri]);
    for (size_t i = first; i < n4; i += stride) {
      float4 pp = p4[i], gg = g4[i], mm = m4[i], vv = v4[i];
      upd(pp.x, gg.x, mm.x, vv.x); upd(pp.y, gg.y, mm.y, vv.y); upd(pp.z, gg.z, mm.z, vv.z); upd(pp.w, gg.w, mm.w, vv.w);
      p4[i] = pp; g4[i] = gg; m4[i] = mm; v4[i] = vv;
    }
  };
  const int nsmall = a.nrange - a.nbig;
  if (eb >= neb - nsmall) run(a.nbig + (eb - (neb - nsmall)), tid, 256);
  else for (int ri = 0; ri < a.nbig; ++ri) run(ri, (size_t)eb * 256 + tid, (size_t)(neb - nsmall) * 256);
}

int launch_clip_adamw_shadows(float* p, float* g, float* m, float* v, float* sumsq, float max_norm, float lr, float b1, float b2,
                              float eps, float wd, int step, int zero_grads, AdamShadowArgs& a, hipStream_t stream) {
  if (a.nblk < 1 || a.nblk > ADAM_SHADOW_MAXB || a.nrange < 0 || a.nrange > ADAM_SHADOW_MAXR) return (int)hipErrorInvalidValue;
  if ((reinterpret_cast<uintptr_t>(p) | reinterpret_cast<uintptr_t>(g) | reinterpret_cast<uintptr_t>(m) | reinterpret_cast<uintptr_t>(v)) & 15)
    return (int)hipErrorInvalidValue;
  int tiles = 0;
  for (int i = 0; i < a.nblk; ++i) {
    AdamShadowBlock& B = a.blk[i];
    if ((B.rows & 31) || (B.cols & 63) || (B.off & 3) || !B.plain || (B.pN & 127) || (B.pn0 & 31) || (B.trans && ((B.cols & 127) || (B.tK & 15) || (B.tk0 & 31))))
      return (int)hipErrorInvalidValue;
    B.tile_begin = tiles;
    tiles += (B.rows >> 5) * (B.cols >> 6);
  }
  for (int i = 0; i < a.nrange; ++i)
    if ((a.range_begin[i] & 3) || (a.range_len[i] & 3)) return (int)hipErrorInvalidValue;
  a.tiles = tiles;
  for (int i = 1; i < a.nrange; ++i)
    for (int j = i; j > 0 && a.range_len[j] > a.range_len[j - 1]; --j) {
      const size_t tb = a.range_begin[j], tl = a.range_len[j];
      a.range_begin[j] = a.range_begin[j - 1]; a.range_len[j] = a.range_len[j - 1]; a.range_begin[j - 1] = tb; a.range_len[j - 1] = tl;
    }
  a.nbig = 0;
  size_t big = 0;
  while (a.nbig < a.nrange && a.range_len[a.nbig] >= 8192) big += a.range_len[a.nbig++];
  size_t nb = (big / 4 + 255) / 256;
  if (nb < 1) nb = 1;
  if (nb > 1000) nb = 1000;
  nb += (size_t)(a.nrange - a.nbig);
  const double bc1 = 1.0 - pow((double)b1, step), bc2 = 1.0 - pow((double)b2, step);
  const int prof = gemm_prof_open(stream, 0.0, PROF_OPT);
  hipLaunchKernelGGL(adamw_shadow_kernel, dim3((unsigned)(tiles + nb)), dim3(256), 0, stream, p, g, m, v, sumsq, max_norm, lr, b1, b2, eps, wd,
                     (float)(1.0 / bc1), (float)(1.0 / sqrt(bc2)), zero_grads, a);
  gemm_prof_close(prof, stream);
  return (int)hipGetLastError();
}

int launch_clip_adamw(float* p, float* g, float* m, float* v, size_t n, float* sumsq, float max_norm,
                      float lr, float b1, float b2, float eps, float wd, int step, int zero_grads, hipStream_t stream) {
  const double bc1 = 1.0 - pow((double)b1, step), bc2 = 1.0 - pow((double)b2, step);
  size_t nb = (n / 4 + 255) / 256;
  if (nb < 1) nb = 1;
  if (nb > 1024) nb = 1024;
  const int prof = gemm_prof_open(stream, 0.0, PROF_OPT);
  hipLaunchKernelGGL(clip_adamw_kernel, dim3((unsigned)nb), dim3(256), 0, stream, p, g, m, v, n, sumsq, max_norm, lr,
                     b1, b2, eps, wd, (float)(1.0 / bc1), (float)(1.0 / sqrt(bc2)), zero_grads);
  gemm_prof_close(prof, stream);
  return (int)hipGetLastError();
}
```

Before: 94510 images/s.

## Split FFN first-layer weight gradient into per-sample mask×Y products and combine

The FFN first-layer weight gradient is factored per sample. The tail kernel gets extra blocks that compute M = mask^T·Y and per-feature mask counts using MFMA, and these run concurrently with the per-sample tail. In bwd1, 128 extra blocks combine M with the per-sample dHm scale to accumulate dW and db. This replaces the two full row-level dH×Y GEMMs and skips materializing and padding dH16. The cost is new per-sample fp32 scratch buffers (B×512×256 each), and the path is limited to B≤16 under one specific plan combination.

```diff
diff --git a/camouflage_multimodal_amd/csrc/fused_rows.h b/camouflage_multimodal_amd/csrc/fused_rows.h
--- a/camouflage_multimodal_amd/csrc/fused_rows.h
+++ b/camouflage_multimodal_amd/csrc/fused_rows.h
@@ -62,6 +62,8 @@
 struct TailWgProd { const float* dy; const float* x; float* dW; float* db; int ld_dy, ld_x, rows, cols; int tile_begin; };
 #define TAIL_WG_MAXP 8
 struct TailWgArgs { TailWgProd p[TAIL_WG_MAXP]; int n, B, tiles; };
+struct FfnCombStream { const float* M; const float* cnt; float* dW; float* db; };
+struct FfnCombArgs { FfnCombStream s[2]; int on; };
 struct Bwd1Args {
   Bwd1Stream s[2];
   const us16* Q16; const us16* KV16;
@@ -74,6 +76,7 @@
   int writer_blocks, writer_first_row;
   void* zero_ptr[FUSED_BWD1_MAXZ]; unsigned zero_bytes[FUSED_BWD1_MAXZ]; int nzero;
   TailWgArgs twg;
+  FfnCombArgs fcomb;
 };
 int launch_fused_bwd1(Bwd1Args& a, int variant, hipStream_t stream, int kg_only = 0);
 int launch_wide2_bwd1(Bwd1Args& a, int variant, hipStream_t stream);
diff --git a/camouflage_multimodal_amd/csrc/fused_rows.hip b/camouflage_multimodal_amd/csrc/fused_rows.hip
--- a/camouflage_multimodal_amd/csrc/fused_rows.hip
+++ b/camouflage_multimodal_amd/csrc/fused_rows.hip
@@ -600,6 +600,40 @@
   stamp(stamps, 3);
 }
 
+__device__ __forceinline__ void ffn_comb_tile(const Bwd1Args& a, int tile, float* cs, unsigned long long* stamps) {
+  stamp(stamps, 0);
+  const int kg = tile >> 6, f0 = 8 * (tile & 63), tid = threadIdx.x, B = a.B;
+  const FfnCombStream& P = a.fcomb.s[kg];
+  const Bwd1Stream& S = a.s[kg];
+  if (tid < 8 * B) {
+    const int sm = tid >> 3;
+    const float gs = (kg ? 1.0f / (float)a.Nk : a.inv_nr[sm]) * a.drop.scale;
+    cs[tid] = S.dHm[(size_t)sm * S.ld_dHm + f0 + (tid & 7)] * gs;
+  }
+  float acc[8];
+#pragma unroll
+  for (int r = 0; r < 8; ++r) acc[r] = P.dW[(size_t)(f0 + r) * 256 + tid];
+  float bacc = tid < 8 ? P.db[f0 + tid] : 0.f;
+  __syncthreads();
+  stamp(stamps, 1);
+  const float* m = P.M + (size_t)f0 * 256 + tid;
+#pragma unroll 4
+  for (int sm = 0; sm < B; ++sm) {
+    float v[8];
+#pragma unroll
+    for (int r = 0; r < 8; ++r) v[r] = m[(size_t)sm * (512 * 256) + r * 256];
+    const float4 c0 = *reinterpret_cast<const float4*>(cs + 8 * sm), c1 = *reinterpret_cast<const float4*>(cs + 8 * sm + 4);
+    acc[0] = fmaf(c0.x, v[0], acc[0]); acc[1] = fmaf(c0.y, v[1], acc[1]); acc[2] = fmaf(c0.z, v[2], acc[2]); acc[3] = fmaf(c0.w, v[3], acc[3]);
+    acc[4] = fmaf(c1.x, v[4], acc[4]); acc[5] = fmaf(c1.y, v[5], acc[5]); acc[6] = fmaf(c1.z, v[6], acc[6]); acc[7] = fmaf(c1.w, v[7], acc[7]);
+    if (tid < 8) bacc = fmaf(cs[8 * sm + tid], P.cnt[(size_t)sm * 512 + f0 + tid], bacc);
+  }
+  stamp(stamps, 2);
+#pragma unroll
+  for (int r = 0; r < 8; ++r) P.dW[(size_t)(f0 + r) * 256 + tid] = acc[r];
+  if (tid < 8) P.db[f0 + tid] = bacc;
+  stamp(stamps, 3);
+}
+
 template <int DEPTH, bool ROT>
 __global__ __launch_bounds__(256, 2) void bwd1_kernel(const Bwd1Args a) {
   extern __shared__ __attribute__((aligned(16))) char smem[];
@@ -607,6 +641,10 @@
   const int w = __builtin_amdgcn_readfirstlane(tid >> 6);
   const bool kg = (int)blockIdx.x >= a.rg_tiles_max && (int)blockIdx.x < a.rg_tiles_max + a.B;
   const int rot = ROT ? (int)(blockIdx.x >> 3) : 0;
+  if ((int)blockIdx.x >= a.B + a.rg_tiles_max + a.writer_blocks + a.nzero + a.twg.tiles) {
+    ffn_comb_tile(a, (int)blockIdx.x - a.B - a.rg_tiles_max - a.writer_blocks - a.nzero - a.twg.tiles, reinterpret_cast<float*>(smem), a.stamps);
+    return;
+  }
   if ((int)blockIdx.x >= a.B + a.rg_tiles_max + a.writer_blocks + a.nzero) {
     tail_wg_tile(a.twg, (int)blockIdx.x - a.B - a.rg_tiles_max - a.writer_blocks - a.nzero, reinterpret_cast<float*>(smem), a.stamps);
     return;
@@ -1347,12 +1385,15 @@
     const Bwd1Stream& S = a.s[i];
     if (!S.W1T || !S.WoT || !S.mask || !S.XH16 || !S.rstd || !S.ln_g || !S.dHm || !S.dcomb || !S.dH16 || !S.dU16 || !S.dgamma || !S.dbeta)
       return (int)hipErrorInvalidValue;
+    const FfnCombStream& F = a.fcomb.s[i];
+    if (a.fcomb.on && (kg_only || a.B > 16 || !F.M || !F.cnt || !F.dW || !F.db)) return (int)hipErrorInvalidValue;
     if (!al16(S.W1T) || !al16(S.WoT) || !al16(S.mask) || !al16(S.ln_g) || !al16(S.dcomb) || (S.ld_dcomb & 3) || !al16(S.dH16) || !al16(S.dU16))
       return (int)hipErrorInvalidValue;
   }
   a.writer_first_row = kg_only ? a.rows_rg : 0;
   a.writer_blocks = (a.rows_rg + a.B * a.Nk - a.writer_first_row + 15) / 16;
   if (a.writer_blocks > 8192) a.writer_blocks = 8192;
+  if (a.fcomb.on) a.writer_blocks = 0;
   if (a.nzero < 0 || a.nzero > FUSED_BWD1_MAXZ) return (int)hipErrorInvalidValue;
   for (int i = 0; i < a.nzero; ++i)
     if (!a.zero_ptr[i] || !al16(a.zero_ptr[i]) || (a.zero_bytes[i] & 15)) return (int)hipErrorInvalidValue;
@@ -1368,7 +1409,7 @@
   }
   Bwd1Args k = a;
   if (kg_only) { k.rg_tiles_max = 0; k.stamps = nullptr; }
-  const dim3 grid(k.B + k.rg_tiles_max + k.writer_blocks + k.nzero + k.twg.tiles);
+  const dim3 grid(k.B + k.rg_tiles_max + k.writer_blocks + k.nzero + k.twg.tiles + (k.fcomb.on ? 128 : 0));
   const double rows = (kg_only ? 0.0 : (double)a.rows_rg) + (double)a.B * a.Nk;
   const int prof = gemm_prof_open(stream, 2.0 * rows * (512.0 * 256.0 + 256.0 * 256.0) + (kg_only ? 0.0 : 10.0 * (double)a.rows_rg * a.Nk * 256.0), PROF_BWD1);
   if (variant == 0) launch_lds<bwd1_kernel<12, false>>(grid, dim3(256), W_LDS, stream, k);
diff --git a/camouflage_multimodal_amd/csrc/fusion_abi.hip b/camouflage_multimodal_amd/csrc/fusion_abi.hip
--- a/camouflage_multimodal_amd/csrc/fusion_abi.hip
+++ b/camouflage_multimodal_amd/csrc/fusion_abi.hip
@@ -85,6 +85,7 @@
     us16 *W1T, *W2T, *Wo1T, *Wo2T, *WcRgT, *WcKgT;
     us16 *dH16, *dH2_16, *dU16, *dU2_16, *dQKV16, *dQKVkg16, *dR16, *dG16, *dO2_16;
     float *delta2, *dGpart;
+    float *ffnM1, *ffnM2, *ffncnt1, *ffncnt2;
     us16* tailw[20];
   } f;
   int* tickets;
@@ -173,6 +174,10 @@
         for (int i = 0; i < 10; ++i) f.tailw[i] = c.take<us>(i < 6 ? 2 * H * H : (i < 8 ? H * H : 2 * H * H));
         for (int i = 10; i < 20; ++i) f.tailw[i] = c.take<us>((i == 12 || i == 13) ? H * H : 2 * H * H);
         f.Wf_rg = c.take<us>(3 * H * D); f.bf_rg = c.take<float>(3 * H);
+        if (B <= 16) {
+          f.ffnM1 = c.take<float>((size_t)B * 2 * H * H); f.ffnM2 = c.take<float>((size_t)B * 2 * H * H);
+          f.ffncnt1 = c.take<float>((size_t)B * 2 * H); f.ffncnt2 = c.take<float>((size_t)B * 2 * H);
+        }
       }
     }
   } else {
@@ -290,6 +295,8 @@
   bool fused_maps;
   int cus;
 };
+
+static bool ffn_wg_split(const camo_plan_t& p) { return p.tail_wg == CAMO_TAIL_WG_BWD1 && p.bwd1 == CAMO_BWD1_ROWS32; }
 
 static void plan_fused_forward(const PlanIn& in, bool save, bool param_space, camo_plan_t& p) {
   const camo_options_t& o = in.o;
@@ -577,9 +584,10 @@
       zero(w.zero_base, w.zero_bytes);
       const size_t t = T, tk = TK;
       auto pad = [&](us* buf, size_t rows, size_t rows_p, size_t width) { zero(buf + rows * width, (rows_p - rows) * width * sizeof(us)); };
-      pad(f.X16, t, w.Tp, D); pad(f.R16, t, w.Tp, H); pad(f.O16, t, w.Tp, H); pad(f.Y16, t, w.Tp, H); pad(f.dH16, t, w.Tp, 2 * H);
+      const bool dh = !ffn_wg_split(pl);
+      pad(f.X16, t, w.Tp, D); pad(f.R16, t, w.Tp, H); pad(f.O16, t, w.Tp, H); pad(f.Y16, t, w.Tp, H); if (dh) pad(f.dH16, t, w.Tp, 2 * H);
       pad(f.dU16, t, w.Tp, H); pad(f.dQKV16, t, w.Tp, 3 * H); pad(f.dR16, t, w.Tp, H);
-      pad(f.KG16, tk, w.TKp, D); pad(f.G16, tk, w.TKp, H); pad(f.O2_16, tk, w.TKp, H); pad(f.Y2_16, tk, w.TKp, H); pad(f.dH2_16, tk, w.TKp, 2 * H);
+      pad(f.KG16, tk, w.TKp, D); pad(f.G16, tk, w.TKp, H); pad(f.O2_16, tk, w.TKp, H); pad(f.Y2_16, tk, w.TKp, H); if (dh) pad(f.dH2_16, tk, w.TKp, 2 * H);
       pad(f.dU2_16, tk, w.TKp, H); pad(f.dQKVkg16, tk, w.TKp, 3 * H); pad(f.dG16, tk, w.TKp, H);
       zero(w.dHm1, (size_t)B * 2 * H * sizeof(float)); zero(w.dHm2, (size_t)B * 2 * H * sizeof(float));
     } else {
@@ -759,6 +767,11 @@
   a.stamps = g_dbg_stamps ? g_dbg_stamps + (size_t)4 * g_dbg_stamp_blocks * 8 : nullptr;
   a.debug_skip = c.tail_skip;
   if (fl) { a.comb_out = w.comb; a.F1_out = w.F1; a.fused_out = w.fused; a.dhid_out = w.dhid; a.dfused_out = w.dfused; a.dF1_out = w.dF1; }
+  if (fl && ffn_wg_split(x.plan)) {
+    const Ws::F17& f = w.f;
+    a.fw.s[0] = FfnWgStream{f.mask1, f.Y16, f.ffnM1, f.ffncnt1}; a.fw.s[1] = FfnWgStream{f.mask2, f.Y2_16, f.ffnM2, f.ffncnt2};
+    a.fw.off = x.rg_offsets; a.fw.Nk = x.Nk; a.fw_rows = x.T + B * x.Nk;
+  }
   CK(launch_tail_fused(a, st), "per-sample tail (one launch)");
   c.tail_skip_taken = a.debug_skip != 0;
   if (x.plan.tail_wg == CAMO_TAIL_WG_LAUNCH) {
@@ -830,6 +843,12 @@
     });
     t.B = B;
   }
+  const bool split = ffn_wg_split(pl);
+  if (split) {
+    a1.fcomb.s[0] = FfnCombStream{f.ffnM1, f.ffncnt1, Gr[CAMO_P_F1_W0], Gr[CAMO_P_F1_B0]};
+    a1.fcomb.s[1] = FfnCombStream{f.ffnM2, f.ffncnt2, Gr[CAMO_P_F2_W0], Gr[CAMO_P_F2_B0]};
+    a1.fcomb.on = 1;
+  }
   if (pl.bwd1 == CAMO_BWD1_64) CK(launch_wide2_bwd1(a1, x.opt->fused_variant, st), "fused backward, first half (64-row half-blocks)");
   else                         CK(launch_fused_bwd1(a1, x.opt->fused_variant, st), "fused backward, first half");
   if (pl.tail_event == CAMO_EVENT_AFTER_BWD1) CK(record_tail_event(c, st), "tail event");
@@ -847,12 +866,12 @@
   else CK(launch_fused_bwd2(a2, x.opt->fused_variant, st), "fused backward, second half");
   if (!param_space) {
     GB16 g(drop, *x.opt, st);
-    g.tn(f.dH16, 2 * H, f.Y16, H, Gr[CAMO_P_F1_W0], H, Gr[CAMO_P_F1_B0], 2 * H, H, T);
+    if (!split) g.tn(f.dH16, 2 * H, f.Y16, H, Gr[CAMO_P_F1_W0], H, Gr[CAMO_P_F1_B0], 2 * H, H, T);
     g.tn(f.dU16, H, f.O16, H, Gr[CAMO_P_A1_OUT_W], H, Gr[CAMO_P_A1_OUT_B], H, H, T);
     g.tn(f.dQKV16, 3 * H, f.R16, H, Gr[CAMO_P_A1_IN_W], H, Gr[CAMO_P_A1_IN_B], H, H, T);
     g.tn(f.dQKV16 + H, 3 * H, f.R16, H, Gr[CAMO_P_A2_IN_W] + HH, H, Gr[CAMO_P_A2_IN_B] + H, 2 * H, H, T);
     g.tn(f.dR16, H, f.X16, D, Gr[CAMO_P_RG_PROJ_W], D, Gr[CAMO_P_RG_PROJ_B], H, D, T);
-    g.tn(f.dH2_16, 2 * H, f.Y2_16, H, Gr[CAMO_P_F2_W0], H, Gr[CAMO_P_F2_B0], 2 * H, H, TK);
+    if (!split) g.tn(f.dH2_16, 2 * H, f.Y2_16, H, Gr[CAMO_P_F2_W0], H, Gr[CAMO_P_F2_B0], 2 * H, H, TK);
     g.tn(f.dU2_16, H, f.O2_16, H, Gr[CAMO_P_A2_OUT_W], H, Gr[CAMO_P_A2_OUT_B], H, H, TK);
     g.tn(f.dQKVkg16, 3 * H, f.G16, H, Gr[CAMO_P_A2_IN_W], H, Gr[CAMO_P_A2_IN_B], H, H, TK);
     g.tn(f.dQKVkg16 + H, 3 * H, f.G16, H, Gr[CAMO_P_A1_IN_W] + HH, H, Gr[CAMO_P_A1_IN_B] + H, 2 * H, H, TK);
@@ -863,12 +882,12 @@
   float* const Mrg = w.parM; float* const Mkg = Mrg + (size_t)3 * H * D;
   float* const dbrg = Mkg + (size_t)3 * H * D; float* const dbkg = dbrg + 3 * H;
   GB16 g(drop, *x.opt, st);
-  g.tn(f.dH16, 2 * H, f.Y16, H, Gr[CAMO_P_F1_W0], H, Gr[CAMO_P_F1_B0], 2 * H, H, T);
+  if (!split) g.tn(f.dH16, 2 * H, f.Y16, H, Gr[CAMO_P_F1_W0], H, Gr[CAMO_P_F1_B0], 2 * H, H, T);
   g.tn(f.dU16, H, f.O16, H, Gr[CAMO_P_A1_OUT_W], H, Gr[CAMO_P_A1_OUT_B], H, H, T);
   g.tn(f.dQKV16, 3 * H, f.X16, D, Mrg, D, dbrg, H, D, T).bias_grad2 = Gr[CAMO_P_A1_IN_B];
   g.tn(f.dQKV16 + H, 3 * H, f.X16, D, Mrg + (size_t)H * D, D, dbrg + H, 2 * H, D, T).bias_grad2 = Gr[CAMO_P_A2_IN_B] + H;
   g.tn(f.dU16, H, f.X16, D, Gr[CAMO_P_RG_PROJ_W], D, Gr[CAMO_P_RG_PROJ_B], H, D, T);
-  g.tn(f.dH2_16, 2 * H, f.Y2_16, H, Gr[CAMO_P_F2_W0], H, Gr[CAMO_P_F2_B0], 2 * H, H, TK);
+  if (!split) g.tn(f.dH2_16, 2 * H, f.Y2_16, H, Gr[CAMO_P_F2_W0], H, Gr[CAMO_P_F2_B0], 2 * H, H, TK);
   g.tn(f.dU2_16, H, f.O2_16, H, Gr[CAMO_P_A2_OUT_W], H, Gr[CAMO_P_A2_OUT_B], H, H, TK);
   g.tn(f.dQKVkg16, 3 * H, f.KG16, D, Mkg, D, dbkg, H, D, TK).bias_grad2 = Gr[CAMO_P_A2_IN_B];
   g.tn(f.dQKVkg16 + H, 3 * H, f.KG16, D, Mkg + (size_t)H * D, D, dbkg + H, 2 * H, D, TK).bias_grad2 = Gr[CAMO_P_A1_IN_B] + H;
diff --git a/camouflage_multimodal_amd/csrc/misc.h b/camouflage_multimodal_amd/csrc/misc.h
--- a/camouflage_multimodal_amd/csrc/misc.h
+++ b/camouflage_multimodal_amd/csrc/misc.h
@@ -43,6 +43,9 @@
 int launch_clip_adamw(float* p, float* g, float* m, float* v, size_t n, float* sumsq, float max_norm,
                       float lr, float b1, float b2, float eps, float wd, int step, int zero_grads, hipStream_t stream);
 
+struct FfnWgStream { const uint32_t* mask; const unsigned short* Y16; float* M; float* cnt; };
+struct FfnWgArgs { FfnWgStream s[2]; const int* off; int Nk; int blocks; };
+
 struct TailFusedArgs {
   const float *Ymean, *H1mean, *Y2mean, *H2mean;
   const float *W13, *b13, *W23, *b23, *Wfu0, *bfu0, *Wfu3, *bfu3; const float* Wh0[4]; const float* bh0[4]; const float* Wh3[4]; const float* bh3[4];
@@ -53,6 +56,7 @@
   float *dcomb, *dHm1, *dHm2;
   float *comb_out, *F1_out, *fused_out, *dhid_out, *dfused_out, *dF1_out;
   int B, C, mode; DropCfg drop;
+  FfnWgArgs fw; int fw_rows;
   unsigned long long* stamps;
   int debug_skip;
 };
diff --git a/camouflage_multimodal_amd/csrc/misc.hip b/camouflage_multimodal_amd/csrc/misc.hip
--- a/camouflage_multimodal_amd/csrc/misc.hip
+++ b/camouflage_multimodal_amd/csrc/misc.hip
@@ -1,5 +1,6 @@
 #include "misc.h"
 #include "gemm.h"
+#include "mfma_inl.h"
 
 
 namespace {
@@ -606,14 +607,122 @@
 }
 
 constexpr int TF_THREADS = 1024;
+static_assert(4 * 32768 <= TF_LDS_FLOATS * 4 && (3 * 4 * 32 * 64 + 64) * 4 <= TF_LDS_FLOATS * 4, "ffn_wg_block lives in the tail launch's LDS");
+
+constexpr int FW_PKA = 192, FW_PKB = 320, FW_A_BYTES = 64 * FW_PKA, FW_BUF = FW_A_BYTES + 64 * FW_PKB;
+__device__ __forceinline__ void ffn_wg_block(const FfnWgArgs& fw, int e, int B, char* smem, unsigned long long* stamps) {
+  unsigned long long* const stp = stamps ? stamps + (size_t)TG * 32 + (size_t)e * 8 : nullptr;
+  if (stp && threadIdx.x == 0) stp[0] = __builtin_amdgcn_s_memrealtime();
+  const int kgs = e >= 16 * B ? 1 : 0, el = e - 16 * B * kgs, smp = el >> 4, ft = (el & 15) >> 1, ch = el & 1;
+  const FfnWgStream& S = fw.s[kgs];
+  const int row0 = kgs ? smp * fw.Nk : fw.off[smp], nrows = kgs ? fw.Nk : fw.off[smp + 1] - row0;
+  const int nsteps = (nrows + 255) >> 8;
+  const int tid = threadIdx.x, lane = tid & 63, l31 = lane & 31, h = lane >> 5;
+  const int kgp = __builtin_amdgcn_readfirstlane(tid >> 8), t = tid & 255, wv = __builtin_amdgcn_readfirstlane((tid >> 6) & 3);
+  const int wr = wv >> 1, wc = wv & 1;
+  char* const base = smem + kgp * FW_BUF;
+  const int mshift = 8 * (t & 3), kra = 64 * kgp + (t >> 3), krb = 64 * kgp + (t >> 4);
+  const int la = (t >> 3) * FW_PKA + 16 * (t & 7), lb = FW_A_BYTES + (t >> 4) * FW_PKB + 16 * (t & 15);
+  const uint32_t* const mbase = S.mask + (size_t)row0 * 16 + 2 * ft + ((t & 7) >> 2);
+  const char* const ybase = reinterpret_cast<const char*>(S.Y16) + (size_t)row0 * 512 + 2 * (128 * ch + 8 * (t & 15));
+  uint32_t ra[2]; u32x4 rb[4];
+  auto gload = [&](int step) {
+#pragma unroll
+    for (int i = 0; i < 2; ++i) {
+      const int r = 256 * step + kra + 32 * i;
+      const uint32_t wd = mbase[(uint32_t)min(r, nrows - 1) * 16u];
+      ra[i] = r < nrows ? (wd >> mshift) & 0xFFu : 0u;
+    }
+#pragma unroll
+    for (int i = 0; i < 4; ++i) rb[i] = *reinterpret_cast<const u32x4*>(ybase + (uint32_t)min(256 * step + krb + 16 * i, nrows - 1) * 512u);
+  };
+  f32x16 acc[2] = {zero16(), zero16()};
+  const bool do_cnt = ch == 0;
+  uint32_t cnt_lo = 0u, cnt_hi = 0u;
+  const int g = (lane >> 4) & 1, q = (lane >> 2) & 3, p = lane & 3;
+  const int fa = (8 * h + q) * FW_PKA + 64 * wr + 32 * g + 8 * p;
+  const int fb = FW_A_BYTES + (8 * h + q) * FW_PKB + 128 * wc + 32 * g + 8 * p;
+  gload(0);
+  if (stp && threadIdx.x == 0) stp[1] = __builtin_amdgcn_s_memrealtime();
+  for (int step = 0; step < nsteps; ++step) {
+#pragma unroll
+    for (int i = 0; i < 2; ++i) {
+      const uint32_t b = ra[i];
+      u32x4 v;
+#pragma unroll
+      for (int d = 0; d < 4; ++d) v[d] = (((b >> (2 * d)) & 1u) ? 0x3F80u : 0u) | (((b >> (2 * d + 1)) & 1u) ? 0x3F800000u : 0u);
+      *reinterpret_cast<u32x4*>(base + la + 32 * i * FW_PKA) = v;
+      cnt_lo += (b & 1u) | ((b & 2u) << 7) | ((b & 4u) << 14) | ((b & 8u) << 21);
+      cnt_hi += ((b >> 4) & 1u) | ((b & 0x20u) << 3) | ((b & 0x40u) << 10) | ((b & 0x80u) << 17);
+    }
+#pragma unroll
+    for (int i = 0; i < 4; ++i) *reinterpret_cast<u32x4*>(base + lb + 16 * i * FW_PKB) = rb[i];
+    __syncthreads();
+    gload(min(step + 1, nsteps - 1));
+    __builtin_amdgcn_sched_barrier(0);
+#pragma unroll
+    for (int s = 0; s < 4; ++s) {
+      const char* pa = base + fa + 16 * s * FW_PKA;
+      const char* pb = base + fb + 16 * s * FW_PKB;
+      const bf16x8 a = join(lds_tr16(pa), lds_tr16(pa + 4 * FW_PKA));
+      const bf16x8 b0 = join(lds_tr16(pb), lds_tr16(pb + 4 * FW_PKB));
+      const bf16x8 b1 = join(lds_tr16(pb + 64), lds_tr16(pb + 64 + 4 * FW_PKB));
+      acc[0] = __builtin_amdgcn_mfma_f32_32x32x16_bf16(a, b0, acc[0], 0, 0, 0);
+      acc[1] = __builtin_amdgcn_mfma_f32_32x32x16_bf16(a, b1, acc[1], 0, 0, 0);
+    }
+    __syncthreads();
+  }
+  if (stp && threadIdx.x == 0) stp[2] = __builtin_amdgcn_s_memrealtime();
+  float* const red = reinterpret_cast<float*>(smem);
+  int* const redc = reinterpret_cast<int*>(red + 3 * 4 * 32 * 64);
+  if (kgp > 0) {
+    float* r = red + ((kgp - 1) * 4 + wv) * (32 * 64) + lane;
+#pragma unroll
+    for (int j = 0; j < 2; ++j)
+#pragma unroll
+      for (int i = 0; i < 16; ++i) r[(16 * j + i) * 64] = acc[j][i];
+  }
+  if (do_cnt) {
+    if (tid < 64) redc[tid] = 0;
+    __syncthreads();
+#pragma unroll
+    for (int j = 0; j < 4; ++j) {
+      atomicAdd(redc + 8 * (t & 7) + j, (int)((cnt_lo >> (8 * j)) & 0xFFu));
+      atomicAdd(redc + 8 * (t & 7) + 4 + j, (int)((cnt_hi >> (8 * j)) & 0xFFu));
+    }
+  }
+  __syncthreads();
+  if (kgp == 0) {
+#pragma unroll 1
+    for (int k = 0; k < 3; ++k) {
+      const float* r = red + (k * 4 + wv) * (32 * 64) + lane;
+#pragma unroll
+      for (int j = 0; j < 2; ++j)
+#pragma unroll
+        for (int i = 0; i < 16; ++i) acc[j][i] += r[(16 * j + i) * 64];
+    }
+    const int f0 = 64 * ft + 32 * wr;
+    float* const Mo = S.M + ((size_t)smp * 512 + f0) * 256 + 128 * ch + 64 * wc + l31;
+#pragma unroll
+    for (int j = 0; j < 2; ++j)
+#pragma unroll
+      for (int i = 0; i < 16; ++i) Mo[(size_t)acc_row(i, h) * 256 + 32 * j] = acc[j][i];
+    if (do_cnt && tid < 64) S.cnt[(size_t)smp * 512 + 64 * ft + tid] = (float)redc[tid];
+  }
+  if (stp && threadIdx.x == 0) stp[3] = __builtin_amdgcn_s_memrealtime();
+}
 
 __global__ __launch_bounds__(TF_THREADS) void tail_fused_kernel(const TailFusedArgs a) {
   extern __shared__ __attribute__((aligned(16))) float sm[];
   __shared__ int s_timed_out;
+  if (a.fw.blocks && (int)blockIdx.x >= TG) {
+    ffn_wg_block(a.fw, (int)blockIdx.x - TG, a.B, reinterpret_cast<char*>(sm), a.stamps);
+    return;
+  }
   if (threadIdx.x == 0) s_timed_out = 0;
   const bool wg = a.mode != 0;
   const int tid = threadIdx.x, lane = tid & 63, g = blockIdx.x & (TG - 1), sg = blockIdx.x >> 6, C = a.C, Wd = 2 * C + 2;
-  const bool multi = gridDim.x > TG;
+  const bool multi = a.B > TF_MAXB;
   const int sb = TF_MAXB * sg, B = min(TF_MAXB, a.B - sb);
   const float* const gYmean = a.Ymean + (size_t)sb * 256; const float* const gY2mean = a.Y2mean + (size_t)sb * 256;
   const float* const gH1mean = a.H1mean + (size_t)sb * 512; const float* const gH2mean = a.H2mean + (size_t)sb * 512;
@@ -1307,8 +1416,19 @@
 int launch_tail_fused(const TailFusedArgs& a, hipStream_t stream) {
   if (!tail_fused_ok(a.B, a.C)) return (int)hipErrorInvalidValue;
   if (a.mode && (!a.comb_out || !a.F1_out || !a.fused_out || !a.dhid_out || !a.dfused_out || !a.dF1_out)) return (int)hipErrorInvalidValue;
-  const int prof = gemm_prof_open(stream, 0.0, PROF_TAIL);
-  launch_lds<tail_fused_kernel>(dim3(TG * ((a.B + TF_MAXB - 1) / TF_MAXB)), dim3(TF_THREADS), TF_LDS_FLOATS * 4, stream, a);
+  TailFusedArgs k = a;
+  k.fw.blocks = 0;
+  double fl = 0.0;
+  if (a.fw.s[0].M || a.fw.s[1].M) {
+    const FfnWgStream& r = a.fw.s[0]; const FfnWgStream& g = a.fw.s[1];
+    if (!a.mode || a.B > TF_MAXB || a.fw.Nk < 1 || !a.fw.off || !r.mask || !r.Y16 || !r.M || !r.cnt || !g.mask || !g.Y16 || !g.M || !g.cnt ||
+        (reinterpret_cast<uintptr_t>(r.Y16) & 15) || (reinterpret_cast<uintptr_t>(g.Y16) & 15))
+      return (int)hipErrorInvalidValue;
+    k.fw.blocks = 2 * a.B * 16;
+    fl = 2.0 * 512.0 * 256.0 * (double)a.fw_rows;
+  }
+  const int prof = gemm_prof_open(stream, fl, PROF_TAIL);
+  launch_lds<tail_fused_kernel>(dim3(TG * ((a.B + TF_MAXB - 1) / TF_MAXB) + k.fw.blocks), dim3(TF_THREADS), TF_LDS_FLOATS * 4, stream, k);
   gemm_prof_close(prof, stream);
   return (int)hipGetLastError();
 }
```

New measurement: 93290 images/s. 0.987x the previous value.
